# cloudflare/zkp-ecdsa

Measured on NVIDIA H100. Metric: ZKAttest proofs/sec, higher is better.
Workload: dtype u256/u258 (32-bit limbs, Montgomery)

## Files before the change

### __graft_entry__.py

```python
from __future__ import annotations

import hashlib
import os
import subprocess
import sys

ROOT = os.path.dirname(os.path.abspath(__file__))
CSRC = os.path.join(ROOT, 'zkp_ecdsa_b200', 'csrc')
LIB = os.path.join(ROOT, 'zkp_ecdsa_b200', 'libzkattest.so')
LIB_WAR = os.path.join(ROOT, 'zkp_ecdsa_b200', 'libzkattest_war256.so')
HOSTSIM = os.path.join(ROOT, 'tests', 'hostsim', 'libzkattest_hostsim.so')
HOSTSIM_WAR = os.path.join(ROOT, 'tests', 'hostsim', 'libzkattest_hostsim_war256.so')
PROBE_SRC = os.path.join(ROOT, 'tests', 'probe', 'zk_probe.cu')
PROBE = os.path.join(ROOT, 'tests', 'probe', 'libzkprobe.so')
PROBE_HOST = os.path.join(ROOT, 'tests', 'probe', 'libzkprobe_host.so')
PROBE_JAC_SRC = os.path.join(ROOT, 'tests', 'probe', 'zk_probe_jac.cu')
PROBE_JAC = os.path.join(ROOT, 'tests', 'probe', 'libzkprobe_jac.so')
PROBE_JAC_HOST = os.path.join(ROOT, 'tests', 'probe', 'libzkprobe_jac_host.so')
PROBE_SEED_SRC = os.path.join(ROOT, 'tests', 'probe', 'zk_probe_seed.cu')
PROBE_SEED = os.path.join(ROOT, 'tests', 'probe', 'libzkprobe_seed.so')
PROBE_SEED_HOST = os.path.join(ROOT, 'tests', 'probe', 'libzkprobe_seed_host.so')
ORACLE_CPU = os.path.join(ROOT, 'oracle', '_ref', 'libzkattest_cpu.so')
ARCH = ['-gencode', 'arch=compute_90a,code=sm_90a']
NVCC_FLAGS = ARCH + ['-O3', '-std=c++17', '-lineinfo',
              '--compiler-options', '-fPIC', '-shared']


def _sources():
    return sorted(os.path.join(CSRC, f) for f in os.listdir(CSRC) if f.endswith(('.cu', '.cuh', '.h', '.inc')))


def _stamp(extra='', files=()):
    h = hashlib.sha256(extra.encode())
    for p in _sources() + [os.path.join(ROOT, 'include', 'zkattest.h')] + list(files):
        h.update(p.encode())
        h.update(open(p, 'rb').read())
    return h.hexdigest()


def _build_if_stale(out, cmd, tag, files=()):
    stamp_file = out + '.stamp'
    stamp = _stamp(' '.join(cmd), files)
    if os.path.exists(out) and os.path.exists(stamp_file) and open(stamp_file).read() == stamp:
        return False
    print(f'[build] {tag}: {" ".join(cmd)}', flush=True)
    tmp = out + '.tmp'
    subprocess.check_call([tmp if c == out else c for c in cmd], cwd=ROOT)
    os.replace(tmp, out)
    open(stamp_file, 'w').write(stamp)
    return True


def build_lib():
    nvcc = os.environ.get('NVCC', '/usr/local/cuda/bin/nvcc')
    cmd = [nvcc] + NVCC_FLAGS + ['-I' + os.path.join(ROOT, 'include'), '-I' + CSRC, '-o', LIB,
                                 os.path.join(CSRC, 'zkattest.cu')]
    return _build_if_stale(LIB, cmd, 'libzkattest.so (sm_90a)')


def build_lib_war():
    nvcc = os.environ.get('NVCC', '/usr/local/cuda/bin/nvcc')
    cmd = [nvcc] + NVCC_FLAGS + ['-DZKA_PG_WAR256', '-I' + os.path.join(ROOT, 'include'), '-I' + CSRC, '-o', LIB_WAR,
                                 os.path.join(CSRC, 'zkattest.cu')]
    return _build_if_stale(LIB_WAR, cmd, 'libzkattest_war256.so (sm_90a)')


def build_hostsim(war=False):
    out = HOSTSIM_WAR if war else HOSTSIM
    os.makedirs(os.path.dirname(out), exist_ok=True)
    cmd = ['g++', '-std=c++17', '-O2', '-DZKA_HOSTSIM'] + (['-DZKA_PG_WAR256'] if war else []) + [
        '-x', 'c++', '-I' + os.path.join(ROOT, 'include'), '-I' + CSRC, '-fPIC', '-shared', '-o', out,
        os.path.join(CSRC, 'zkattest.cu')]
    return _build_if_stale(out, cmd, 'hostsim war256 (tests only)' if war else 'hostsim (tests only)')


def build_probe(host=False, jac=False):
    out = (PROBE_JAC_HOST if host else PROBE_JAC) if jac else (PROBE_HOST if host else PROBE)
    src = PROBE_JAC_SRC if jac else PROBE_SRC
    if host:
        cmd = ['g++', '-std=c++17', '-O2', '-DZKA_HOSTSIM', '-x', 'c++', '-fPIC', '-shared']
    else:
        cmd = [os.environ.get('NVCC', '/usr/local/cuda/bin/nvcc')] + NVCC_FLAGS
    cmd += ['-I' + os.path.join(ROOT, 'include'), '-I' + CSRC, '-o', out, src]
    tag = ('probe_jac' if jac else 'probe') + (' host (tests only)' if host else ' (sm_90a, tests only)')
    return _build_if_stale(out, cmd, tag, [PROBE_SRC, PROBE_JAC_SRC] if jac else [PROBE_SRC])


def build_probe_seed(host=False):
    out = PROBE_SEED_HOST if host else PROBE_SEED
    if host:
        cmd = ['g++', '-std=c++17', '-O2', '-DZKA_HOSTSIM', '-x', 'c++', '-fPIC', '-shared']
    else:
        cmd = [os.environ.get('NVCC', '/usr/local/cuda/bin/nvcc')] + NVCC_FLAGS
    cmd += ['-I' + os.path.join(ROOT, 'include'), '-I' + CSRC, '-o', out, PROBE_SEED_SRC]
    return _build_if_stale(out, cmd, 'probe_seed' + (' host (tests only)' if host else ' (sm_90a, tests only)'), [PROBE_SEED_SRC])


def build_oracle_cpu():
    src = os.path.join(ROOT, 'oracle', 'cpu', 'zkattest_cpu.cpp')
    hdr = os.path.join(ROOT, 'include', 'zkattest.h')
    if os.path.exists(ORACLE_CPU) and os.path.getmtime(ORACLE_CPU) >= max(os.path.getmtime(src), os.path.getmtime(hdr)):
        return False
    print('[build] oracle/cpu -> oracle/_ref/libzkattest_cpu.so', flush=True)
    subprocess.check_call(['make', '-C', os.path.join(ROOT, 'oracle', 'cpu')])
    return True


def build_tools():
    nvcc = os.environ.get('NVCC', '/usr/local/cuda/bin/nvcc')
    tdir = os.path.join(ROOT, 'tools')
    for name in ('imad_peak', 'mul_peak'):
        src, out = os.path.join(tdir, name + '.cu'), os.path.join(tdir, name)
        if not os.path.exists(src):
            continue
        if os.path.exists(out) and os.path.getmtime(out) >= max(os.path.getmtime(p) for p in _sources() + [src]):
            continue
        cmd = [nvcc] + ARCH + ['-O3', '-std=c++17', '-I' + CSRC,
               '-I' + os.path.join(ROOT, 'include'), '-o', out, src]
        print(f'[build] tools/{name}: {" ".join(cmd)}', flush=True)
        subprocess.check_call(cmd, cwd=ROOT)


def build() -> None:
    from concurrent.futures import ThreadPoolExecutor
    jobs = [build_lib, build_lib_war, build_hostsim, lambda: build_hostsim(war=True), build_oracle_cpu, build_tools,
            build_probe, lambda: build_probe(host=True), lambda: build_probe(jac=True),
            lambda: build_probe(host=True, jac=True), build_probe_seed, lambda: build_probe_seed(host=True)]
    with ThreadPoolExecutor(max_workers=min(len(jobs), max(1, (os.cpu_count() or 2)))) as ex:
        for f in [ex.submit(j) for j in jobs]:
            f.result()
    sys.path.insert(0, ROOT)
    import zkp_ecdsa_b200
    import oracle


def smoke() -> None:
    sys.path.insert(0, ROOT)
    import numpy as np
    from zkp_ecdsa_b200 import api, synth
    from oracle import flat
    from oracle import zkattest as OZ
    from oracle.big import Tape

    eng = api.Engine(device=0)
    rnd = synth.params_rnd(1)
    params = eng.generate_params_list(rnd=rnd)
    wl = synth.Workload(B=2, N=8, seed=1)
    tape = synth.random_tape(2, eng.lib.prove_tape_len(8), seed=2)
    res = eng.prove_batch(params, wl.msg_hash, wl.sig, wl.pk, wl.which, wl.ring, tape)
    assert (res.status == 0).all(), res.status
    oparams = OZ.generate_params_list(Tape(rnd))
    for b in range(2):
        pr = OZ.prove_signature_list(oparams, wl.msg_hash[b].tobytes(), wl.sig[b].tobytes(), wl.pk[b].tobytes(),
                                     int(wl.which[b]), wl.ring_ints(), Tape(tape[b].tobytes()))
        assert flat.ser_proof(pr) == res.proof_bytes(b), f'proof {b} differs from the oracle'
    from oracle import seed_tape as ST
    seed = bytes(range(32))
    rs = eng.prove_batch_seeded(params, wl.msg_hash[:1], wl.sig[:1], wl.pk[:1], wl.which[:1], wl.ring,
                                np.frombuffer(seed, np.uint8).reshape(1, 32).copy())
    assert rs.status[0] == 0, rs.status
    pr = OZ.prove_signature_list(oparams, wl.msg_hash[0].tobytes(), wl.sig[0].tobytes(), wl.pk[0].tobytes(),
                                 int(wl.which[0]), wl.ring_ints(), Tape(ST.prove_tape(seed, 80, 3)))
    assert flat.ser_proof(pr) == rs.proof_bytes(0), 'seeded proof differs from the oracle on the expanded tape'
    from zkp_ecdsa_b200 import verify_tape as VT
    vts = eng.lib.verify_tape_len(8, 80)
    ok = np.zeros(2, np.uint8)
    st = np.zeros(2, np.int32)
    eng.lib.verify_batch(params.handle, 2, wl.msg_hash, wl.ring, 8, res.proofs, res.proofs.shape[1], res.proof_len,
                         VT.random_verify_tape(2, vts, 8, 80, seed=3), vts, ok, st)
    assert list(ok) == [1, 1] and not st.any(), (ok, st)
    rw = synth.RingsWorkload(2, [17, 5], [1, 0], seed=5)
    rings = eng.load_rings(rw.rings)
    rt = synth.random_tape(2, eng.lib.prove_tape_len(17), seed=6)
    rr = eng.prove_batch_rings(params, rings, rw.ring_of, rw.msg_hash, rw.sig, rw.pk, rw.which, rt)
    assert (rr.status == 0).all(), rr.status
    for b in range(2):
        pr = OZ.prove_signature_list(oparams, rw.msg_hash[b].tobytes(), rw.sig[b].tobytes(), rw.pk[b].tobytes(),
                                     int(rw.which[b]), rw.ring_ints(int(rw.ring_of[b])), Tape(rt[b].tobytes()))
        assert flat.ser_proof(pr) == rr.proof_bytes(b), f'ring-set proof {b} differs from the oracle'
    rings.close()
    launched = eng.lib.launch_count()
    war = ''
    if os.path.exists(LIB_WAR):
        from oracle.curves import tomEdwards256, war256
        ew = api.Engine(device=0, proof_group='war256')
        pw = ew.generate_params_list(16, rnd=rnd)
        tw = synth.random_tape(1, ew.lib.prove_tape_len(8, 16), seed=4)
        rw = ew.prove_batch(pw, wl.msg_hash[:1], wl.sig[:1], wl.pk[:1], wl.which[:1], wl.ring, tw)
        assert (rw.status == 0).all(), rw.status
        flat.set_proof_group(war256)
        try:
            ow = OZ.generate_params_list(Tape(rnd), 16, war256)
            pr = OZ.prove_signature_list(ow, wl.msg_hash[0].tobytes(), wl.sig[0].tobytes(), wl.pk[0].tobytes(),
                                         int(wl.which[0]), wl.ring_ints(), Tape(tw[0].tobytes()))
            assert flat.ser_proof(pr) == rw.proof_bytes(0), 'war256 proof differs from the oracle'
        finally:
            flat.set_proof_group(tomEdwards256)
        launched += ew.lib.launch_count()
        war = '; war256 build: 1 proof bit-exact'
    print(f'smoke ok: 2 proofs bit-exact vs oracle and accepted by the verifier, 1 seeded proof bit-exact, '
          f'2 ring-set proofs over rings of depths 3 and 5 bit-exact{war}; '
          'kernels launched:', launched)


if __name__ == '__main__':
    build()
    if len(sys.argv) > 1 and sys.argv[1] == 'smoke':
        smoke()
```

### zkp_ecdsa_b200/capi.py

```python
from __future__ import annotations

import ctypes as C
import os
from typing import Optional

import numpy as np

_HERE = os.path.dirname(os.path.abspath(__file__))
DEFAULT_LIB = os.path.join(_HERE, 'libzkattest.so')

SYMBOLS = [
    'zka_init', 'zka_shutdown', 'zka_last_error', 'zka_version', 'zka_launch_count',
    'zka_params_generate', 'zka_params_create', 'zka_params_destroy', 'zka_key_to_int',
    'zka_proof_max_len', 'zka_prove_tape_len', 'zka_verify_tape_len',
    'zka_prove_batch', 'zka_verify_batch',
    'zka_tom_commit_batch', 'zka_p256_mul_batch', 'zka_field_op_batch', 'zka_hash80_batch',
    'zka_get_stream', 'zka_set_profiling', 'zka_profile_reset', 'zka_profile_json', 'zka_config',
    'zka_lanes', 'zka_set_option', 'zka_proofs_pack', 'zka_proofs_unpack', 'zka_verify_batch_ex', 'zka_verify_tape_len_ex',
    'zka_verify_exp_batch', 'zka_verify_membership_batch', 'zka_verify_equality_batch', 'zka_verify_mult_batch',
    'zka_verify_pointadd_batch', 'zka_prove_exp_batch', 'zka_prove_membership_batch',
    'zka_prove_equality_batch', 'zka_prove_mult_batch', 'zka_prove_pointadd_batch', 'zka_stat', 'zka_proof_group', 'zka_set_progress', 'zka_chunk_schedule',
    'zka_prove_batch_seeded', 'zka_verify_batch_seeded', 'zka_seed_tape',
    'zka_rings_create', 'zka_rings_destroy', 'zka_prove_batch_rings', 'zka_prove_batch_rings_seeded', 'zka_verify_batch_rings',
    'zka_verify_batch_rings_seeded',
# ... 96 lines not shown
                                              C.c_size_t, C.c_void_p, C.c_void_p, C.c_size_t, C.c_void_p, C.c_void_p, C.c_uint32]
            L.zka_set_option.argtypes = [C.c_void_p, C.c_char_p, C.c_long]
            L.zka_stat.restype = C.c_longlong
            L.zka_stat.argtypes = [C.c_void_p, C.c_char_p]
            L.zka_verify_exp_batch.argtypes = [C.c_void_p, C.c_void_p, C.c_uint32] + [C.c_void_p] * 6 + [C.c_size_t, C.c_void_p, C.c_void_p,
                                               C.c_size_t, C.c_uint32, C.c_void_p, C.c_void_p]
            L.zka_verify_membership_batch.argtypes = [C.c_void_p, C.c_void_p, C.c_uint32, C.c_void_p, C.c_void_p, C.c_uint32, C.c_void_p,
                                                      C.c_size_t, C.c_void_p, C.c_void_p, C.c_size_t, C.c_void_p, C.c_void_p]
            for f in ('zka_verify_equality_batch', 'zka_verify_mult_batch', 'zka_verify_pointadd_batch'):
                getattr(L, f).argtypes = [C.c_void_p, C.c_void_p, C.c_uint32, C.c_void_p, C.c_void_p, C.c_void_p, C.c_size_t,
                                          C.c_void_p, C.c_void_p]
            L.zka_prove_exp_batch.argtypes = [C.c_void_p, C.c_void_p, C.c_uint32] + [C.c_void_p] * 5 + [C.c_size_t, C.c_void_p, C.c_size_t,
                                              C.c_void_p, C.c_void_p]
            L.zka_prove_membership_batch.argtypes = [C.c_void_p, C.c_void_p, C.c_uint32, C.c_void_p, C.c_void_p, C.c_void_p, C.c_uint32,
                                                     C.c_void_p, C.c_size_t, C.c_void_p, C.c_size_t, C.c_void_p, C.c_void_p]
            for f in ('zka_prove_equality_batch', 'zka_prove_mult_batch'):
                getattr(L, f).argtypes = [C.c_void_p, C.c_void_p, C.c_uint32, C.c_void_p, C.c_void_p, C.c_size_t, C.c_void_p, C.c_void_p,
                                          C.c_void_p]
            L.zka_prove_pointadd_batch.argtypes = [C.c_void_p, C.c_void_p, C.c_uint32, C.c_void_p, C.c_void_p, C.c_void_p, C.c_size_t,
                                                   C.c_void_p, C.c_void_p, C.c_void_p]
            L.zka_proofs_pack.argtypes = [C.c_void_p, C.c_uint32, C.c_void_p, C.c_size_t, C.c_void_p, C.c_void_p, C.c_size_t,
                                          C.c_void_p, C.c_void_p]
            L.zka_proofs_unpack.argtypes = [C.c_void_p, C.c_uint32, C.c_void_p, C.c_size_t, C.c_void_p, C.c_void_p, C.c_size_t,
                                            C.c_void_p, C.c_void_p]
        if hasattr(L, 'zka_seed_tape'):
            L.zka_prove_batch_seeded.argtypes = [C.c_void_p, C.c_void_p, C.c_uint32] + [C.c_void_p] * 5 + [C.c_uint32, C.c_void_p,
                                                 C.c_void_p, C.c_size_t, C.c_void_p, C.c_void_p]
            L.zka_verify_batch_seeded.argtypes = [C.c_void_p, C.c_void_p, C.c_uint32, C.c_void_p, C.c_void_p, C.c_uint32, C.c_void_p,
                                                  C.c_size_t, C.c_void_p, C.c_void_p, C.c_uint32, C.c_void_p, C.c_void_p]
            L.zka_seed_tape.argtypes = [C.c_void_p, C.c_int, C.c_uint32, C.c_void_p, C.c_uint32, C.c_uint32, C.c_uint32, C.c_void_p,
                                        C.c_size_t]
        if hasattr(L, 'zka_rings_create'):
            L.zka_rings_create.argtypes = [C.c_void_p, C.c_uint32, C.c_void_p, C.c_void_p, C.POINTER(C.c_void_p)]
            L.zka_rings_destroy.argtypes = [C.c_void_p]
            L.zka_prove_batch_rings.argtypes = [C.c_void_p, C.c_void_p, C.c_void_p, C.c_void_p, C.c_uint32] + [C.c_void_p] * 5 + [
                C.c_size_t, C.c_void_p, C.c_size_t, C.c_void_p, C.c_void_p]
            L.zka_prove_batch_rings_seeded.argtypes = [C.c_void_p, C.c_void_p, C.c_void_p, C.c_void_p, C.c_uint32] + [C.c_void_p] * 6 + [
                C.c_size_t, C.c_void_p, C.c_void_p]
            L.zka_verify_batch_rings.argtypes = [C.c_void_p, C.c_void_p, C.c_void_p, C.c_void_p, C.c_uint32, C.c_void_p, C.c_void_p,
                                                 C.c_size_t, C.c_void_p, C.c_void_p, C.c_size_t, C.c_uint32, C.c_void_p, C.c_void_p]
            L.zka_verify_batch_rings_seeded.argtypes = [C.c_void_p, C.c_void_p, C.c_void_p, C.c_void_p, C.c_uint32, C.c_void_p,
                                                        C.c_void_p, C.c_size_t, C.c_void_p, C.c_void_p, C.c_uint32, C.c_void_p,
                                                        C.c_void_p]
        ctx = C.c_void_p()
        rc = L.zka_init(device, C.byref(ctx))
        if rc != 0 or not ctx:
            raise ZkaError(f'zka_init(device={device}) failed with {rc}: no usable CUDA device '
                           '(libzkattest has no CPU fallback)')
        self.ctx = ctx
        self.device = device

    def close(self):
        if getattr(self, 'ctx', None):
            self.lib.zka_shutdown(self.ctx)
            self.ctx = None

    def _check(self, rc, what):
        if rc != 0:
            raise ZkaError(f'{what} failed ({rc}): {self.lib.zka_last_error(self.ctx).decode()}')

    def launch_count(self) -> int:
        return int(self.lib.zka_launch_count(self.ctx))

    def stream_ptr(self) -> int:
        return int(self.lib.zka_get_stream(self.ctx) or 0)

    def set_profiling(self, on: bool):
        self._check(self.lib.zka_set_profiling(self.ctx, 1 if on else 0), 'zka_set_profiling')

    def profile_reset(self):
        self._check(self.lib.zka_profile_reset(self.ctx), 'zka_profile_reset')

    def profile(self) -> dict:
        import json
        n = self.lib.zka_profile_json(self.ctx, None, 0)
        buf = C.create_string_buffer(int(n) + 16)
        self.lib.zka_profile_json(self.ctx, buf, len(buf))
        return json.loads(buf.value.decode())

    def config(self) -> dict:
        w, nw, ch = C.c_int(), C.c_int(), C.c_int()
        self._check(self.lib.zka_config(self.ctx, C.byref(w), C.byref(nw), C.byref(ch)), 'zka_config')
        lanes = int(self.lib.zka_lanes(self.ctx)) if hasattr(self.lib, 'zka_lanes') else 1
        return {'tom_w': w.value, 'tom_nwin': nw.value, 'chunk': ch.value, 'lanes': lanes}

    def set_option(self, key: str, value: int):
        self._check(self.lib.zka_set_option(self.ctx, key.encode(), int(value)), f'zka_set_option({key})')

    def chunk_schedule(self, B: int, host_buffers: bool = False):
        off = np.zeros(4096, np.uint32)
        self.lib.zka_chunk_schedule.argtypes = [C.c_void_p, C.c_uint32, C.c_int, C.c_void_p, C.c_uint32]
        n = self.lib.zka_chunk_schedule(self.ctx, B, 1 if host_buffers else 0, _ptr(off), off.size)
        if n < 0:
            raise ZkaError('zka_chunk_schedule')
        return [int(v) for v in off[:n + 1]]

    def set_progress(self, flags: Optional[np.ndarray]):
        self.lib.zka_set_progress.argtypes = [C.c_void_p, C.c_void_p, C.c_uint32]
        if flags is None:
            self._check(self.lib.zka_set_progress(self.ctx, None, 0), 'zka_set_progress')
        else:
            assert flags.dtype == np.uint32 and flags.flags['C_CONTIGUOUS']
            self._check(self.lib.zka_set_progress(self.ctx, _ptr(flags), flags.size), 'zka_set_progress')

    def stat(self, key: str) -> int:
        return int(self.lib.zka_stat(self.ctx, key.encode()))

    def proof_max_len(self, ring_size, sec_level=80): return int(self.lib.zka_proof_max_len(ring_size, sec_level))
    def prove_tape_len(self, ring_size, sec_level=80): return int(self.lib.zka_prove_tape_len(ring_size, sec_level))
    def verify_tape_len(self, ring_size, sec_level=80): return int(self.lib.zka_verify_tape_len(ring_size, sec_level))

    def params_generate(self, rnd: bytes):
        assert len(rnd) == 64
        hn = np.zeros(65, np.uint8)
        hp = np.zeros(self.wp, np.uint8)
        self._check(self.lib.zka_params_generate(self.ctx, _ptr(rnd), _ptr(hn), _ptr(hp)), 'zka_params_generate')
        return hn.tobytes(), hp.tobytes()

    def params_create(self, h_nist: bytes, h_proof: bytes, sec_level: int = 80):
        h = C.c_void_p()
        self._check(self.lib.zka_params_create(self.ctx, _ptr(h_nist), _ptr(h_proof), sec_level, C.byref(h)),
                    'zka_params_create')
        return h

    def params_destroy(self, h):
        self.lib.zka_params_destroy(h)

    def key_to_int(self, pk: np.ndarray):
        count = pk.shape[0]
        out = np.zeros((count, 32), np.uint8)
        st = np.zeros(count, np.int32)
        self._check(self.lib.zka_key_to_int(self.ctx, count, _ptr(pk), _ptr(out), _ptr(st)), 'zka_key_to_int')
        return out, st

    def prove_batch(self, params, B, msg_hash, sig, pk, which, ring, N, tape, tape_stride,
                    proofs, proof_stride, proof_len, status):
        self._check(self.lib.zka_prove_batch(self.ctx, params, B, _ptr(msg_hash), _ptr(sig), _ptr(pk), _ptr(which),
                                             _ptr(ring), N, _ptr(tape), tape_stride, _ptr(proofs), proof_stride,
                                             _ptr(proof_len), _ptr(status)), 'zka_prove_batch')

    def verify_batch(self, params, B, msg_hash, ring, N, proofs, proof_stride, proof_len, tape, tape_stride,
                     ok, status):
        self._check(self.lib.zka_verify_batch(self.ctx, params, B, _ptr(msg_hash), _ptr(ring), N, _ptr(proofs),
                                              proof_stride, _ptr(proof_len), _ptr(tape), tape_stride, _ptr(ok),
                                              _ptr(status)), 'zka_verify_batch')

    def verify_tape_len_ex(self, ring_size, sec_level, samples):
        return int(self.lib.zka_verify_tape_len_ex(ring_size, sec_level, samples))

    def verify_batch_ex(self, params, B, msg_hash, ring, N, proofs, proof_stride, proof_len, tape, tape_stride, ok, status, samples):
        self._check(self.lib.zka_verify_batch_ex(self.ctx, params, B, _ptr(msg_hash), _ptr(ring), N, _ptr(proofs), proof_stride,
                                                 _ptr(proof_len), _ptr(tape), tape_stride, _ptr(ok), _ptr(status), samples),
                    'zka_verify_batch_ex')

    def prove_batch_seeded(self, params, B, msg_hash, sig, pk, which, ring, N, seeds, proofs, proof_stride, proof_len, status):
        self._check(self.lib.zka_prove_batch_seeded(self.ctx, params, B, _ptr(msg_hash), _ptr(sig), _ptr(pk), _ptr(which), _ptr(ring),
                                                    N, _ptr(seeds), _ptr(proofs), proof_stride, _ptr(proof_len), _ptr(status)),
                    'zka_prove_batch_seeded')

    def verify_batch_seeded(self, params, B, msg_hash, ring, N, proofs, proof_stride, proof_len, seeds, samples, ok, status):
        self._check(self.lib.zka_verify_batch_seeded(self.ctx, params, B, _ptr(msg_hash), _ptr(ring), N, _ptr(proofs), proof_stride,
                                                     _ptr(proof_len), _ptr(seeds), samples, _ptr(ok), _ptr(status)),
                    'zka_verify_batch_seeded')

    def seed_tape(self, kind, seeds, ring_size, sec_level=80, samples=20) -> np.ndarray:
        B = seeds.shape[0]
        ln = self.prove_tape_len(ring_size, sec_level) if kind == 0 else self.verify_tape_len_ex(ring_size, sec_level, samples)
# ... 136 lines not shown
```

### zkp_ecdsa_b200/csrc/zk_launch.cuh

```cuda
#pragma once
#include <stdint.h>
#include <stdlib.h>
#include <string.h>

#include <map>
#include <stdexcept>
#include <string>
#include <typeinfo>
#include <vector>

#include <cxxabi.h>

#if !defined(ZKA_HOSTSIM)
#include <cuda_runtime.h>
#endif

namespace zk {

#if !defined(ZKA_HOSTSIM)

#define ZK_CUDA_CHECK(expr)                                                                   \
  do {                                                                                        \
    cudaError_t _e = (expr);                                                                  \
    if (_e != cudaSuccess)                                                                    \
// ... 86 lines not shown
inline void copy_d2h_2d(Stream& st, void* h, size_t hpitch, const void* d, size_t dpitch, size_t width, size_t height) {
  if (width && height) ZK_CUDA_CHECK(cudaMemcpy2DAsync(h, hpitch, d, dpitch, width, height, cudaMemcpyDefault, st.s));
}
inline void dev_memset(Stream& st, void* d, int v, size_t n) {
  if (n) ZK_CUDA_CHECK(cudaMemsetAsync(d, v, n, st.s));
}
inline void sync(Stream& st) {
  ZK_CUDA_CHECK(cudaStreamSynchronize(st.s));
  if (!st.pending.empty()) prof_collect(st);
}
struct Event { cudaEvent_t e = nullptr; };
inline void stream_create(Stream& st) {
  if (!st.s) ZK_CUDA_CHECK(cudaStreamCreateWithFlags(&st.s, cudaStreamNonBlocking));
}
inline void stream_destroy(Stream& st) {
  if (st.s) cudaStreamDestroy(st.s);
  st.s = nullptr;
}
inline void ev_record(Event& ev, Stream& st) {
  if (!ev.e) ZK_CUDA_CHECK(cudaEventCreateWithFlags(&ev.e, cudaEventDisableTiming));
  ZK_CUDA_CHECK(cudaEventRecord(ev.e, st.s));
}
inline void ev_wait(Stream& st, Event& ev) {
  if (ev.e) ZK_CUDA_CHECK(cudaStreamWaitEvent(st.s, ev.e, 0));
}
inline void ev_destroy(Event& ev) {
  if (ev.e) cudaEventDestroy(ev.e);
  ev.e = nullptr;
}
inline bool is_device_ptr(const void* p) {
  cudaPointerAttributes a;
  cudaError_t e = cudaPointerGetAttributes(&a, p);
  if (e != cudaSuccess) {
    cudaGetLastError();
    return false;
  }
  return a.type == cudaMemoryTypeDevice || a.type == cudaMemoryTypeManaged;
}

#else

struct ProfEntry {
  uint64_t launches = 0;
  double ms = 0.0;
  uint64_t items = 0;
};
struct Stream {
  uint64_t launches = 0;
  bool profiling = false;
  std::map<std::string, ProfEntry> prof;
};
template <class Task>
inline void launch(Stream& st, long long n, const Task& task) {
  for (long long t = 0; t < n; t++) task((int)t);
  st.launches++;
}
inline void* dev_alloc(size_t bytes) { return calloc(bytes ? bytes : 1, 1); }
inline void dev_free(void* p) { free(p); }
inline void copy_h2d(Stream&, void* d, const void* h, size_t n) { if (n) memcpy(d, h, n); }
inline void copy_d2h(Stream&, void* h, const void* d, size_t n) { if (n) memcpy(h, d, n); }
inline void copy_d2d(Stream&, void* d, const void* s, size_t n) { if (n) memcpy(d, s, n); }
inline void copy_d2h_2d(Stream&, void* h, size_t hpitch, const void* d, size_t dpitch, size_t width, size_t height) {
  for (size_t r = 0; r < height; r++) memcpy((char*)h + r * hpitch, (const char*)d + r * dpitch, width);
}
inline void dev_memset(Stream&, void* d, int v, size_t n) { if (n) memset(d, v, n); }
inline void sync(Stream&) {}
struct Event {};
inline void stream_create(Stream&) {}
inline void stream_destroy(Stream&) {}
inline void ev_record(Event&, Stream&) {}
inline void ev_wait(Stream&, Event&) {}
inline void ev_destroy(Event&) {}
inline bool is_device_ptr(const void*) { return false; }

#endif

struct DevBuf {
  void* p = nullptr;
  size_t cap = 0;
  DevBuf() = default;
  DevBuf(const DevBuf&) = delete;
  DevBuf& operator=(const DevBuf&) = delete;
  ~DevBuf() { dev_free(p); }
  template <class T>
  T* get(size_t count) {
    size_t bytes = count * sizeof(T);
    if (bytes > cap) {
      dev_free(p);
      size_t want = bytes + bytes / 8 + 256;
      p = dev_alloc(want);
      cap = want;
    }
    return reinterpret_cast<T*>(p);
  }
};

struct Cursor {
  DevBuf *next_, *end_;
  template <size_t N>
  explicit Cursor(DevBuf (&pool)[N]) : next_(pool), end_(pool + N) {}
  DevBuf& next() {
    if (next_ == end_) throw std::runtime_error("workspace pool exhausted");
    return *next_++;
  }
  template <class T>
  T* take(size_t count) { return next().get<T>(count); }
  template <class T>
  T* take_if(bool need, size_t count) {
    T* p = take<T>(need ? count : 0);
    return need ? p : nullptr;
  }
};

}
```

### zkp_ecdsa_b200/csrc/zk_ops.cuh

```cuda
#pragma once
#include "zk_curves.cuh"
#include "zk_layout.h"
#include "zk_sha256.cuh"

namespace zk {

#if defined(__CUDA_ARCH__)
#define ZK_SET_STATUS(ptr, code) atomicCAS((int*)(ptr), 0, (int)(code))
#define ZK_SET_STATUS_OVER(ptr, code, over) \
  do {                                      \
    atomicCAS((int*)(ptr), 0, (int)(code)); \
    atomicCAS((int*)(ptr), (int)(over), (int)(code)); \
  } while (0)
#else
#define ZK_SET_STATUS_OVER(ptr, code, over)              \
  do {                                                   \
    if (*(ptr) == 0 || *(ptr) == (over)) *(ptr) = (code); \
  } while (0)
#define ZK_SET_STATUS(ptr, code) \
  do {                           \
    if (*(ptr) == 0) *(ptr) = (code); \
  } while (0)
#endif

// ... 97 lines not shown
#pragma unroll
  for (int i = 0; i < 9; i++) {
    const uint32_t a = q.x[i], b = q.y[i];
    q.x[i] = neg ? b : a;
    q.y[i] = neg ? a : b;
    q.k[i] = neg ? nk[i] : q.k[i];
  }
}
ZK_HD void tom_ld_pre(TomPre& q, const uint32_t* m) {
#if defined(__CUDA_ARCH__)
  const uint4* v = reinterpret_cast<const uint4*>(m);
  uint32_t w[32];
#pragma unroll
  for (int i = 0; i < 7; i++) {
    uint4 u = __ldg(v + i);
    w[4 * i] = u.x; w[4 * i + 1] = u.y; w[4 * i + 2] = u.z; w[4 * i + 3] = u.w;
  }
#pragma unroll
  for (int i = 0; i < 9; i++) { q.x[i] = w[i]; q.y[i] = w[9 + i]; q.k[i] = w[18 + i]; }
#else
  ld<9>(q.x, m); ld<9>(q.y, m + 9); ld<9>(q.k, m + 18);
#endif
}

#endif

ZK_HD void ld4(uint32_t* w, const void* p) {
#if defined(__CUDA_ARCH__)
  const uint4 u = *reinterpret_cast<const uint4*>(p);
  w[0] = u.x; w[1] = u.y; w[2] = u.z; w[3] = u.w;
#else
  const uint32_t* q = reinterpret_cast<const uint32_t*>(p);
  for (int i = 0; i < 4; i++) w[i] = q[i];
#endif
}
ZK_HD void st4(void* p, const uint32_t* w) {
#if defined(__CUDA_ARCH__)
  *reinterpret_cast<uint4*>(p) = make_uint4(w[0], w[1], w[2], w[3]);
#else
  uint32_t* q = reinterpret_cast<uint32_t*>(p);
  for (int i = 0; i < 4; i++) q[i] = w[i];
#endif
}
ZK_HD void ld8v(uint32_t* r, const uint32_t* p) { ld4(r, p); ld4(r + 4, p + 4); }
ZK_HD void st8v(uint32_t* p, const uint32_t* r) { st4(p, r); st4(p + 4, r + 4); }
ZK_HD bool aligned16(const void* p) { return ((size_t)p & 15) == 0; }

template <int N, int CB>
ZK_HD uint32_t enc_byte(int i, uint32_t tag, const uint32_t* x, const uint32_t* y) {
  if (i == 0) return tag;
  if (i >= 1 + 2 * CB) return 0u;
  const uint32_t* c = i <= CB ? x : y;
  const int pos = CB - 1 - (i <= CB ? i - 1 : i - 1 - CB);
  return (pos >> 2) < N ? ((c[pos >> 2] >> (8 * (pos & 3))) & 0xffu) : 0u;
}
template <int N, int CB>
ZK_HD void store_point_words(uint8_t* o, uint32_t tag, const uint32_t* x, const uint32_t* y) {
  uint32_t w[BSTRIDE / 4];
#pragma unroll
  for (int j = 0; j < BSTRIDE / 4; j++)
    w[j] = enc_byte<N, CB>(4 * j, tag, x, y) | (enc_byte<N, CB>(4 * j + 1, tag, x, y) << 8) |
           (enc_byte<N, CB>(4 * j + 2, tag, x, y) << 16) | (enc_byte<N, CB>(4 * j + 3, tag, x, y) << 24);
  if (aligned16(o)) {
#pragma unroll
    for (int j = 0; j < BSTRIDE / 16; j++) st4(o + 16 * j, w + 4 * j);
  } else {
    uint32_t* ow = reinterpret_cast<uint32_t*>(o);
#pragma unroll
    for (int j = 0; j < BSTRIDE / 4; j++) ow[j] = w[j];
  }
}

ZK_HD uint32_t digit4(const uint32_t* k, int j) { return (k[j >> 3] >> (4 * (j & 7))) & 15u; }
ZK_HD uint32_t digit8(const uint32_t* k, int j) { return (k[j >> 2] >> (8 * (j & 3))) & 255u; }
ZK_HD uint32_t digit_w(const uint32_t* k, int pos, int w) {
  int wi = pos >> 5, sh = pos & 31;
  uint64_t v = k[wi];
  if (wi + 1 < 8) v |= (uint64_t)k[wi + 1] << 32;
  return (uint32_t)(v >> sh) & ((1u << w) - 1u);
}

ZK_HD int fb_entries(int w) { return (1 << (w - 1)) + 1; }
ZK_HD int fb_windows(int w) { return (256 + w) / w; }
ZK_HD uint32_t signed_digit(const uint32_t* k, int j, int w, uint32_t& carry, bool& neg) {
  const int pos = j * w;
  uint32_t d = carry;
  if (pos < 256) d += digit_w(k, pos, (256 - pos) < w ? (256 - pos) : w);
  const uint32_t half = 1u << (w - 1);
  neg = d > half;
  carry = neg ? 1u : 0u;
  return neg ? (1u << w) - d : d;
}

ZK_HD uint32_t bswap32(uint32_t x) {
#if defined(__CUDA_ARCH__)
  return __byte_perm(x, 0u, 0x0123);
#else
  return (x >> 24) | ((x >> 8) & 0xff00u) | ((x << 8) & 0xff0000u) | (x << 24);
#endif
}
ZK_HD void tape_draw(uint32_t* r, const uint8_t* tape, int draw) {
  const uint8_t* p = tape + 32 * (size_t)draw;
#if defined(__CUDA_ARCH__)
  if (aligned16(p)) {
    const uint4 a = __ldg(reinterpret_cast<const uint4*>(p)), b = __ldg(reinterpret_cast<const uint4*>(p) + 1);
    r[7] = bswap32(a.x); r[6] = bswap32(a.y); r[5] = bswap32(a.z); r[4] = bswap32(a.w);
    r[3] = bswap32(b.x); r[2] = bswap32(b.y); r[1] = bswap32(b.z); r[0] = bswap32(b.w);
    return;
  }
#endif
#pragma unroll
  for (int i = 0; i < 8; i++) {
    const uint8_t* q = p + 28 - 4 * i;
    r[i] = ((uint32_t)q[0] << 24) | ((uint32_t)q[1] << 16) | ((uint32_t)q[2] << 8) | (uint32_t)q[3];
  }
}

#define WEI_PT P256Pt
#define WEI_AFF P256Aff
#define WEI_JAC P256Jac
#define WEI_F P256p
#define WEI_FN(n) p256_##n
#define WEI_T(n) P256##n
#include "zk_weier_ops.inc"
#undef WEI_PT
#undef WEI_AFF
#undef WEI_JAC
#undef WEI_F
#undef WEI_FN
#undef WEI_T

enum : int { KEY_W_MIN = 5, KEY_W_MAX = 8, KEY_CAP = 52 * 17 };
ZK_HD int key_window_bits(uint32_t count, uint32_t B, uint32_t uses) {
  int best = KEY_W_MIN;
  uint64_t best_cost = ~0ull;
  for (int w = KEY_W_MIN; w <= KEY_W_MAX; w++) {
    const uint64_t nwin = (uint64_t)fb_windows(w), ne = (uint64_t)fb_entries(w);
    if (w > KEY_W_MIN && (uint64_t)count * nwin * ne > (uint64_t)B * KEY_CAP) break;
    const uint64_t cost = nwin * ((uint64_t)count * (ne - 1) * 2 + (uint64_t)B * uses);
    if (cost < best_cost) { best_cost = cost; best = w; }
  }
  return best;
}
ZK_HD size_t key_table_words(int w) { return (size_t)fb_windows(w) * fb_entries(w) * P256_AFF_WORDS; }

enum : int { RT_W = 5, RT_NWIN = 52, RT_ROW = 16, RT_ENTRIES = RT_NWIN * RT_ROW };
struct P256RowsSignedTask {
  const uint32_t* pows;
  uint32_t* rows;
  const uint32_t* count_dev = nullptr;
  ZK_HD void operator()(int t) const {
    if (count_dev && (uint32_t)(t / RT_NWIN) >= *count_dev) return;
    P256Pt p, acc;
    p256_ld_proj(p, pows + (size_t)t * P256_PROJ_WORDS);
    acc = p;
    uint32_t* out = rows + (size_t)t * RT_ROW * P256_PROJ_WORDS;
    for (int d = 1; d <= RT_ROW; d++) {
      p256_st_proj(out + (size_t)(d - 1) * P256_PROJ_WORDS, acc);
      if (d < RT_ROW) p256_add(acc, acc, p);
    }
  }
};
ZK_HD void p256_accum_rtab(P256Pt& acc, const uint32_t* tab, const uint32_t* k) {
  uint32_t carry = 0;
  for (int j = 0; j < RT_NWIN; j++) {
    const int pos = j * RT_W;
    uint32_t d = (pos < 256 ? digit_w(k, pos, (256 - pos) < RT_W ? (256 - pos) : RT_W) : 0u) + carry;
    carry = d > 16 ? 1u : 0u;
    const bool neg = d > 16;
    if (neg) d = 32 - d;
    if (d) {
      P256Aff q;
      p256_ld_aff(q, tab + ((size_t)j * RT_ROW + (d - 1)) * P256_AFF_WORDS);
      if (neg) P256p::neg(q.y, q.y);
      p256_madd(acc, acc, q);
    }
  }
}
#if defined(ZKA_PG_WAR256)
enum : int { GJOBS_PER_ITEM = 28, TOM_EXT_WORDS = 24 };
#else
enum : int { GJOBS_PER_ITEM = 28, TOM_EXT_WORDS = 36 };
#endif
ZK_HD int item_gpart_of_job(int j) {
  if (j < 6) return j;
  if (j < 30) {
    const int m = (j - 6) / 6, u = (j - 6) % 6;
    return 6 + 5 * m + (u < 4 ? u : u - 1);
  }
  return 26 + ((j - 30) >> 1);
}
ZK_HD int item_job_of_gpart(int g) {
  if (g < 6) return g;
  if (g < 26) {
    const int m = (g - 6) / 5, u = (g - 6) % 5;
    return 6 + 6 * m + (u < 4 ? u : 5);
  }
  return 30 + 2 * (g - 26);
}
#if defined(ZKA_PG_WAR256)
#include "zk_ops_war.cuh"
#else
struct TomPowsTask {
  const uint32_t* base_aff;
  uint32_t* pows;
  int nbase, nwin, w;
  ZK_HD void operator()(int t) const {
    uint32_t x[9], y[9];
    ld<9>(x, base_aff + (size_t)t * TOM_AFF_WORDS);
    ld<9>(y, base_aff + (size_t)t * TOM_AFF_WORDS + 9);
    TomPt p;
    tom_from_affine(p, x, y);
    for (int j = 0; j < nwin; j++) {
      uint32_t* o = pows + ((size_t)t * nwin + j) * 36;
      st<9>(o, p.x); st<9>(o + 9, p.y); st<9>(o + 18, p.t); st<9>(o + 27, p.z);
      for (int k = 0; k < w; k++) tom_dbl(p, p);
    }
  }
};
struct TomRowsTask {
  const uint32_t* pows;
  uint32_t* rows;
  int w;
  ZK_HD void operator()(int t) const {
    TomPt p, acc;
    const uint32_t* s = pows + (size_t)t * 36;
    ld<9>(p.x, s); ld<9>(p.y, s + 9); ld<9>(p.t, s + 18); ld<9>(p.z, s + 27);
    tom_set_identity(acc);
    const int ne = fb_entries(w);
    uint32_t* out = rows + (size_t)t * ne * TOM_PROJ_WORDS;
    for (int d = 0; d < ne; d++) {
      uint32_t* o = out + (size_t)d * TOM_PROJ_WORDS;
      tom_st_xyz(o, acc.x, acc.y, acc.z);
      tom_add(acc, acc, p);
    }
  }
};
struct TomRowsHiTask {
  const uint32_t* pows;
  uint32_t* hi;
  uint32_t* rows;
  int w;
  ZK_HD void operator()(int t) const {
    TomPt p, acc;
    const uint32_t* s = pows + (size_t)t * 36;
    ld<9>(p.x, s); ld<9>(p.y, s + 9); ld<9>(p.t, s + 18); ld<9>(p.z, s + 27);
    for (int k = 0; k < 8; k++) tom_dbl(p, p);
    tom_set_identity(acc);
    const int nh = 1 << (w - 9);
    for (int m = 0; m < nh; m++) {
      uint32_t* o = hi + ((size_t)t * nh + m) * 36;
      st<9>(o, acc.x); st<9>(o + 9, acc.y); st<9>(o + 18, acc.t); st<9>(o + 27, acc.z);
      tom_add(acc, acc, p);
    }
    tom_st_xyz(rows + ((size_t)t * fb_entries(w) + ((size_t)1 << (w - 1))) * TOM_PROJ_WORDS, acc.x, acc.y, acc.z);
  }
};
struct TomRowsLoTask {
  const uint32_t* pows;
  const uint32_t* hi;
  uint32_t* rows;
  int w;
  ZK_HD void operator()(int t) const {
    const int nh = 1 << (w - 9);
    const int j = t / nh, m = t % nh;
    TomPt p, acc;
    const uint32_t* s = pows + (size_t)j * 36;
    ld<9>(p.x, s); ld<9>(p.y, s + 9); ld<9>(p.t, s + 18); ld<9>(p.z, s + 27);
    const uint32_t* h = hi + (size_t)t * 36;
    ld<9>(acc.x, h); ld<9>(acc.y, h + 9); ld<9>(acc.t, h + 18); ld<9>(acc.z, h + 27);
    uint32_t* out = rows + ((size_t)j * fb_entries(w) + ((size_t)m << 8)) * TOM_PROJ_WORDS;
    for (int d = 0; d < 256; d++) {
      uint32_t* o = out + (size_t)d * TOM_PROJ_WORDS;
      tom_st_xyz(o, acc.x, acc.y, acc.z);
      tom_add(acc, acc, p);
    }
  }
};
struct TomTabE2Task {
  const uint32_t* proj;
  uint32_t* pre;
  int count;
  ZK_HD void operator()(int t) const {
    using F = Tomp;
    constexpr int CH = 16;
    const int lo = t * CH;
    int n = count - lo;
    if (n > CH) n = CH;
    if (n <= 0) return;
    uint32_t pf[CH][9];
    uint32_t acc[9], y[9], z[9], den[9];
    F::set_one(acc);
    for (int k = 0; k < n; k++) {
      const uint32_t* src = proj + (size_t)(lo + k) * TOM_PROJ_WORDS;
      uint32_t xx[9];
      tom_ld_xyz(xx, y, z, src);
      F::mul(den, y, z);
      F::mul(acc, acc, den);
      copy_n<9>(pf[k], acc);
    }
    uint32_t inv[9], s2[9], dd2[9];
    F::inv(inv, acc);
    tom_const(s2, TOM_SQRTND1);
    tom_const(dd2, TOM_2D2);
    for (int k = n - 1; k >= 0; k--) {
      const uint32_t* src = proj + (size_t)(lo + k) * TOM_PROJ_WORDS;
      uint32_t x[9], di[9], w[9], v[9], kk[9], ym[9], yp[9];
      tom_ld_xyz(x, y, z, src);
      F::mul(den, y, z);
      if (k > 0) F::mul(di, inv, pf[k - 1]); else copy_n<9>(di, inv);
      F::mul(inv, inv, den);
      F::mul(w, x, y);
      F::mul(w, w, di);
      F::mul(w, w, s2);
      F::sqr(v, z);
      F::mul(v, v, di);
      F::mul(kk, w, v);
      F::mul(kk, kk, dd2);
      F::sub(ym, v, w);
      F::add(yp, v, w);
      F::reduce(ym); F::reduce(yp); F::reduce(kk);
      uint32_t* o = pre + (size_t)(lo + k) * TOM_PRE_WORDS;
      st<9>(o, ym); st<9>(o + 9, yp); st<9>(o + 18, kk);
      for (int i = 27; i < 32; i++) o[i] = 0;
    }
  }
};

struct TomNormTask {
  const uint32_t* proj;
  uint32_t* aff;
  uint8_t* bytes;
  int count;
  int chunk;
  int e2;
  int aff_mod, aff_lim;
  int stride;
  ZK_HD static void canon2p(uint32_t* r) {
    uint32_t t[9], p2[9];
#pragma unroll
    for (int i = 0; i < 9; i++) p2[i] = (FpTom::p(i) << 1) | (i > 0 ? (FpTom::p(i - 1) >> 31) : 0u);
    uint32_t br = sub_n<9>(t, r, p2);
    csel_n<9>(r, br == 0, t, r);
    br = sub_p<FpTom>(t, r);
    csel_n<9>(r, br == 0, t, r);
  }
  ZK_HD void operator()(int t) const {
    using F = Tomp;
    const int lo = t * chunk;
    int n = count - lo;
    if (n > chunk) n = chunk;
    if (n <= 0) return;
    uint32_t pre[NORM_CHUNK_MAX][9];
    uint32_t acc[9], z[9], h[9], den[9];
    F::set_one(acc);
    for (int k = 0; k < n; k++) {
      const uint32_t* src = proj + (size_t)(lo + k) * stride;
      uint32_t xx[9], yy[9];
      if (e2) {
        tom_ld_efgh(xx, yy, z, h, src);
        F::mul(den, z, h);
      } else {
        tom_ld_xyz(xx, yy, den, src);
      }
      F::mul(acc, acc, den);
      copy_n<9>(pre[k], acc);
    }
    uint32_t inv[9], cxk[9], is2[9], one_plain[9];
    F::inv(inv, acc);
    tom_const(cxk, e2 ? TOM_INVSQRTND : TOM_INVSQRTA);
    tom_const(is2, TOM_INVSQRTND1);
    zero_n<9>(one_plain);
    one_plain[0] = 1;
    for (int k = n - 1; k >= 0; k--) {
      const uint32_t* src = proj + (size_t)(lo + k) * stride;
      uint32_t X[9], Y[9], di[9];
      if (e2) {
        tom_ld_efgh(X, Y, z, h, src);
        F::mul(den, z, h);
        F::mul(X, X, h);
        F::mul(Y, Y, z);
      } else {
        tom_ld_xyz(X, Y, den, src);
      }
      if (k > 0) F::mul(di, inv, pre[k - 1]); else copy_n<9>(di, inv);
      F::mul(inv, inv, den);
      if (bytes) {
        uint32_t Dp[9], cx[9], cy[9];
        F::mul(Dp, di, one_plain);
        F::mul(cx, X, cxk);
        F::mul(cx, cx, Dp);
        F::mul(cy, Y, Dp);
        canon2p(cx);
        canon2p(cy);
        store_point_words<9, 33>(bytes + (size_t)(lo + k) * BSTRIDE, 0x04u, cx, cy);
      }
      if (aff && ((lo + k) % aff_mod) < aff_lim) {
        uint32_t x[9], y[9];
        F::mul(x, X, di);
        if (e2) F::mul(x, x, is2);
        F::mul(y, Y, di);
        uint32_t* a = aff + (size_t)(lo + k) * TOM_AFF_WORDS;
        st<9>(a, x);
        st<9>(a + 9, y);
      }
    }
  }
};

ZK_HD void tom2_ld_entry(TomPre& q, const uint32_t* tab, int j, size_t ne, uint32_t d, bool neg) {
  tom_ld_pre(q, tab + ((size_t)j * ne + d) * TOM_PRE_WORDS);
  tom2_pre_neg(q, neg);
}

struct TomCommitTask {
  const uint32_t* jv;
  const uint32_t* jr;
  const uint32_t* gtab;
  const uint32_t* htab;
  uint32_t* proj;
  int w, nwin;
  int xyz = 0;
  ZK_HD void operator()(int t) const {
    uint32_t v[8], r[8];
    ld<8>(v, jv + (size_t)t * 8);
    ld<8>(r, jr + (size_t)t * 8);
    const size_t ne = (size_t)fb_entries(w);
    uint32_t cv = 0, cr = 0;
    bool nv, nr;
    TomPre q;
    uint32_t dv = signed_digit(v, 0, w, cv, nv);
    tom2_ld_entry(q, gtab, 0, ne, dv, nv);
    TomPt acc;
    tom2_from_pre(acc, q);
    for (int j = 0;; j++) {
      const uint32_t dr = signed_digit(r, j, w, cr, nr);
      tom2_ld_entry(q, htab, j, ne, dr, nr);
      if (j == nwin - 1) break;
      tom2_madd<true>(acc, acc, q);
      dv = signed_digit(v, j + 1, w, cv, nv);
      tom2_ld_entry(q, gtab, j + 1, ne, dv, nv);
      tom2_madd<true>(acc, acc, q);
    }
    if (xyz) {
      tom2_madd<false>(acc, acc, q);
      tom_st_xyz(proj + (size_t)t * TOM_PROJ_WORDS, acc.x, acc.y, acc.z);
    } else {
      TomEfgh e;
      tom2_madd_end(e, acc, q);
      tom_st_efgh(proj + (size_t)t * TOM_E2_WORDS, e);
    }
  }
};

struct TomCommitGTask {
  const uint32_t* jv;
  const uint32_t* gtab;
  uint32_t* ext;
  int w, nwin;
  ZK_HD void operator()(int t) const {
    const int item = t / GJOBS_PER_ITEM, g = t % GJOBS_PER_ITEM;
    uint32_t v[8];
    ld<8>(v, jv + ((size_t)item * JOBS_PER_ITEM + item_job_of_gpart(g)) * 8);
    const size_t ne = (size_t)fb_entries(w);
    uint32_t carry = 0;
    bool neg;
    TomPre q;
    const uint32_t d0 = signed_digit(v, 0, w, carry, neg);
    tom2_ld_entry(q, gtab, 0, ne, d0, neg);
    TomPt acc;
    tom2_from_pre<TompCommit>(acc, q);
#pragma unroll 1
    for (int j = 1; j < nwin; j++) {
      const uint32_t d = signed_digit(v, j, w, carry, neg);
      tom2_ld_entry(q, gtab, j, ne, d, neg);
      tom2_madd<true, TompCommit>(acc, acc, q);
    }
    uint32_t* o = ext + (size_t)t * TOM_EXT_WORDS;
    st<9>(o, acc.x); st<9>(o + 9, acc.y); st<9>(o + 18, acc.t); st<9>(o + 27, acc.z);
  }
};
struct TomCommitHTask {
  const uint32_t* jr;
  const uint32_t* htab;
  const uint32_t* ext;
  uint32_t* proj;
  int w, nwin;
  ZK_HD void operator()(int t) const {
    const int item = t / JOBS_PER_ITEM, jb = t % JOBS_PER_ITEM;
    uint32_t r[8];
    ld<8>(r, jr + (size_t)t * 8);
    TomPt acc;
    const uint32_t* s = ext + ((size_t)item * GJOBS_PER_ITEM + item_gpart_of_job(jb)) * TOM_EXT_WORDS;
    ld<9>(acc.x, s); ld<9>(acc.y, s + 9); ld<9>(acc.t, s + 18); ld<9>(acc.z, s + 27);
    const size_t ne = (size_t)fb_entries(w);
    uint32_t carry = 0;
    bool neg;
    TomPre q;
#pragma unroll 1
    for (int j = 0; j < nwin - 1; j++) {
      const uint32_t d = signed_digit(r, j, w, carry, neg);
      tom2_ld_entry(q, htab, j, ne, d, neg);
      tom2_madd<true, TompCommit>(acc, acc, q);
    }
    const uint32_t d = signed_digit(r, nwin - 1, w, carry, neg);
    tom2_ld_entry(q, htab, nwin - 1, ne, d, neg);
    TomEfgh e;
    tom2_madd_end<TompCommit>(e, acc, q);
    tom_st_efgh(proj + (size_t)t * TOM_E2_WORDS, e);
  }
};

#if !defined(ZKA_HOSTSIM) && defined(ZKA_COMMIT_MINBLOCKS)
template <> struct TaskMinBlocks<TomCommitHTask> { static constexpr int value = ZKA_COMMIT_MINBLOCKS; };
template <> struct TaskMinBlocks<TomCommitGTask> { static constexpr int value = ZKA_COMMIT_MINBLOCKS; };
template <> struct TaskMinBlocks<TomCommitTask> { static constexpr int value = ZKA_COMMIT_MINBLOCKS; };
#endif

#endif

enum : int { GK_BLOCK_BITS = 10 };
ZK_HD int gk_block_bits(int n) { return n < GK_BLOCK_BITS ? n : GK_BLOCK_BITS; }
ZK_HD void gk_block_sum(uint32_t* acc, const uint32_t* ring_m, const uint32_t (*fz)[8], const uint32_t (*fo)[8], int n,
                        int k, uint32_t blk, const uint32_t* vw) {
  using F = Tomq;
  uint32_t P[21][8];
  F::set_one(P[n]);
  for (int j = n - 1; j >= k; j--) F::mul(P[j], P[j + 1], ((blk >> (j - k)) & 1u) ? fo[j] : fz[j]);
  for (int j = k - 1; j >= 0; j--) F::mul(P[j], P[j + 1], fz[j]);
  zero_n<8>(acc);
  const size_t base = (size_t)blk << k;
  const uint32_t cnt = 1u << k;
  for (uint32_t l = 0;;) {
    uint32_t vi[8], term[8];
    ld<8>(vi, ring_m + (base + l) * 8);
    if (vw) F::sub(vi, vw, vi);
    F::mul(term, vi, P[0]);
    F::add(acc, acc, term);
    l++;
    if (l == cnt) break;
    int tz = 0;
    while (!((l >> tz) & 1u)) tz++;
    F::mul(P[tz], P[tz + 1], fo[tz]);
    for (int j = tz - 1; j >= 0; j--) F::mul(P[j], P[j + 1], fz[j]);
  }
}

ZK_HD bool hash_pt_fetch(uint32_t* t, const uint8_t* p, int len) {
  if (((size_t)p & 3) || len < 64 || len > 68) return false;
  if (aligned16(p)) {
#pragma unroll
    for (int j = 0; j < 4; j++) ld4(t + 4 * j, p + 16 * j);
    t[16] = len > 64 ? *reinterpret_cast<const uint32_t*>(p + 64) : 0u;
    return true;
  }
  const uint32_t* q = reinterpret_cast<const uint32_t*>(p);
#pragma unroll
  for (int j = 0; j < 17; j++) t[j] = (4 * j < len) ? q[j] : 0u;
  return true;
}
template <class Src>
ZK_HD void hash_points80(uint32_t* c3, const Src& src, int npts) {
  Sha256 h;
  h.init();
  uint32_t nx[17], cu[17];
  int nlen = 0;
  const uint8_t* np = npts > 0 ? src(0, nlen) : nullptr;
  bool nfast = npts > 0 && hash_pt_fetch(nx, np, nlen);
  for (int i = 0; i < npts; i++) {
    const uint8_t* p = np;
    const int len = nlen;
    const bool fast = nfast;
#pragma unroll
    for (int j = 0; j < 17; j++) cu[j] = nx[j];
    if (i + 1 < npts) {
      np = src(i + 1, nlen);
      nfast = hash_pt_fetch(nx, np, nlen);
    }
    if (fast) h.feed17(cu, len);
    else h.update(p, len);
  }
  h.final80(c3);
}

ZK_HD void challenge_to_limbs(uint32_t* r, const uint32_t* c3) {
  zero_n<8>(r);
  r[0] = c3[0]; r[1] = c3[1]; r[2] = c3[2];
}

// ... 125 lines not shown
```

### zkp_ecdsa_b200/csrc/zk_ops_war.cuh

```cuda
#pragma once

#define WEI_PT WarPt
#define WEI_AFF WarAff
#define WEI_JAC WarJac
#define WEI_F Warp
#define WEI_FN(n) war_##n
#define WEI_T(n) War##n
#include "zk_weier_ops.inc"
#undef WEI_PT
#undef WEI_AFF
#undef WEI_JAC
#undef WEI_F
#undef WEI_FN
#undef WEI_T

struct TomNormTask {
  const uint32_t* proj;
  uint32_t* aff;
  uint8_t* bytes;
  int count;
  int chunk;
  int e2;
  int aff_mod, aff_lim;
  int stride;
  ZK_HD void operator()(int t) const {
    using F = Warp;
    const int lo = t * chunk;
    int n = count - lo;
    if (n > chunk) n = chunk;
    if (n <= 0) return;
    uint32_t pre[NORM_CHUNK_MAX][8];
    uint32_t acc[8], z[8], one[8];
    F::set_one(one);
    copy_n<8>(acc, one);
    for (int k = 0; k < n; k++) {
      ld<8>(z, proj + (size_t)(lo + k) * stride + 16);
      if (is_zero_n<8>(z)) copy_n<8>(z, one);
      F::mul(acc, acc, z);
      copy_n<8>(pre[k], acc);
    }
    uint32_t inv[8];
    F::inv(inv, acc);
    for (int k = n - 1; k >= 0; k--) {
      const uint32_t* src = proj + (size_t)(lo + k) * stride;
      ld<8>(z, src + 16);
      const bool isinf = is_zero_n<8>(z);
      if (isinf) copy_n<8>(z, one);
      uint32_t zi[8];
      if (k > 0) F::mul(zi, inv, pre[k - 1]); else copy_n<8>(zi, inv);
      F::mul(inv, inv, z);
      uint32_t X[8], Y[8], x[8], y[8];
      ld<8>(X, src);
      ld<8>(Y, src + 8);
      F::mul(x, X, zi);
      F::mul(y, Y, zi);
      if (aff && ((lo + k) % aff_mod) < aff_lim) {
        uint32_t* a = aff + (size_t)(lo + k) * TOM_AFF_WORDS;
        st<8>(a, x);
        st<8>(a + 8, y);
      }
      if (bytes) {
        uint32_t cx[8], cy[8];
        F::from_mont(cx, x);
        F::from_mont(cy, y);
        if (isinf) { zero_n<8>(cx); zero_n<8>(cy); }
        store_point_words<8, 32>(bytes + (size_t)(lo + k) * BSTRIDE, isinf ? 0x00u : 0x04u, cx, cy);
      }
    }
  }
};

struct TomCommitTask {
  const uint32_t* jv;
  const uint32_t* jr;
  const uint32_t* gtab;
  const uint32_t* htab;
  uint32_t* proj;
  int w, nwin;
  int xyz = 0;
  ZK_HD void operator()(int t) const {
    uint32_t v[8], r[8];
    ld<8>(v, jv + (size_t)t * 8);
    ld<8>(r, jr + (size_t)t * 8);
    WarJac aj;
    war_set_identity_jac(aj);
    war_accum_fixed_jac(aj, gtab, v, w);
    war_accum_fixed_jac(aj, htab, r, w);
    WarPt acc;
    war_jac_to_hom(acc, aj);
    war_st_proj(proj + (size_t)t * TOM_PROJ_WORDS, acc);
  }
};
struct TomCommitGTask {
  const uint32_t* jv;
  const uint32_t* gtab;
  uint32_t* ext;
  int w, nwin;
  ZK_HD void operator()(int t) const {
    const int item = t / GJOBS_PER_ITEM, g = t % GJOBS_PER_ITEM;
    uint32_t v[8];
    ld<8>(v, jv + ((size_t)item * JOBS_PER_ITEM + item_job_of_gpart(g)) * 8);
    WarJac aj;
    war_set_identity_jac(aj);
    war_accum_fixed_jac(aj, gtab, v, w);
    WarPt acc;
    war_jac_to_hom(acc, aj);
    war_st_proj(ext + (size_t)t * TOM_EXT_WORDS, acc);
  }
};
struct TomCommitHTask {
  const uint32_t* jr;
  const uint32_t* htab;
  const uint32_t* ext;
  uint32_t* proj;
  int w, nwin;
  ZK_HD void operator()(int t) const {
    const int item = t / JOBS_PER_ITEM, jb = t % JOBS_PER_ITEM;
    uint32_t r[8];
    ld<8>(r, jr + (size_t)t * 8);
    WarPt acc;
    war_ld_proj(acc, ext + ((size_t)item * GJOBS_PER_ITEM + item_gpart_of_job(jb)) * TOM_EXT_WORDS);
    war_accum_fixed(acc, htab, r, w);
    war_st_proj(proj + (size_t)t * TOM_PROJ_WORDS, acc);
  }
};
```

### zkp_ecdsa_b200/csrc/zk_prove.cuh

```cuda
#pragma once
#include "zk_sigma.cuh"

namespace zk {

struct ProveCtx {
  int B;
  int S;
  int N;
  int n;
  int M;
  int tom_w, tom_nwin;
  int mode;
  int head_len;
  const uint8_t* base;
  const uint8_t* s_in;
  const uint8_t* q_in;
  uint32_t* base_aff;
  const uint8_t* msg_hash;
  const uint8_t* sig;
  const uint8_t* pk;
  const uint32_t* which;
  uint32_t* which_s;
  const uint8_t* tape;
  size_t tape_stride;
  uint32_t tape_draws;
  const uint32_t* ring_m;
  const uint32_t* ring_of;
  const uint32_t* ring_base;
  const uint32_t* ring_size;
  const uint32_t* ring_depth;
  const uint32_t* g_tab8;
  const uint32_t* h_tab8;
  int h_w;
  const uint32_t* g_tabw;
  int g_w;
  const uint32_t* tg_tab;
  const uint32_t* th_tab;
  const uint8_t* tg_bytes;
  uint32_t* s1;
  uint32_t* pk_aff;
  uint32_t* q_aff;
  uint8_t* q_inf;
  uint32_t* r_aff;
  uint8_t* r_bytes;
  uint32_t* u12;
  uint32_t* tab_of;
  uint32_t* tab_rep;
  uint32_t* tab_count;
  uint32_t* rpows;
  uint32_t* rrows;
  uint32_t* rtab;
  uint32_t* pa_T;
  uint32_t* pa_A;
  uint32_t* pa_T_aff;
  uint8_t* pa_T_inf;
  uint32_t* pa_A_aff;
  uint8_t* pa_A_bytes;
  uint8_t* pa_A_inf;
  uint32_t *s1_jv, *s1_jr, *s1_proj, *s1_aff;
  uint8_t* s1_bytes;
  uint32_t* chal;
  uint32_t* zcount;
  uint32_t* item_base;
  uint32_t* item_total;
  uint32_t* rep_off;
  uint32_t* gk_off;
  uint32_t* item_b;
  uint32_t* item_i;
  uint32_t* item_k;
  uint32_t* pb_T1;
  uint32_t* pb_T1_aff;
  uint8_t* pb_T1_inf;
  uint32_t *s2_jv, *s2_jr, *s2_proj, *s2_aff;
  uint8_t* s2_bytes;
  uint32_t* item_inv;
  uint32_t* secrets;
  uint32_t* item_chal;
  uint32_t* gk_dv;
  uint32_t* gk_part;
  uint32_t* gk_lag;
  uint32_t* gk_x;
  uint8_t* proofs;
  size_t proof_stride;
  uint32_t* proof_len;
  int32_t* status;

  ZK_HD size_t s2_job(size_t item, int j) const { return item * JOBS_PER_ITEM + j; }
  ZK_HD size_t s2_der(size_t item, int j) const { return (size_t)M * JOBS_PER_ITEM + item * DERS_PER_ITEM + j; }
  ZK_HD size_t s2_gk(size_t b, int j) const { return (size_t)M * (JOBS_PER_ITEM + DERS_PER_ITEM) + b * 4 * n + j; }
  ZK_HD size_t s2_count() const { return (size_t)M * (JOBS_PER_ITEM + DERS_PER_ITEM) + (size_t)B * 4 * n; }
  ZK_HD size_t s1_pt(size_t b, int j) const { return b * (2 + 2 * S) + j; }
  ZK_HD const uint8_t* tape_of(int b) const { return tape + (size_t)b * tape_stride; }
  ZK_HD const uint32_t* ring_of_row(int b) const { return ring_of ? ring_m + (size_t)8 * ring_base[ring_of[b]] : ring_m; }
  ZK_HD uint32_t ring_size_row(int b) const { return ring_of ? ring_size[ring_of[b]] : (uint32_t)N; }
// ... 1114 lines not shown
```

### zkp_ecdsa_b200/csrc/zk_verify.cuh

```cuda
#pragma once
#include "zk_prove.cuh"

namespace zk {

enum : int {
  V_SAMPLES = 20,
  V_ENT_PER_SAMPLE = 2 + PA_ENTRIES,
  V_SEG = 20,
  V_ENT_SEG = V_SEG * V_ENT_PER_SAMPLE + 2,
  V_IDX_PAD = 96,
  V_PART_WORDS = 7 * 8,
  MSM_C = 6,
  MSM_NWIN = 43,
  MSM_C_N = 4,
  MSM_NWIN_N = 65,
  AGG_SKIP = 0,
  AGG_TOM_PASS = 1,
  AGG_NIST_PASS = 2,
  AGG_CTL_WORDS = 4,
};

ZK_LAYOUT_FN size_t verify_tape_len(int n, int , int K = V_SAMPLES) {
  return (size_t)32 * (2 * n + 1) + V_IDX_PAD + (size_t)32 * 25 * K;
}

struct VerifyCtx {
  int B, S, N, n;
  int K;
  int mode;
  const uint8_t* q_ext;
  int tom_w, tom_nwin;
  const uint8_t* msg_hash;
  const uint8_t* proofs;
  size_t proof_stride;
  const uint32_t* proof_len;
  const uint8_t* tape;
  size_t tape_stride;
  const uint32_t* ring_m;
  const uint32_t* ring_of;
  const uint32_t* ring_base;
  const uint32_t* ring_depth;
  const uint32_t* g_tab8;
  const uint32_t* h_tab8;
  int h_w;
  const uint32_t* tg_tab;
  const uint32_t* th_tab;
  const uint8_t* tg_bytes;
  uint32_t* rep_off;
  uint32_t* gk_off;
  uint32_t* tagbits;
  uint32_t* chal;
  uint8_t* gk_ok_len;
  uint8_t* gk_tape_bad;
  uint32_t* r_aff;
  uint32_t* q_aff;
  uint8_t* q_inf;
  uint32_t* rpows;
  uint32_t* rrows;
  uint32_t* rtab;
  uint32_t* samp_idx;
  uint32_t* samp_draw;
  uint32_t* sp_T;
  uint32_t* sp_T_aff;
  uint8_t* sp_T_inf;
  uint32_t *ta_jv, *ta_jr, *ta_proj, *ta_aff;
  uint32_t *td_proj, *td_aff;
  uint8_t* td_bytes;
  uint32_t* item_chal;
  uint32_t* ent_scalar;
  uint32_t* ent_off;
  uint32_t* ent_pre;
  uint32_t* ent_cnt;
  uint32_t* part;
  uint32_t* nent_scalar;
  uint32_t* nent_aff;
  uint8_t* nent_skip;
  uint32_t* gk_scalar;
  uint32_t* gk_part;
  uint32_t* gk_pre;
  uint32_t *fx_jv, *fx_jr, *fx_proj;
  uint32_t* nfix;
  uint32_t* win_w;
  uint32_t* win_g;
  uint32_t* win_n;
  uint8_t* id_flags;
  const uint32_t* agg_ctl;
  uint8_t* ok;
  int32_t* status;

  ZK_HD int ent_tom() const { return K * V_ENT_PER_SAMPLE + 2; }
  ZK_HD int ent_nist() const { return K + 1; }
  ZK_HD int segs() const { return (K + V_SEG - 1) / V_SEG; }
  ZK_HD const uint8_t* proof_of(int b) const { return proofs + (size_t)b * proof_stride; }
  ZK_HD const uint8_t* tape_of(int b) const { return tape + (size_t)b * tape_stride; }
  ZK_HD const uint32_t* ring_of_row(int b) const { return ring_of ? ring_m + (size_t)8 * ring_base[ring_of[b]] : ring_m; }
  ZK_HD int n_row(int b) const { return ring_of ? (int)ring_depth[ring_of[b]] : n; }
  ZK_HD size_t gk_tape_bytes(int b) const { return mode == 1 ? 0 : (size_t)32 * (2 * n_row(b) + 1); }
  ZK_HD const uint8_t* exp_tape(int b) const { return tape_of(b) + gk_tape_bytes(b) + V_IDX_PAD; }
  ZK_HD size_t ta_pt(size_t sample, int j) const { return sample * 2 + j; }
  ZK_HD size_t td_pt(size_t sample, int j) const { return sample * DERS_PER_ITEM + j; }
};

struct VLayoutTask {
  VerifyCtx c;
  ZK_HD void operator()(int b) const {
    using Fn = P256n;
    using Fp = P256p;
    c.status[b] = ZKA_OK;
    c.ok[b] = 0;
    const uint8_t* pr = c.proof_of(b);
    const uint32_t len = c.proof_len[b];
    bool bad = len < HEAD_LEN || len > c.proof_stride;
    uint32_t off = HEAD_LEN, tg[3] = {0, 0, 0};
    for (int i = 0; i < c.S && !bad; i++) {
// ... 989 lines not shown
```

### zkp_ecdsa_b200/csrc/zkattest.cu

```cuda
#include "zkattest.h"

#include <math.h>
#include <stdio.h>

#include <algorithm>
#include <atomic>
#include <cmath>
#include <mutex>
#include <chrono>
#include <memory>
#include <thread>
#include <string>
#include <vector>

#include "zk_launch.cuh"
#include "zk_prove.cuh"
#include "zk_seed.cuh"
#include "zk_verify_agg.cuh"

namespace zk {
struct ParsePointsTask {
  const uint8_t* nist;
  const uint8_t* tom;
  uint32_t* nist_aff;
// ... 184 lines not shown
  uint8_t* rows;
  size_t stride;
  const uint32_t* len;
  const uint64_t* off;
  uint8_t* packed;
  size_t cap;
  int pieces;
  int dir;
  ZK_HD void operator()(int t) const {
    const int b = t / pieces, j = t % pieces;
    const size_t o = (size_t)16 * j;
    if (o >= len[b]) return;
    const size_t po = (size_t)off[b] + o;
    if (po + 16 > cap) return;
    uint8_t* r = rows + (size_t)b * stride + o;
    uint8_t* q = packed + po;
    if (dir == 0) { for (int i = 0; i < 16; i++) q[i] = o + i < stride ? r[i] : 0; }
    else { for (int i = 0; i < 16; i++) if (o + i < stride) r[i] = q[i]; }
  }
};
struct PackCopy16Task {
  uint8_t* rows;
  size_t stride;
  const uint32_t* len;
  const uint64_t* off;
  uint8_t* packed;
  size_t cap;
  int pieces;
  int dir;
  ZK_HD void operator()(int t) const {
    const int b = t / pieces, j = t % pieces;
    const size_t o = (size_t)16 * j;
    if (o >= len[b]) return;
    const size_t po = (size_t)off[b] + o;
    if (po + 16 > cap) return;
    U4* r = reinterpret_cast<U4*>(rows + (size_t)b * stride + o);
    U4* q = reinterpret_cast<U4*>(packed + po);
    if (dir == 0) *q = *r; else *r = *q;
  }
};

}

using namespace zk;

namespace {

struct FixedTable {
  DevBuf buf;
  uint32_t* tab = nullptr;
};

}

struct Lane {
  Stream st;
  Stream cs_in, cs_out;
  Event ev_small[2], ev_tape[2], ev_done[2], ev_out[2];
  Stream aux[2];
  Event ev_fork, ev_join[2];
  DevBuf w[51];
  DevBuf in[2][10], out[2][3];
  DevBuf agg[8], agg_tom[5 + 2 * AGG_MAX_LEVELS], agg_nist[5 + 2 * AGG_MAX_LEVELS];
  std::string err;
  ~Lane() {
    for (int i = 0; i < 2; i++) {
      ev_destroy(ev_small[i]); ev_destroy(ev_tape[i]); ev_destroy(ev_done[i]); ev_destroy(ev_out[i]);
    }
    ev_destroy(ev_fork); ev_destroy(ev_join[0]); ev_destroy(ev_join[1]);
    stream_destroy(cs_in);
    stream_destroy(cs_out);
    stream_destroy(aux[0]);
    stream_destroy(aux[1]);
    stream_destroy(st);
  }
};

struct zka_ctx : Lane {
  int device = 0;
  std::vector<std::unique_ptr<Lane>> extra;
  int nlanes = 3;
  DevBuf ring_in, ring_m;
  Lane& lane(int i) { return i == 0 ? *this : *extra[i - 1]; }
  int tom_w = 22, tom_nwin = 12;
  int chunk = 4096;
  int host_chunk = 2048;
  volatile uint32_t* progress = nullptr;
  uint32_t progress_cap = 0;
  int agg = 1;
  int agg_c = 0;
  uint64_t agg_pass = 0, agg_fail = 0;
  std::mutex stat_mu;
  std::mutex copy_mu;
  int agg_c_last = 0;
  bool tape_split = true;
  int p256_hw = 20;
  FixedTable g8;
  FixedTable gw;
  FixedTable tg;
  DevBuf tg_bytes;
  DevBuf lag;
  int lag_n = -1;
};

struct zka_params {
  zka_ctx* ctx = nullptr;
  uint32_t sec_level = 80;
  FixedTable h8;
  int h_w = 20;
  FixedTable th;
  uint8_t h_nist[65];
  uint8_t h_proof[WP];
};

struct zka_rings {
  zka_ctx* ctx = nullptr;
  uint32_t R = 0;
  std::vector<uint32_t> size;
  std::vector<int> depth;
  DevBuf ring_m, ring_base, ring_size, ring_depth;
  DevBuf lag;
};

namespace {

int fail(zka_ctx* ctx, int code, const std::string& msg) {
  if (ctx) ctx->err = msg;
  return code;
}
template <class Fn>
int guarded(zka_ctx* ctx, Fn&& body) {
  try {
    return body();
  } catch (const std::exception& e) {
    return fail(ctx, ZKA_E_CUDA, e.what());
  }
}

template <class Src>
void agg_msm(Stream& st, Cursor A, const Src& src, const AggPlan& pl, const uint32_t* ctl, const uint32_t** rootA,
             const uint32_t** rootB) {
  const AggDigits& D = pl.D;
  const int nwin = D.nwin, nb = D.nb, nseg = (nb + 1 + AGG_SEG - 1) / AGG_SEG;
  const size_t cap = (size_t)src.slots();
  uint32_t* hist = A.take<uint32_t>((size_t)nwin * (nb + 1));
  uint32_t* bstart = A.take<uint32_t>((size_t)nwin * (nb + 2));
  uint32_t* segtot = A.take<uint32_t>((size_t)nwin * nseg);
  uint32_t* sorted = A.take<uint32_t>((size_t)nwin * cap);
  uint32_t* bsum = A.take<uint32_t>((size_t)nwin * nb * Src::PTW);
  dev_memset(st, hist, 0, (size_t)nwin * (nb + 1) * 4);
  launch(st, (long long)cap, AggHistTask<Src>{src, D, ctl, hist});
  launch(st, (long long)nwin * nseg, AggSegSumTask{ctl, hist, segtot, nb, nseg});
  launch(st, nwin, AggSegScanTask{ctl, segtot, nseg});
  launch(st, (long long)nwin * nseg, AggOffsetsTask{ctl, segtot, hist, bstart, nb, nseg});
  launch(st, (long long)cap, AggScatterTask<Src>{src, D, ctl, hist, sorted, cap});
  launch(st, (long long)nwin * nb, AggBucketTask<Src>{src, ctl, bstart, sorted, bsum, cap, nb});
  const uint32_t *inA = bsum, *inB = nullptr;
  int nin = nb, ll = 0;
  for (int lv = 0; lv < pl.levels; lv++) {
    const int nout = nin >> pl.lm[lv];
    uint32_t* oA = A.take<uint32_t>((size_t)nwin * nout * Src::PTW);
    uint32_t* oB = A.take<uint32_t>((size_t)nwin * nout * Src::PTW);
    launch(st, (long long)nwin * nout, AggLevelTask<Src>{ctl, inA, inB, oA, oB, nin, pl.lm[lv], ll, nwin, D.top_shift});
    inA = oA; inB = oB; nin = nout; ll += pl.lm[lv];
  }
  *rootA = inA;
  *rootB = inB;
}

int ceil_log2(uint32_t v) {
  int n = 0;
  while ((1ull << n) < v) n++;
  return n;
}


static int g_norm_slots = 132 * 4;
static bool g_norm_model = true;
inline int norm_chunk_for(long long count, int per_point = 11) {
  if (!g_norm_model) {
    long long c = count / 100000;
    if (c < 8) c = 8;
    if (c > NORM_CHUNK_MAX) c = NORM_CHUNK_MAX;
    return (int)c;
  }
  int best = 8;
  long long best_cost = -1;
  for (int c = 8; c <= NORM_CHUNK_MAX; c++) {
    const long long threads = (count + c - 1) / c, ctas = (threads + 127) / 128;
    const long long waves = (ctas + g_norm_slots - 1) / g_norm_slots;
    const long long cost = waves * ((long long)per_point * c + 70);
    if (best_cost < 0 || cost < best_cost) { best_cost = cost; best = c; }
  }
  return best;
}
inline void launch_p256_norm(Stream& st, const uint32_t* proj, uint32_t* aff, uint8_t* bytes, uint8_t* inf, long long count) {
  if (count <= 0) return;
  const int ch = norm_chunk_for(count, bytes ? 7 : 5);
  launch(st, (count + ch - 1) / ch, P256NormTask{proj, aff, bytes, inf, (int)count, ch});
}
inline void launch_tom_norm(Stream& st, const uint32_t* proj, uint32_t* aff, uint8_t* bytes, long long count, int e2,
                            int aff_mod = 1, int aff_lim = 1, int stride = 0) {
  if (count <= 0) return;
  const int ch = norm_chunk_for(count);
  if (stride == 0) stride = e2 ? TOM_E2_WORDS : TOM_PROJ_WORDS;
  launch(st, (count + ch - 1) / ch, TomNormTask{proj, aff, bytes, (int)count, ch, e2, aff_mod, aff_lim, stride});
}

void build_p256_tab(zka_ctx* ctx, const uint32_t* base_aff_dev, FixedTable& out, int w) {
  Stream& st = ctx->st;
  const int nwin = fb_windows(w);
  const size_t E = (size_t)fb_entries(w), count = (size_t)nwin * E;
  DevBuf pows, rows;
  uint32_t* d_pows = pows.get<uint32_t>((size_t)nwin * P256_PROJ_WORDS);
  uint32_t* d_rows = rows.get<uint32_t>(count * P256_PROJ_WORDS);
  out.tab = out.buf.get<uint32_t>(count * P256_AFF_WORDS);
  launch(st, 1, P256PowsTask{base_aff_dev, nullptr, d_pows, 1, nwin, w});
  if (w > 9) {
    DevBuf hi;
    const int nh = 1 << (w - 9);
    uint32_t* d_hi = hi.get<uint32_t>((size_t)nwin * nh * P256_PROJ_WORDS);
    launch(st, nwin, P256RowsHiTask{d_pows, d_hi, d_rows, w});
    launch(st, (long long)nwin * nh, P256RowsLoTask{d_pows, d_hi, d_rows, w});
    sync(st);
  } else {
    launch(st, nwin, P256RowsTask{d_pows, d_rows, w});
  }
  launch_p256_norm(st, d_rows, out.tab, nullptr, nullptr, (long long)(count));
  sync(st);
}
#if defined(ZKA_PG_WAR256)
void build_tom_tab(zka_ctx* ctx, const uint32_t* base_aff_dev, FixedTable& out) {
  Stream& st = ctx->st;
  const int w = ctx->tom_w, nwin = fb_windows(w);
  const size_t E = (size_t)fb_entries(w), count = (size_t)nwin * E;
  DevBuf pows, rows;
  uint32_t* d_pows = pows.get<uint32_t>((size_t)nwin * P256_PROJ_WORDS);
  uint32_t* d_rows = rows.get<uint32_t>(count * P256_PROJ_WORDS);
  out.tab = out.buf.get<uint32_t>(count * TOM_PRE_WORDS);
  launch(st, 1, WarPowsTask{base_aff_dev, nullptr, d_pows, 1, nwin, w});
  if (w > 9) {
    DevBuf hi;
    const int nh = 1 << (w - 9);
    uint32_t* d_hi = hi.get<uint32_t>((size_t)nwin * nh * P256_PROJ_WORDS);
    launch(st, nwin, WarRowsHiTask{d_pows, d_hi, d_rows, w});
    launch(st, (long long)nwin * nh, WarRowsLoTask{d_pows, d_hi, d_rows, w});
    sync(st);
  } else {
    launch(st, nwin, WarRowsTask{d_pows, d_rows, w});
  }
  {
    const int ch = norm_chunk_for((long long)count, 5);
    launch(st, ((long long)count + ch - 1) / ch, WarNormTask{d_rows, out.tab, nullptr, nullptr, (int)count, ch});
  }
  sync(st);
}
#else
void build_tom_tab(zka_ctx* ctx, const uint32_t* base_aff_dev, FixedTable& out) {
  Stream& st = ctx->st;
  const int w = ctx->tom_w, nwin = ctx->tom_nwin;
  const size_t ne = (size_t)fb_entries(w), count = (size_t)nwin * ne;
  DevBuf pows, rows;
  uint32_t* d_pows = pows.get<uint32_t>((size_t)nwin * 36);
  uint32_t* d_rows = rows.get<uint32_t>(count * TOM_PROJ_WORDS);
  out.tab = out.buf.get<uint32_t>(count * TOM_PRE_WORDS);
  launch(st, 1, TomPowsTask{base_aff_dev, d_pows, 1, nwin, w});
  if (w > 9) {
    DevBuf hi;
    const int nh = 1 << (w - 9);
    uint32_t* d_hi = hi.get<uint32_t>((size_t)nwin * nh * 36);
    launch(st, nwin, TomRowsHiTask{d_pows, d_hi, d_rows, w});
    launch(st, (long long)nwin * nh, TomRowsLoTask{d_pows, d_hi, d_rows, w});
    sync(st);
  } else {
    launch(st, nwin, TomRowsTask{d_pows, d_rows, w});
  }
  launch(st, (long long)(count + 15) / 16, TomTabE2Task{d_rows, out.tab, (int)count});
  sync(st);
}

#endif

template <class T>
const T* stage_in(Stream& st, DevBuf& buf, const T* p, size_t count) {
  if (!p || count == 0) return p;
  if (is_device_ptr(p)) return p;
  T* d = buf.get<T>(count);
  copy_h2d(st, d, p, count * sizeof(T));
  return d;
}

template <class T>
struct Output {
  T* dst;
  size_t width;
  bool dev;
  Output(T* p, size_t width) : dst(p), width(width), dev(is_device_ptr(p)) {}
  T* rows(DevBuf& stage, uint32_t b0, size_t rows) const { return dev ? dst + b0 * width : stage.get<T>(rows * width); }
  void copy_back(Stream& st, uint32_t b0, const T* d, size_t rows) const {
    if (!dev) copy_d2h(st, dst + b0 * width, d, rows * width * sizeof(T));
  }
  void copy_back_2d(Stream& st, uint32_t b0, const T* d, size_t rows, size_t bytes) const {
    if (!dev) copy_d2h_2d(st, dst + b0 * width, width * sizeof(T), d, width * sizeof(T), bytes, rows);
  }
};

std::vector<uint32_t> chunk_schedule(uint32_t B, uint32_t cmax, int lanes, bool taper) {
  std::vector<uint32_t> off{0};
  auto r32 = [](uint32_t v) { return v < 32 ? std::max<uint32_t>(v, 1) : ((v + 31) & ~31u); };
  if (lanes > 1) {
    uint32_t per = r32((B + (uint32_t)lanes - 1) / (uint32_t)lanes);
    cmax = std::min(cmax, std::max<uint32_t>(per, 256));
  }
  uint32_t done = 0;
  auto push = [&](uint32_t n) { n = std::min(n, B - done); if (n) { done += n; off.push_back(done); } };
  if (taper && cmax >= 1024 && B >= 3 * cmax) {
    const uint32_t q = r32(cmax / 4), h = r32(cmax / 2);
    push(q);
    push(h);
    const uint32_t mid = B - done - (h + q);
    const uint32_t nm = (mid + cmax - 1) / cmax;
    const uint32_t each = r32((mid + nm - 1) / nm);
    for (uint32_t i = 0; i + 1 < nm; i++) push(each);
    push(B - done - (h + q));
    push(h);
    push(q);
  } else {
    const uint32_t nk = (B + cmax - 1) / cmax;
    const uint32_t each = r32((B + nk - 1) / nk);
    while (done < B) push(each);
  }
  return off;
}

#if !defined(ZKA_HOSTSIM)
void CUDART_CB progress_cb(void* p) { *reinterpret_cast<volatile uint32_t*>(p) = 1u; }
void notify_progress(Stream& st, volatile uint32_t* flag) { ZK_CUDA_CHECK(cudaLaunchHostFunc(st.s, progress_cb, (void*)flag)); }
#else
void notify_progress(Stream&, volatile uint32_t* flag) { *flag = 1u; }
#endif

template <class Fn>
void run_lanes(zka_ctx* ctx, int used, Fn fn) {
  if (used <= 1) { fn(0); return; }
  std::vector<std::thread> th;
  std::vector<std::exception_ptr> errs((size_t)used);
  for (int li = 1; li < used; li++)
    th.emplace_back([&, li] {
      try {
#if !defined(ZKA_HOSTSIM)
        ZK_CUDA_CHECK(cudaSetDevice(ctx->device));
#endif
        fn(li);
      } catch (...) {
        errs[(size_t)li] = std::current_exception();
      }
    });
  try { fn(0); } catch (...) { errs[0] = std::current_exception(); }
  for (auto& t : th) t.join();
  for (auto& e : errs)
// ... 28 lines not shown
    skip(v.s_in, 32); skip(v.q_in, 65); skip(v.seeds, 32); skip(v.tape, tape_stride);
    skip(v.proofs, proof_stride); skip(v.proof_len, 1); skip(v.status, 1);
    return v;
  }
};
struct VerifyRows {
  const uint8_t *msg_hash{}, *proofs{}, *tape{}, *seeds{}, *q_ext{};
  const uint32_t *proof_len{}, *ring_of{};
  size_t proof_stride{}, tape_stride{};
  uint8_t* ok{}; int32_t* status{};
  VerifyRows() = default;
  VerifyRows(const uint8_t* proofs, size_t stride, const uint32_t* len, uint8_t* ok, int32_t* status)
      : proofs(proofs), proof_len(len), proof_stride(stride), ok(ok), status(status) {}
  VerifyRows at(size_t r0) const {
    VerifyRows v = *this;
    auto skip = [r0](auto*& p, size_t width) { if (p) p += r0 * width; };
    skip(v.msg_hash, 32); skip(v.proofs, proof_stride); skip(v.proof_len, 1); skip(v.tape, tape_stride); skip(v.seeds, 32);
    skip(v.ring_of, 1); skip(v.q_ext, NP); skip(v.ok, 1); skip(v.status, 1);
    return v;
  }
};

struct RingSrc {
  const uint8_t* ring; uint32_t N;
  const zka_rings* set; int n;
  static RingSrc one(const uint8_t* ring, uint32_t N) { return {ring, N, nullptr, ceil_log2(N)}; }
  static RingSrc pass(const zka_rings* set, int n) { return {nullptr, 0, set, n}; }
  static RingSrc none(int n) { return {nullptr, 2, nullptr, n}; }
  const uint32_t* prepare(zka_ctx* ctx, bool lagrange) const {
    if (!set && !ring) return nullptr;
    if (set) return (const uint32_t*)set->ring_m.p;
    const uint32_t* ring_m = prep_ring(ctx, ctx->st, ring, N, n, lagrange);
    sync(ctx->st);
    return ring_m;
  }
  template <class Ctx>
  void fill(Ctx& c, const uint32_t* ring_m, const uint32_t* ring_of) const {
    c.ring_m = ring_m;
    if (!set) return;
    c.ring_of = ring_of;
    c.ring_base = (const uint32_t*)set->ring_base.p;
    c.ring_depth = (const uint32_t*)set->ring_depth.p;
    if constexpr (std::is_same<Ctx, ProveCtx>::value) {
      c.ring_size = (const uint32_t*)set->ring_size.p;
      c.gk_lag = (uint32_t*)set->lag.p;
    }
  }
};

template <class Check, class Pass>
int ring_passes(zka_ctx* ctx, const RingSrc& ring, const uint32_t* ring_of, uint32_t B, Check check, Pass pass) {
  if (ring.set && ring.set->ctx != ctx) return fail(ctx, ZKA_E_ARG, "ring set of another context");
  if (B == 0) return 0;
  return guarded(ctx, [&] {
    if (!ring.set) {
      if (ring.N < 2 || ring.N > (1u << 20)) return fail(ctx, ZKA_E_ARG, "ring size must be in [2, 2^20]");
      const int rc = check(ring.n);
      return rc ? rc : pass(ring);
    }
    std::vector<uint32_t> h(B);
    if (is_device_ptr(ring_of)) {
      copy_d2h(ctx->st, h.data(), ring_of, (size_t)B * 4);
      sync(ctx->st);
    } else {
      memcpy(h.data(), ring_of, (size_t)B * 4);
    }
    const std::vector<int>& depth = ring.set->depth;
    int nmax = 0;
    for (uint32_t b = 0; b < B; b++) {
      if (h[b] >= ring.set->R) return fail(ctx, ZKA_E_ARG, "ring_of[i] >= number of rings in the set");
      nmax = std::max(nmax, depth[h[b]]);
    }
    const int rc = check(nmax);
    return rc ? rc : pass(RingSrc::pass(ring.set, nmax));
  });
}

int gk_blocks(int n) { return 1 << (n - gk_block_bits(n)); }

ProveCtx prove_ctx(const zka_ctx* ctx, const zka_params* P, int B, int S, int N, int n) {
  ProveCtx c;
  memset(&c, 0, sizeof(c));
  c.B = B; c.S = S; c.N = N; c.n = n;
  c.tom_w = ctx->tom_w; c.tom_nwin = ctx->tom_nwin;
  c.g_tab8 = ctx->g8.tab; c.h_tab8 = P->h8.tab; c.h_w = P->h_w;
  c.g_tabw = ctx->gw.tab; c.g_w = ctx->p256_hw;
  c.tg_tab = ctx->tg.tab; c.th_tab = P->th.tab;
  c.tg_bytes = (const uint8_t*)ctx->tg_bytes.p;
  c.gk_lag = (uint32_t*)ctx->lag.p;
  return c;
}
VerifyCtx verify_ctx(const zka_ctx* ctx, const zka_params* P, int B, int S, int N, int n, int K, int mode) {
  VerifyCtx c;
  memset(&c, 0, sizeof(c));
  c.B = B; c.S = S; c.N = N; c.n = n; c.K = K; c.mode = mode;
  c.tom_w = ctx->tom_w; c.tom_nwin = ctx->tom_nwin;
  c.g_tab8 = ctx->g8.tab; c.h_tab8 = P->h8.tab; c.h_w = P->h_w;
  c.tg_tab = ctx->tg.tab; c.th_tab = P->th.tab;
  c.tg_bytes = (const uint8_t*)ctx->tg_bytes.p;
  return c;
}

void prove_store1(Stream& st, const ProveCtx& c) {
  const long long n1 = (long long)c.B * (2 + 2 * c.S);
  launch(st, n1, JobsATask{c});
  launch(st, n1, TomCommitTask{c.s1_jv, c.s1_jr, c.tg_tab, c.th_tab, c.s1_proj, c.tom_w, c.tom_nwin});
  launch_tom_norm(st, c.s1_proj, c.s1_aff, c.s1_bytes, n1, 1);
}
void prove_items_gk(Stream& st, const ProveCtx& c, uint32_t* gext, bool items, bool gk) {
  const long long M = c.M, nj = M * JOBS_PER_ITEM, nd = M * DERS_PER_ITEM;
  const long long Bn = (long long)c.B * c.n, ng = 4 * Bn;
  const int nblk = gk_blocks(c.n);
  const size_t g0 = c.s2_gk(0, 0);
  if (items) {
    launch(st, (M + ITEM_INV_CHUNK - 1) / ITEM_INV_CHUNK, ItemInvTask{c});
    launch(st, M, ItemScalarsTask{c});
  }
  if (gk) {
    launch(st, Bn, GkJobsTask{c});
    launch(st, Bn * nblk, GkPolyTask{c});
    if (nblk > 1) launch(st, Bn, GkPolyReduceTask{c});
    launch(st, Bn, GkCdJobsTask{c});
  }
  if (items) {
    launch(st, M * GJOBS_PER_ITEM, TomCommitGTask{c.s2_jv, c.tg_tab, gext, c.tom_w, c.tom_nwin});
    launch(st, nj, TomCommitHTask{c.s2_jr, c.th_tab, gext, c.s2_proj, c.tom_w, c.tom_nwin});
  }
  if (gk)
    launch(st, ng, TomCommitTask{c.s2_jv + g0 * 8, c.s2_jr + g0 * 8, c.tg_tab, c.th_tab, c.s2_proj + g0 * TOM_E2_WORDS, c.tom_w,
                                 c.tom_nwin});
  if (items) {
    launch_tom_norm(st, c.s2_proj, c.s2_aff, c.s2_bytes, nj, 1, JOBS_PER_ITEM, 2);
    launch(st, M, DerivedTask{c});
    launch_tom_norm(st, c.s2_proj + nj * TOM_E2_WORDS, nullptr, c.s2_bytes + nj * BSTRIDE, nd, 0, 1, 1, TOM_E2_WORDS);
  }
  if (gk) launch_tom_norm(st, c.s2_proj + g0 * TOM_E2_WORDS, nullptr, c.s2_bytes + g0 * BSTRIDE, ng, 1);
  if (items) {
    launch(st, M * HASHES_PER_ITEM, ItemHashTask{c});
    launch(st, M * 7, ItemEmitTask{c});
  }
}
void verify_gk(Stream& st, const VerifyCtx& c, uint32_t* gk_offs) {
  const int nblk = gk_blocks(c.n), ngk = 4 * c.n + 1;
  if (nblk > 1) launch(st, (long long)c.B * nblk, VGkSumTask{c});
  launch(st, c.B, VGkTask{c});
  launch(st, (long long)c.B * ngk, VGkOffsetsTask{c, gk_offs});
}

}

extern "C" {

int zka_version(void) { return 1; }

const char* zka_last_error(const zka_ctx* ctx) { return ctx ? ctx->err.c_str() : "null context"; }

uint64_t zka_launch_count(const zka_ctx* ctx) {
  if (!ctx) return 0;
  uint64_t n = ctx->st.launches + ctx->aux[0].launches + ctx->aux[1].launches;
  for (const auto& l : ctx->extra) n += l->st.launches + l->aux[0].launches + l->aux[1].launches;
  return n;
}

void* zka_get_stream(zka_ctx* ctx) {
#if !defined(ZKA_HOSTSIM)
  return ctx ? (void*)ctx->st.s : nullptr;
#else
  return nullptr;
#endif
}
int zka_set_profiling(zka_ctx* ctx, int enable) {
  if (!ctx) return ZKA_E_ARG;
  try {
    for (int i = 0; i < 1 + (int)ctx->extra.size(); i++) { sync(ctx->lane(i).st); ctx->lane(i).st.profiling = enable != 0; }
  } catch (...) { return ZKA_E_CUDA; }
  return 0;
}
int zka_profile_reset(zka_ctx* ctx) {
  if (!ctx) return ZKA_E_ARG;
  try {
    for (int i = 0; i < 1 + (int)ctx->extra.size(); i++) { sync(ctx->lane(i).st); ctx->lane(i).st.prof.clear(); }
  } catch (...) { return ZKA_E_CUDA; }
  return 0;
}
int zka_set_option(zka_ctx* ctx, const char* key, long value) {
  if (!ctx || !key || value < 1) return ZKA_E_ARG;
  const std::string k(key);
  return guarded(ctx, [&]() -> int {
    if (k == "lanes") {
      if (value > 8) return ZKA_E_ARG;
      while ((int)ctx->extra.size() + 1 < value) {
        auto l = std::make_unique<Lane>();
        stream_create(l->st);
        stream_create(l->cs_in);
        stream_create(l->cs_out);
        stream_create(l->aux[0]);
        stream_create(l->aux[1]);
        l->st.profiling = ctx->st.profiling;
        ctx->extra.push_back(std::move(l));
      }
      ctx->nlanes = (int)value;
    } else if (k == "chunk") {
      ctx->chunk = (int)value;
    } else if (k == "host_chunk") {
      ctx->host_chunk = (int)value;
    } else if (k == "agg") {
      ctx->agg = (int)value - 1;
    } else if (k == "agg_c") {
      if (value < 4 || value > 16) return ZKA_E_ARG;
      ctx->agg_c = (int)value;
    } else {
      return ZKA_E_ARG;
    }
    return 0;
  });
}
long long zka_stat(zka_ctx* ctx, const char* key) {
  if (!ctx || !key) return -1;
  const std::string k(key);
  std::lock_guard<std::mutex> g(ctx->stat_mu);
  if (k == "agg_pass") return (long long)ctx->agg_pass;
  if (k == "agg_fail") return (long long)ctx->agg_fail;
  if (k == "agg_c") return (long long)ctx->agg_c_last;
  return -1;
}
size_t zka_profile_json(zka_ctx* ctx, char* buf, size_t cap) {
  if (!ctx) return 0;
  std::map<std::string, ProfEntry> all;
  try {
    for (int i = 0; i < 1 + (int)ctx->extra.size(); i++) {
      sync(ctx->lane(i).st);
      for (auto& kv : ctx->lane(i).st.prof) {
        ProfEntry& e = all[kv.first];
        e.launches += kv.second.launches; e.ms += kv.second.ms; e.items += kv.second.items;
      }
    }
  } catch (...) { return 0; }
  std::string j = "{";
  bool first = true;
  for (auto& kv : all) {
    char tmp[512];
    snprintf(tmp, sizeof tmp, "%s\"%s\": {\"launches\": %llu, \"ms\": %.6f, \"items\": %llu}", first ? "" : ", ",
             kv.first.c_str(), (unsigned long long)kv.second.launches, kv.second.ms,
             (unsigned long long)kv.second.items);
    j += tmp;
    first = false;
  }
  j += "}";
  if (buf && cap) {
    size_t n = std::min(cap - 1, j.size());
    memcpy(buf, j.data(), n);
    buf[n] = 0;
  }
  return j.size() + 1;
}
int zka_proof_group(char* name, size_t cap, int* point_bytes, int* scalar_bytes) {
#if defined(ZKA_PG_WAR256)
  const char* n = "war256";
#else
  const char* n = "tomEdwards256";
#endif
  if (name && cap) {
    strncpy(name, n, cap - 1);
    name[cap - 1] = 0;
  }
  if (point_bytes) *point_bytes = WP;
  if (scalar_bytes) *scalar_bytes = WS;
  return 0;
}
int zka_set_progress(zka_ctx* ctx, volatile uint32_t* flags, uint32_t cap) {
  if (!ctx) return ZKA_E_ARG;
  ctx->progress = flags;
  ctx->progress_cap = flags ? cap : 0;
  return 0;
}
int zka_chunk_schedule(zka_ctx* ctx, uint32_t B, int host_buffers, uint32_t* off, uint32_t cap) {
  if (!ctx || !off || cap == 0) return ZKA_E_ARG;
  const std::vector<uint32_t> v = chunk_schedule(B, (uint32_t)(host_buffers ? std::min(ctx->chunk, ctx->host_chunk) : ctx->chunk), ctx->nlanes,
                                                 host_buffers != 0);
  if (v.size() > cap) return ZKA_E_ARG;
  for (size_t i = 0; i < v.size(); i++) off[i] = v[i];
  return (int)v.size() - 1;
}
int zka_lanes(const zka_ctx* ctx) { return ctx ? ctx->nlanes : 0; }
int zka_config(const zka_ctx* ctx, int* tom_w, int* tom_nwin, int* chunk) {
  if (!ctx) return ZKA_E_ARG;
  if (tom_w) *tom_w = ctx->tom_w;
  if (tom_nwin) *tom_nwin = ctx->tom_nwin;
  if (chunk) *chunk = ctx->chunk;
  return 0;
}

int zka_init(int device, zka_ctx** out) {
  if (!out) return ZKA_E_ARG;
  *out = nullptr;
#if !defined(ZKA_HOSTSIM)
  int ndev = 0;
  cudaError_t e = cudaGetDeviceCount(&ndev);
  if (e != cudaSuccess || ndev == 0 || device >= ndev) {
    cudaGetLastError();
    return ZKA_E_CUDA;
  }
#endif
  std::unique_ptr<zka_ctx> ctx(new zka_ctx());
  const int rc = guarded(ctx.get(), [&] {
#if !defined(ZKA_HOSTSIM)
    ZK_CUDA_CHECK(cudaSetDevice(device));
    ZK_CUDA_CHECK(cudaStreamCreateWithFlags(&ctx->st.s, cudaStreamNonBlocking));
#endif
    ctx->device = device;
    if (const char* e = getenv("ZKA_TOM_W")) {
      int w = atoi(e);
      if (w >= 2 && w <= 24) ctx->tom_w = w;
    }
    ctx->tom_nwin = fb_windows(ctx->tom_w);
    if (const char* e = getenv("ZKA_CHUNK")) {
      int c = atoi(e);
      if (c >= 1) ctx->chunk = c;
    }
    if (const char* e = getenv("ZKA_NORM_MODEL")) g_norm_model = atoi(e) != 0;
#if !defined(ZKA_HOSTSIM)
    {
      int sms = 0;
      if (cudaDeviceGetAttribute(&sms, cudaDevAttrMultiProcessorCount, device) == cudaSuccess && sms > 0) g_norm_slots = sms * 4;
    }
#endif
    if (const char* e = getenv("ZKA_HOST_CHUNK")) {
      int c = atoi(e);
      if (c >= 1) ctx->host_chunk = c;
    }
    stream_create(ctx->cs_in);
    stream_create(ctx->cs_out);
    stream_create(ctx->aux[0]);
    stream_create(ctx->aux[1]);
    {
      int lanes = 3;
#if defined(ZKA_HOSTSIM)
      lanes = 1;
#endif
      if (const char* e = getenv("ZKA_LANES")) lanes = atoi(e);
      if (lanes < 1) lanes = 1;
      if (lanes > 8) lanes = 8;
      if (zka_set_option(ctx.get(), "lanes", lanes) != 0) throw std::runtime_error("lanes");
    }
    if (const char* e = getenv("ZKA_TAPE_SPLIT")) ctx->tape_split = atoi(e) != 0;
    if (const char* e = getenv("ZKA_AGG")) ctx->agg = atoi(e);
    if (const char* e = getenv("ZKA_AGG_C")) {
      int c = atoi(e);
      if (c >= 4 && c <= 16) ctx->agg_c = c;
    }
    if (const char* e = getenv("ZKA_P256_HW")) {
      int w = atoi(e);
      if (w >= 8 && w <= 24) ctx->p256_hw = w;
    }
    DevBuf gen;
    uint32_t* d_gen = gen.get<uint32_t>(16 + TOM_AFF_WORDS);
    launch(ctx->st, 1, GenAffTask{d_gen, d_gen + 16});
    build_p256_tab(ctx.get(), d_gen, ctx->g8, 8);
    build_p256_tab(ctx.get(), d_gen, ctx->gw, ctx->p256_hw);
    build_tom_tab(ctx.get(), d_gen + 16, ctx->tg);
    DevBuf proj, aff;
    uint32_t* d_proj = proj.get<uint32_t>(TOM_PROJ_WORDS);
    uint32_t* d_aff = aff.get<uint32_t>(TOM_AFF_WORDS);
    uint8_t* d_bytes = ctx->tg_bytes.get<uint8_t>(BSTRIDE);
    launch(ctx->st, 1, GProjTask{d_gen + 16, d_proj});
    launch_tom_norm(ctx->st, d_proj, d_aff, d_bytes, 1, 0);
    sync(ctx->st);
    return 0;
  });
  if (rc) {
    fprintf(stderr, "zka_init: %s\n", ctx->err.c_str());
    return rc;
  }
  *out = ctx.release();
  return 0;
}

void zka_shutdown(zka_ctx* ctx) { delete ctx; }

int zka_params_create(zka_ctx* ctx, const uint8_t h_nist[65], const uint8_t h_proof[67], uint32_t sec_level,
                      zka_params** out) {
  if (!ctx || !h_nist || !h_proof || !out) return ZKA_E_ARG;
  if (sec_level < 1 || sec_level > MAX_REPS) return fail(ctx, ZKA_E_ARG, "sec_level must be in [1,80]");
  return guarded(ctx, [&] {
    std::unique_ptr<zka_params> P(new zka_params());
    P->ctx = ctx;
    P->sec_level = sec_level;
    P->h_w = ctx->p256_hw;
    memcpy(P->h_nist, h_nist, 65);
    memcpy(P->h_proof, h_proof, WP);
    DevBuf bn, bt, an, at, bad, inf;
    uint8_t* d_bn = bn.get<uint8_t>(65);
    uint8_t* d_bt = bt.get<uint8_t>(WP);
    uint32_t* d_an = an.get<uint32_t>(16);
    uint32_t* d_at = at.get<uint32_t>(TOM_AFF_WORDS);
    uint8_t* d_bad = bad.get<uint8_t>(2);
    uint8_t* d_inf = inf.get<uint8_t>(1);
    copy_h2d(ctx->st, d_bn, h_nist, 65);
    copy_h2d(ctx->st, d_bt, h_proof, WP);
    launch(ctx->st, 1, ParsePointsTask{d_bn, nullptr, d_an, nullptr, d_bad, d_inf});
    launch(ctx->st, 1, ParsePointsTask{nullptr, d_bt, nullptr, d_at, d_bad + 1, nullptr});
    uint8_t hb[3];
    copy_d2h(ctx->st, hb, d_bad, 2);
    copy_d2h(ctx->st, hb + 2, d_inf, 1);
    sync(ctx->st);
    if (hb[0] || hb[1] || hb[2]) return fail(ctx, ZKA_E_ARG, "params: h point not on its group");
    build_p256_tab(ctx, d_an, P->h8, P->h_w);
    build_tom_tab(ctx, d_at, P->th);
    *out = P.release();
    return 0;
  });
}

void zka_params_destroy(zka_params* P) { delete P; }

int zka_rings_create(zka_ctx* ctx, uint32_t R, const uint32_t* sizes, const uint8_t* keys, zka_rings** out) {
  if (!ctx || !sizes || !keys || !out) return ZKA_E_ARG;
  *out = nullptr;
  if (R == 0) return fail(ctx, ZKA_E_ARG, "a ring set holds at least one ring");
  if (R > (1u << 23)) return fail(ctx, ZKA_E_ARG, "ring set exceeds 2^24 padded entries");
  std::unique_ptr<zka_rings> set(new zka_rings());
  set->ctx = ctx;
  set->R = R;
  std::vector<uint32_t> key_off(R), base(R);
  uint64_t nkeys = 0, total = 0;
  for (uint32_t r = 0; r < R; r++) {
    const uint32_t N = sizes[r];
    if (N < 2 || N > (1u << 20)) return fail(ctx, ZKA_E_ARG, "ring size must be in [2, 2^20]");
    const int n = ceil_log2(N);
    set->size.push_back(N);
    set->depth.push_back(n);
    key_off[r] = (uint32_t)nkeys;
    base[r] = (uint32_t)total;
    nkeys += N;
    total += 1ull << n;
    if (total > (1ull << 24)) return fail(ctx, ZKA_E_ARG, "ring set exceeds 2^24 padded entries");
  }
  return guarded(ctx, [&] {
    Stream& st = ctx->st;
    DevBuf kbuf, obuf;
    const uint8_t* d_keys = stage_in(st, kbuf, keys, (size_t)nkeys * 32);
    uint32_t* d_off = obuf.get<uint32_t>(R);
    uint32_t* d_base = set->ring_base.get<uint32_t>(R);
    uint32_t* d_size = set->ring_size.get<uint32_t>(R);
    uint32_t* d_depth = set->ring_depth.get<uint32_t>(R);
    const std::vector<uint32_t> depth(set->depth.begin(), set->depth.end());
    const int nmax = *std::max_element(set->depth.begin(), set->depth.end());
    uint32_t* ring_m = set->ring_m.get<uint32_t>((size_t)total * 8);
    copy_h2d(st, d_off, key_off.data(), (size_t)R * 4);
    copy_h2d(st, d_base, base.data(), (size_t)R * 4);
    copy_h2d(st, d_size, set->size.data(), (size_t)R * 4);
    copy_h2d(st, d_depth, depth.data(), (size_t)R * 4);
    launch(st, (long long)total, RingSetPrepTask{d_keys, d_off, d_base, d_size, ring_m, (int)R});
    launch(st, nmax, GkLagrangeSetTask{set->lag.get<uint32_t>(ProveCtx::gk_lag_off(nmax + 1))});
    sync(st);
    *out = set.release();
    return 0;
  });
}

void zka_rings_destroy(zka_rings* set) { delete set; }

size_t zka_proof_max_len(uint32_t ring_size, uint32_t sec_level) {
  return (size_t)proof_len((int)sec_level, ceil_log2(ring_size), (int)sec_level);
}
size_t zka_prove_tape_len(uint32_t ring_size, uint32_t sec_level) {
  return (size_t)32 * prove_draws((int)sec_level, ceil_log2(ring_size), (int)sec_level);
}
size_t zka_verify_tape_len(uint32_t ring_size, uint32_t sec_level) {
  return verify_tape_len(ceil_log2(ring_size), (int)sec_level);
}

int zka_tom_commit_batch(zka_ctx* ctx, const zka_params* P, uint32_t count, const uint8_t* v, const uint8_t* r,
                         uint8_t* out) {
  if (!ctx || !P || !v || !r || !out) return ZKA_E_ARG;
  if (count == 0) return 0;
  return guarded(ctx, [&] {
    Stream& st = ctx->st;
    Cursor in(ctx->in[0]), w(ctx->w), ob(ctx->out[0]);
    const uint8_t* dv = stage_in(st, in.next(), v, (size_t)count * 32);
    const uint8_t* dr = stage_in(st, in.next(), r, (size_t)count * 32);
    uint32_t* jv = w.take<uint32_t>((size_t)count * 8);
    uint32_t* jr = w.take<uint32_t>((size_t)count * 8);
    uint32_t* proj = w.take<uint32_t>((size_t)count * TOM_E2_WORDS);
    uint32_t* aff = w.take<uint32_t>((size_t)count * TOM_AFF_WORDS);
    uint8_t* bytes = w.take<uint8_t>((size_t)count * BSTRIDE);
    const Output<uint8_t> o(out, WP);
    uint8_t* packed = o.rows(ob.next(), 0, count);
    launch(st, count, CommitConvTask{dv, dr, jv, jr});
    launch(st, count, TomCommitTask{jv, jr, ctx->tg.tab, P->th.tab, proj, ctx->tom_w, ctx->tom_nwin});
    launch_tom_norm(st, proj, aff, bytes, (long long)(count), 1);
    launch(st, count, PackTomTask{bytes, packed});
    o.copy_back(st, 0, packed, count);
    sync(st);
    return 0;
  });
}

int zka_p256_mul_batch(zka_ctx* ctx, uint32_t count, const uint8_t* base, const uint8_t* k, uint8_t* out) {
  if (!ctx || !k || !out) return ZKA_E_ARG;
  if (count == 0) return 0;
  return guarded(ctx, [&] {
    Stream& st = ctx->st;
    Cursor in(ctx->in[0]), w(ctx->w), ob(ctx->out[0]);
    const uint8_t* dk = stage_in(st, in.next(), k, (size_t)count * 32);
    const uint8_t* db = stage_in(st, in.next(), base, (size_t)count * 65);
    uint32_t* proj = w.take<uint32_t>((size_t)count * P256_PROJ_WORDS);
    uint32_t* aff = w.take<uint32_t>((size_t)count * P256_AFF_WORDS);
    uint8_t* bytes = w.take<uint8_t>((size_t)count * BSTRIDE);
    uint8_t* inf = w.take<uint8_t>(count);
    const bool per_base = db != nullptr;
    uint32_t* baff = w.take_if<uint32_t>(per_base, (size_t)count * 16);
    uint8_t* bad = w.take_if<uint8_t>(per_base, count);
    uint8_t* binf = w.take_if<uint8_t>(per_base, count);
    uint32_t* pows = w.take_if<uint32_t>(per_base, (size_t)count * RT_NWIN * P256_PROJ_WORDS);
    uint32_t* rows = w.take_if<uint32_t>(per_base, (size_t)count * RT_ENTRIES * P256_PROJ_WORDS);
    uint32_t* rtab = w.take_if<uint32_t>(per_base, (size_t)count * RT_ENTRIES * P256_AFF_WORDS);
    const Output<uint8_t> o(out, NP);
    uint8_t* packed = o.rows(ob.next(), 0, count);
    if (per_base) {
      launch(st, count, ParsePointsTask{db, nullptr, baff, nullptr, bad, binf});
      launch(st, count, P256PowsTask{baff, binf, pows, (int)count, RT_NWIN, RT_W});
      launch(st, (long long)count * RT_NWIN, P256RowsSignedTask{pows, rows});
      const long long np = (long long)count * RT_ENTRIES;
      launch_p256_norm(st, rows, rtab, nullptr, nullptr, (long long)(np));
    }
    launch(st, count, P256MulTask{dk, ctx->g8.tab, rtab, binf, proj});
    launch_p256_norm(st, proj, aff, bytes, inf, (long long)(count));
    launch(st, count, PackP256Task{bytes, packed});
    o.copy_back(st, 0, packed, count);
    sync(st);
    return 0;
  });
}


int zka_field_op_batch(zka_ctx* ctx, int field, int op, uint32_t count, const uint8_t* a, const uint8_t* b,
                       uint8_t* out) {
  if (!ctx || !a || !out || field < 0 || field > 2 || op < 0 || op > 4 || (op < 3 && !b)) return ZKA_E_ARG;
  if (count == 0) return 0;
  return guarded(ctx, [&] {
    Stream& st = ctx->st;
    Cursor in(ctx->in[0]), ob(ctx->out[0]);
    const int nb = field == 2 ? WCB : 32;
    const uint8_t* da = stage_in(st, in.next(), a, (size_t)count * nb);
    const uint8_t* db = stage_in(st, in.next(), b, (size_t)count * nb);
    const Output<uint8_t> o(out, nb);
    uint8_t* dout = o.rows(ob.next(), 0, count);
    if (field == 0) launch(st, count, FieldOpTask<P256p, 32>{da, db, dout, op});
    else if (field == 1) launch(st, count, FieldOpTask<P256n, 32>{da, db, dout, op});
    else launch(st, count, FieldOpTask<PGp, WCB>{da, db, dout, op});
    o.copy_back(st, 0, dout, count);
    sync(st);
    return 0;
  });
}

int zka_hash80_batch(zka_ctx* ctx, uint32_t count, const uint8_t* msgs, size_t msg_stride, const uint32_t* len,
                     uint8_t* out) {
  if (!ctx || !msgs || !len || !out) return ZKA_E_ARG;
  if (count == 0) return 0;
  return guarded(ctx, [&] {
    Stream& st = ctx->st;
    Cursor in(ctx->in[0]), ob(ctx->out[0]);
    const uint8_t* dm = stage_in(st, in.next(), msgs, (size_t)count * msg_stride);
    const uint32_t* dl = stage_in(st, in.next(), len, (size_t)count);
    const Output<uint8_t> o(out, 10);
    uint8_t* dout = o.rows(ob.next(), 0, count);
    launch(st, count, Hash80Task{dm, msg_stride, dl, dout});
    o.copy_back(st, 0, dout, count);
    sync(st);
    return 0;
  });
}

int zka_params_generate(zka_ctx* ctx, const uint8_t rnd[64], uint8_t h_nist[65], uint8_t h_proof[67]) {
  if (!ctx || !rnd || !h_nist || !h_proof) return ZKA_E_ARG;
  return guarded(ctx, [&] {
    int rc = zka_p256_mul_batch(ctx, 1, nullptr, rnd, h_nist);
    if (rc) return rc;
    Stream& st = ctx->st;
    Cursor in(ctx->in[0]), w(ctx->w);
    uint32_t* jv = w.take<uint32_t>(8);
    uint32_t* jr = w.take<uint32_t>(8);
    uint32_t* proj = w.take<uint32_t>(TOM_E2_WORDS);
    uint32_t* aff = w.take<uint32_t>(TOM_AFF_WORDS);
    uint8_t* bytes = w.take<uint8_t>(BSTRIDE);
    uint8_t* d_rnd = in.take<uint8_t>(32);
    copy_h2d(st, d_rnd, rnd + 32, 32);
    launch(st, 1, GenConvTask{d_rnd, jv, jr});
    launch(st, 1, TomCommitTask{jv, jr, ctx->tg.tab, ctx->tg.tab, proj, ctx->tom_w, ctx->tom_nwin});
    launch_tom_norm(st, proj, aff, bytes, (long long)(1), 1);
    copy_d2h(st, h_proof, bytes, WP);
    sync(st);
    return 0;
  });
}

int zka_key_to_int(zka_ctx* ctx, uint32_t count, const uint8_t* pk, uint8_t* x_out, int32_t* status) {
  if (!ctx || !pk || !x_out) return ZKA_E_ARG;
  if (count == 0) return 0;
  return guarded(ctx, [&] {
    Stream& st = ctx->st;
    Cursor in(ctx->in[0]), w(ctx->w), ob(ctx->out[0]);
    const uint8_t* dp = stage_in(st, in.next(), pk, (size_t)count * 65);
    uint32_t* aff = w.take<uint32_t>((size_t)count * 16);
    uint8_t* bad = w.take<uint8_t>(count);
    uint8_t* inf = w.take<uint8_t>(count);
    const Output<uint8_t> xo(x_out, 32);
    const Output<int32_t> so(status, 1);
    uint8_t* dx = xo.rows(ob.next(), 0, count);
    int32_t* ds = so.rows(ob.next(), 0, count);
    launch(st, count, ParsePointsTask{dp, nullptr, aff, nullptr, bad, inf});
    launch(st, count, KeyToIntTask{aff, bad, inf, dx, ds});
    xo.copy_back(st, 0, dx, count);
    if (status) so.copy_back(st, 0, ds, count);
    sync(st);
    return 0;
  });
}

static int prove_impl(zka_ctx* ctx, const zka_params* P, uint32_t B, const ProveRows& rows, const RingSrc& ring, int mode) {
  const int S = (int)P->sec_level, n = ring.n;
  const bool seeded = rows.seeds != nullptr;
  const int seed_draws = prove_draws(S, n, S);
  const uint32_t* ring_m = ring.prepare(ctx, true);
  const Output<uint8_t> po(rows.proofs, rows.proof_stride);
  const Output<uint32_t> lo(rows.proof_len, 1);
  const Output<int32_t> so(rows.status, 1);
  const int lanes = ctx->nlanes;
  const size_t dev_tape_stride = (rows.tape_stride + 15) & ~(size_t)15;
  const bool all_dev = po.dev && is_device_ptr(seeded ? rows.seeds : rows.tape);
  const std::vector<uint32_t> off = chunk_schedule(B, (uint32_t)(all_dev ? ctx->chunk : std::min(ctx->chunk, ctx->host_chunk)), lanes, !all_dev);
  const uint32_t nchunks = (uint32_t)off.size() - 1;
  const int used = (int)std::min<uint32_t>((uint32_t)lanes, nchunks);
  const bool trace = getenv("ZKA_TRACE") != nullptr;
  const auto t_call = std::chrono::steady_clock::now();
  auto ms_now = [&] { return std::chrono::duration<double, std::milli>(std::chrono::steady_clock::now() - t_call).count(); };
  std::atomic<uint32_t> next_chunk((uint32_t)used);
  auto run_lane = [&](int li) {
    Lane& ln = ctx->lane(li);
    Stream& st = ln.st;
    ProveRows cin[2];
    auto issue_inputs = [&](uint32_t k, int slot) {
      const ProveRows r = rows.at(off[k]), e = rows.at(off[k + 1]);
      const size_t Bc = off[k + 1] - off[k];
      Stream& ci = ln.cs_in;
      Cursor in(ln.in[slot]);
      DevBuf& tape_buf = in.next();
      auto stage = [&](auto* p, auto* end) { return stage_in(ci, in.next(), p, (size_t)(end - p)); };
      ev_wait(ci, ln.ev_done[slot]);
      ProveRows& d = cin[slot];
      d.msg_hash = stage(r.msg_hash, e.msg_hash);
      d.sig = stage(r.sig, e.sig);
      d.pk = stage(r.pk, e.pk);
      d.which = stage(r.which, e.which);
      d.ring_of = stage(r.ring_of, e.ring_of);
      d.base = stage(r.base, e.base);
      d.s_in = stage(r.s_in, e.s_in);
      d.q_in = stage(r.q_in, e.q_in);
      d.seeds = stage(r.seeds, e.seeds);
      ev_record(ln.ev_small[slot], ci);
      if (seeded) {
        d.tape = tape_buf.get<uint8_t>(Bc * (size_t)32 * seed_draws);
      } else if (is_device_ptr(rows.tape)) {
        d.tape = r.tape;
      } else if (!ctx->tape_split && dev_tape_stride == rows.tape_stride) {
        d.tape = stage_in(ci, tape_buf, r.tape, (size_t)(e.tape - r.tape));
      } else {
        uint8_t* dt = tape_buf.get<uint8_t>(Bc * dev_tape_stride);
        const size_t width = ctx->tape_split ? std::min(rows.tape_stride, (size_t)32 * draws_before_items(S)) : rows.tape_stride;
        copy_d2h_2d(ci, dt, dev_tape_stride, r.tape, rows.tape_stride, width, Bc);
        d.tape = dt;
      }
// ... 261 lines not shown

int zka_prove_membership_batch(zka_ctx* ctx, const zka_params* P, uint32_t B, const uint8_t* com_r, const uint32_t* index,
                               const uint8_t* ring, uint32_t N, const uint8_t* tape, size_t tape_stride, uint8_t* proofs,
                               size_t proof_stride, uint32_t* proof_len, int32_t* status) {
  if (!ctx || !P || !com_r || !index || !ring || !tape || !proofs || !proof_len || !status) return ZKA_E_ARG;
  if (B == 0) return 0;
  if (N < 2 || N > (1u << 20)) return fail(ctx, ZKA_E_ARG, "ring size must be in [2, 2^20]");
  const int n = ceil_log2(N);
  if (proof_stride < (size_t)gk_len(n)) return fail(ctx, ZKA_E_ARG, "proof_stride < GK block length");
  if (tape_stride < (size_t)32 * 5 * n) return fail(ctx, ZKA_E_ARG, "tape_stride < 32 * 5n");
  return guarded(ctx, [&] {
    Stream& st = ctx->st;
    const uint32_t* ring_m = prep_ring(ctx, st, ring, N, n, true);
    const Output<uint8_t> po(proofs, proof_stride);
    const Output<uint32_t> lo(proof_len, 1);
    const Output<int32_t> so(status, 1);
    const size_t it_len = 96 + tape_stride, it_stride = (it_len + 15) & ~(size_t)15;
    const uint32_t chunk = 8192;
    for (uint32_t b0 = 0; b0 < B; b0 += chunk) {
      const int Bc = (int)std::min<uint32_t>(chunk, B - b0);
      Cursor in(ctx->in[0]), w(ctx->w), ob(ctx->out[0]);
      const uint8_t* d_cr = stage_in(st, in.next(), com_r + (size_t)b0 * 32, (size_t)Bc * 32);
      const uint32_t* d_idx = stage_in(st, in.next(), index + b0, (size_t)Bc);
      const uint8_t* d_tape = stage_in(st, in.next(), tape + (size_t)b0 * tape_stride, (size_t)Bc * tape_stride);
      ProveCtx c = prove_ctx(ctx, P, Bc, 0, (int)N, n);
      c.which = d_idx;
      c.ring_m = ring_m;
      uint8_t* itape = w.take<uint8_t>((size_t)Bc * it_stride);
      c.tape = itape; c.tape_stride = it_stride; c.tape_draws = (uint32_t)(it_len / 32);
      c.which_s = w.take<uint32_t>(Bc);
      c.zcount = w.take<uint32_t>(Bc);
      c.gk_off = w.take<uint32_t>(Bc);
      c.gk_dv = w.take<uint32_t>((size_t)Bc * n * 8);
      c.gk_x = w.take<uint32_t>((size_t)Bc * 3);
      const size_t ng = (size_t)Bc * 4 * n;
      c.s2_jv = w.take<uint32_t>(ng * 8);
      c.s2_jr = w.take<uint32_t>(ng * 8);
      c.s2_proj = w.take<uint32_t>(ng * TOM_E2_WORDS);
      c.s2_bytes = w.take<uint8_t>(ng * BSTRIDE);
      c.gk_part = w.take_if<uint32_t>(gk_blocks(n) > 1, (size_t)Bc * n * gk_blocks(n) * 8);
      c.proof_stride = proof_stride;
      c.proofs = po.rows(ob.next(), b0, Bc);
      c.proof_len = lo.rows(ob.next(), b0, Bc);
      c.status = so.rows(ob.next(), b0, Bc);
      launch(st, Bc, GkAloneSetupTask{c, d_cr, d_tape, tape_stride, itape});
      prove_items_gk(st, c, nullptr, false, true);
      launch(st, Bc, GkEmitTask{c});
      launch(st, (long long)Bc * FIN_PARTS, FinalizeTask{c});
      po.copy_back_2d(st, b0, c.proofs, Bc, (size_t)gk_len(n));
      lo.copy_back(st, b0, c.proof_len, Bc);
      so.copy_back(st, b0, c.status, Bc);
      sync(st);
    }
    return 0;
  });
}

static int prove_sub(zka_ctx* ctx, const zka_params* P, int kind, uint32_t B, const uint8_t* scalars, const uint8_t* tape,
                     size_t tape_stride, uint8_t* commitments, uint8_t* proofs, int32_t* status) {
  if (!ctx || !P || !scalars || !tape || !commitments || !proofs || !status) return ZKA_E_ARG;
  if (B == 0) return 0;
  const int ns = kind == 0 ? 3 : 6, nd = kind == 0 ? 3 : 7, J = kind == 0 ? SUBP_EQ_JOBS : SUBP_MULT_JOBS;
  const int nc = kind == 0 ? 2 : 3, plen = kind == 0 ? EQ_LEN : MULT_LEN;
  if (tape_stride < (size_t)32 * nd) return fail(ctx, ZKA_E_ARG, "tape_stride too small for this sub-proof");
  return guarded(ctx, [&] {
    Stream& st = ctx->st;
    const Output<uint8_t> co(commitments, (size_t)nc * WP), po(proofs, plen);
    const Output<int32_t> so(status, 1);
    const uint32_t chunk = 16384;
    for (uint32_t b0 = 0; b0 < B; b0 += chunk) {
      const int Bc = (int)std::min<uint32_t>(chunk, B - b0);
      Cursor in(ctx->in[0]), w(ctx->w), ob(ctx->out[0]);
      const uint8_t* d_sc = stage_in(st, in.next(), scalars + (size_t)b0 * ns * 32, (size_t)Bc * ns * 32);
      const uint8_t* d_tape = stage_in(st, in.next(), tape + (size_t)b0 * tape_stride, (size_t)Bc * tape_stride);
      const size_t nj = (size_t)Bc * J;
      uint32_t* jv = w.take<uint32_t>(nj * 8);
      uint32_t* jr = w.take<uint32_t>(nj * 8);
      uint32_t* proj = w.take<uint32_t>(nj * TOM_E2_WORDS);
      uint8_t* bytes = w.take<uint8_t>(nj * BSTRIDE);
      uint8_t* d_com = co.rows(ob.next(), b0, Bc);
      uint8_t* d_prf = po.rows(ob.next(), b0, Bc);
      int32_t* d_st = so.rows(ob.next(), b0, Bc);
      launch(st, Bc, SubProveJobsTask{kind, d_sc, d_tape, tape_stride, jv, jr, d_st});
      launch(st, (long long)nj, TomCommitTask{jv, jr, ctx->tg.tab, P->th.tab, proj, ctx->tom_w, ctx->tom_nwin});
      launch_tom_norm(st, proj, nullptr, bytes, (long long)nj, 1);
      launch(st, Bc, SubProveEmitTask{kind, d_sc, d_tape, tape_stride, jr, bytes, d_com, d_prf, d_st});
      co.copy_back(st, b0, d_com, Bc);
      po.copy_back(st, b0, d_prf, Bc);
      so.copy_back(st, b0, d_st, Bc);
      sync(st);
    }
    return 0;
  });
}
int zka_prove_equality_batch(zka_ctx* ctx, const zka_params* P, uint32_t B, const uint8_t* scalars, const uint8_t* tape,
                             size_t tape_stride, uint8_t* commitments, uint8_t* proofs, int32_t* status) {
  return prove_sub(ctx, P, 0, B, scalars, tape, tape_stride, commitments, proofs, status);
}
int zka_prove_mult_batch(zka_ctx* ctx, const zka_params* P, uint32_t B, const uint8_t* scalars, const uint8_t* tape,
                         size_t tape_stride, uint8_t* commitments, uint8_t* proofs, int32_t* status) {
  return prove_sub(ctx, P, 1, B, scalars, tape, tape_stride, commitments, proofs, status);
}

int zka_prove_pointadd_batch(zka_ctx* ctx, const zka_params* P, uint32_t B, const uint8_t* points, const uint8_t* blinders,
                             const uint8_t* tape, size_t tape_stride, uint8_t* commitments, uint8_t* proofs, int32_t* status) {
  if (!ctx || !P || !points || !blinders || !tape || !commitments || !proofs || !status) return ZKA_E_ARG;
  if (B == 0) return 0;
  if (tape_stride < (size_t)32 * 38) return fail(ctx, ZKA_E_ARG, "tape_stride < 32 * 38");
  return guarded(ctx, [&] {
    Stream& st = ctx->st;
    const size_t it_stride = (size_t)32 * (9 + 38);
    const size_t row_stride = REP0_LEN;
    const Output<uint8_t> co(commitments, 6 * WP), po(proofs, PA_LEN);
    const Output<int32_t> so(status, 1);
    const uint32_t chunk = 8192;
    for (uint32_t b0 = 0; b0 < B; b0 += chunk) {
      const int Bc = (int)std::min<uint32_t>(chunk, B - b0);
      Cursor in(ctx->in[0]), w(ctx->w), ob(ctx->out[0]);
      const uint8_t* d_pts = stage_in(st, in.next(), points + (size_t)b0 * 195, (size_t)Bc * 195);
      const uint8_t* d_bl = stage_in(st, in.next(), blinders + (size_t)b0 * 192, (size_t)Bc * 192);
      const uint8_t* d_tape = stage_in(st, in.next(), tape + (size_t)b0 * tape_stride, (size_t)Bc * tape_stride);
      ProveCtx c = prove_ctx(ctx, P, Bc, 1, 2, 0);
      c.M = Bc; c.mode = 1; c.head_len = 0;
      uint8_t* itape = w.take<uint8_t>((size_t)Bc * it_stride);
      c.tape = itape; c.tape_stride = it_stride; c.tape_draws = (uint32_t)(it_stride / 32);
      const size_t n1 = (size_t)Bc * 4, n2 = (size_t)Bc * (JOBS_PER_ITEM + DERS_PER_ITEM);
      c.s1 = w.take<uint32_t>((size_t)Bc * 8);
      c.pk_aff = w.take<uint32_t>((size_t)Bc * 16);
      c.pa_T_aff = w.take<uint32_t>((size_t)Bc * 2 * 16);
      c.pa_T_inf = w.take<uint8_t>((size_t)Bc * 2);
      c.pa_A_inf = w.take<uint8_t>((size_t)Bc * 2);
      c.pb_T1_aff = w.take<uint32_t>((size_t)Bc * 16);
      c.pb_T1_inf = w.take<uint8_t>(Bc);
      c.chal = w.take<uint32_t>((size_t)Bc * 3);
      c.zcount = w.take<uint32_t>(Bc);
      c.item_base = w.take<uint32_t>(Bc);
      c.item_b = w.take<uint32_t>(Bc);
      c.item_i = w.take<uint32_t>(Bc);
      c.item_k = w.take<uint32_t>(Bc);
      c.rep_off = w.take<uint32_t>(Bc);
      c.s1_jv = w.take<uint32_t>(n1 * 8);
      c.s1_jr = w.take<uint32_t>(n1 * 8);
      c.s1_proj = w.take<uint32_t>(n1 * TOM_E2_WORDS);
      c.s1_aff = w.take<uint32_t>(n1 * TOM_AFF_WORDS);
      c.s1_bytes = w.take<uint8_t>(n1 * BSTRIDE);
      c.s2_jv = w.take<uint32_t>(n2 * 8);
      c.s2_jr = w.take<uint32_t>(n2 * 8);
      c.s2_proj = w.take<uint32_t>(n2 * TOM_E2_WORDS);
      c.s2_aff = w.take<uint32_t>(n2 * TOM_AFF_WORDS);
      c.s2_bytes = w.take<uint8_t>(n2 * BSTRIDE);
      c.secrets = w.take<uint32_t>((size_t)Bc * SECRETS_PER_ITEM * 8);
      c.item_inv = w.take<uint32_t>((size_t)Bc * 8);
      c.item_chal = w.take<uint32_t>((size_t)Bc * HASHES_PER_ITEM * 3);
      uint32_t* gext = w.take<uint32_t>((size_t)Bc * GJOBS_PER_ITEM * TOM_EXT_WORDS);
      c.proof_stride = row_stride;
      c.proofs = w.take<uint8_t>((size_t)Bc * row_stride);
      c.proof_len = w.take<uint32_t>(Bc);
      uint8_t* d_com = co.rows(ob.next(), b0, Bc);
      uint8_t* d_prf = po.rows(ob.next(), b0, Bc);
      c.status = so.rows(ob.next(), b0, Bc);
      launch(st, Bc, PaddSetupTask{c, d_pts, d_bl, d_tape, tape_stride, itape});
      prove_store1(st, c);
      prove_items_gk(st, c, gext, true, false);
      launch(st, Bc, PaddExtractTask{c, d_com, d_prf});
      co.copy_back(st, b0, d_com, Bc);
      po.copy_back(st, b0, d_prf, Bc);
      so.copy_back(st, b0, c.status, Bc);
// ... 79 lines not shown
    c.tape_stride = seeded ? seed_stride : rows.tape_stride;
    ring.fill(c, ring_m, cur.ring_of);
    if (seeded) {
      const SeedVerifyTapeTask vt{cur.seeds, const_cast<uint8_t*>(cur.tape), seed_stride, n, S, K, c.ring_of, c.ring_depth};
      launch(st, (long long)Bc * vt.slots(), vt);
    }
    double t_in = 0.0;
    if (trace) { sync(st); t_in = ms_now(); }
    const size_t ns = (size_t)Bc * K;
    const int ET = c.ent_tom(), EN = c.ent_nist(), SG = c.segs();
    const int ngk = 4 * n + 1;
    Cursor w(ln.w);
    c.rep_off = w.take<uint32_t>((size_t)Bc * S);
    c.gk_off = w.take<uint32_t>(Bc);
    c.tagbits = w.take<uint32_t>((size_t)Bc * 3);
    c.chal = w.take<uint32_t>((size_t)Bc * 3);
    c.gk_ok_len = w.take<uint8_t>(Bc);
    c.r_aff = w.take<uint32_t>((size_t)Bc * 16);
    c.q_aff = w.take<uint32_t>((size_t)Bc * 16);
    c.q_inf = w.take<uint8_t>(Bc);
    c.rpows = w.take<uint32_t>((size_t)Bc * RT_NWIN * P256_PROJ_WORDS);
    c.rrows = w.take<uint32_t>((size_t)Bc * RT_ENTRIES * P256_PROJ_WORDS);
    c.rtab = w.take<uint32_t>((size_t)Bc * RT_ENTRIES * P256_AFF_WORDS);
    c.samp_idx = w.take<uint32_t>(ns);
    c.samp_draw = w.take<uint32_t>(ns);
    c.sp_T = w.take<uint32_t>(ns * P256_PROJ_WORDS);
    c.sp_T_aff = w.take<uint32_t>(ns * 16);
    c.sp_T_inf = w.take<uint8_t>(ns);
    c.ta_jv = w.take<uint32_t>(ns * 2 * 8);
    c.ta_jr = w.take<uint32_t>(ns * 2 * 8);
    c.ta_proj = w.take<uint32_t>(ns * 2 * TOM_E2_WORDS);
    c.ta_aff = w.take<uint32_t>(ns * 2 * TOM_AFF_WORDS);
    c.td_proj = w.take<uint32_t>(ns * DERS_PER_ITEM * TOM_PROJ_WORDS);
    c.td_aff = w.take<uint32_t>(ns * DERS_PER_ITEM * TOM_AFF_WORDS);
    c.td_bytes = w.take<uint8_t>(ns * DERS_PER_ITEM * BSTRIDE);
    c.item_chal = w.take<uint32_t>(ns * HASHES_PER_ITEM * 3);
    c.ent_scalar = w.take<uint32_t>((size_t)Bc * ET * 8);
    c.ent_off = w.take<uint32_t>((size_t)Bc * ET);
    c.ent_pre = w.take<uint32_t>((size_t)Bc * ET * TOM_PRE_WORDS);
    c.ent_cnt = w.take<uint32_t>(ns);
    c.part = w.take<uint32_t>(ns * V_PART_WORDS);
    c.fx_jv = w.take<uint32_t>((size_t)Bc * 2 * 8);
    c.fx_jr = w.take<uint32_t>((size_t)Bc * 2 * 8);
    c.fx_proj = w.take<uint32_t>((size_t)Bc * 2 * TOM_PROJ_WORDS);
    c.nfix = w.take<uint32_t>((size_t)Bc * P256_PROJ_WORDS);
    c.id_flags = w.take<uint8_t>((size_t)Bc * 3);
    c.gk_tape_bad = w.take_if<uint8_t>(mode == 0, Bc);
    c.nent_scalar = w.take<uint32_t>((size_t)Bc * EN * 8);
    c.nent_aff = w.take<uint32_t>((size_t)Bc * EN * 16);
    c.nent_skip = w.take<uint8_t>((size_t)Bc * EN);
    c.gk_scalar = w.take<uint32_t>((size_t)Bc * ngk * 8);
    c.gk_pre = w.take<uint32_t>((size_t)Bc * ngk * TOM_PRE_WORDS);
    uint32_t* gk_offs = w.take<uint32_t>((size_t)Bc * ngk);
    c.win_w = w.take<uint32_t>((size_t)Bc * SG * MSM_NWIN * 36);
    c.win_g = w.take<uint32_t>((size_t)Bc * MSM_NWIN * 36);
    c.win_n = w.take<uint32_t>((size_t)Bc * MSM_NWIN_N * P256_PROJ_WORDS);
    c.gk_part = w.take_if<uint32_t>(gk_blocks(n) > 1, (size_t)Bc * gk_blocks(n) * 8);
    Cursor ob(ln.out[0]);
    c.ok = oo.rows(ob.next(), b0, Bc);
    c.status = so.rows(ob.next(), b0, Bc);

    launch(st, Bc, VLayoutTask{c});
    launch(st, (long long)Bc * (S + 1), VValidateTask{c});
    {
      const bool fork = !st.profiling;
      Stream& sr = fork ? ln.aux[0] : st;
      if (fork) { ev_record(ln.ev_fork, st); ev_wait(sr, ln.ev_fork); }
      launch(sr, Bc, P256PowsTask{c.r_aff, nullptr, c.rpows, Bc, RT_NWIN, RT_W});
      launch(sr, (long long)Bc * RT_NWIN, P256RowsSignedTask{c.rpows, c.rrows});
      launch_p256_norm(sr, c.rrows, c.rtab, nullptr, nullptr, (long long)Bc * RT_ENTRIES);
      launch(st, Bc, VChallengeTask{c});
      if (fork) { ev_record(ln.ev_join[0], sr); ev_wait(st, ln.ev_join[0]); }
    }
    const bool gk_fork = mode == 0 && !st.profiling;
    if (gk_fork) {
      ev_record(ln.ev_fork, st);
      ev_wait(ln.aux[1], ln.ev_fork);
      verify_gk(ln.aux[1], c, gk_offs);
      ev_record(ln.ev_join[1], ln.aux[1]);
    }
    launch(st, (long long)ns, VSampleP256Task{c});
    launch_p256_norm(st, c.sp_T, c.sp_T_aff, nullptr, c.sp_T_inf, (long long)(ns));
    launch(st, (long long)ns, VSampleJobsTask{c});
    launch(st, (long long)ns * 2, TomCommitTask{c.ta_jv, c.ta_jr, c.tg_tab, c.th_tab, c.ta_proj, c.tom_w, c.tom_nwin});
    launch_tom_norm(st, c.ta_proj, c.ta_aff, nullptr, (long long)(ns * 2), 1);
    launch(st, (long long)ns, VDerivedTask{c});
    launch_tom_norm(st, c.td_proj, nullptr, c.td_bytes, (long long)(ns * DERS_PER_ITEM), 0);
    launch(st, (long long)ns * HASHES_PER_ITEM, VItemHashTask{c});
    dev_memset(st, c.ent_off, 0, (size_t)Bc * ET * 4);
    launch(st, (long long)ns, VRelationsTask{c});
    if (mode == 0) {
      if (gk_fork) ev_wait(st, ln.ev_join[1]);
      else verify_gk(st, c, gk_offs);
    }
    launch(st, Bc, VReduceTask{c});
    launch(st, (long long)Bc * ET, VParseEntriesTask{c.proofs, c.proof_stride, c.ent_off, c.ent_pre, ET});
    if (mode == 0) launch(st, (long long)Bc * ngk, VParseEntriesTask{c.proofs, c.proof_stride, gk_offs, c.gk_pre, ngk});
    launch(st, (long long)Bc * 2, TomCommitTask{c.fx_jv, c.fx_jr, c.tg_tab, c.th_tab, c.fx_proj, c.tom_w, c.tom_nwin, 1});
    uint32_t* ctl = nullptr;
    if (ctx->agg && mode == 0) {
      Cursor A(ln.agg);
      const int fgroups = (Bc * 2 + 63) / 64, ngroups = (Bc + 31) / 32, ngroups2 = (ngroups + 31) / 32;
      ctl = A.take<uint32_t>(AGG_CTL_WORDS);
#if !defined(ZKA_PG_WAR256)
      uint32_t* tpart = A.take<uint32_t>((size_t)Bc * (K + 1) * 2 * PG_EXT_WORDS);
#endif
      uint32_t* fpart = A.take<uint32_t>((size_t)fgroups * 16);
      uint32_t* fjv = A.take<uint32_t>(8);
      uint32_t* fjr = A.take<uint32_t>(8);
      uint32_t* fproj = A.take<uint32_t>(TOM_PROJ_WORDS);
      uint32_t* npart = A.take<uint32_t>((size_t)ngroups * P256_PROJ_WORDS);
      uint32_t* npart2 = A.take_if<uint32_t>(ngroups > 32, (size_t)ngroups2 * P256_PROJ_WORDS);
      dev_memset(st, ctl, 0, AGG_CTL_WORDS * 4);
      launch(st, Bc, AggGateTask{c, ctl});
      const AggTomSrc tsrc{c.ent_scalar, c.ent_pre, c.ent_cnt, c.gk_scalar, c.gk_pre, Bc, ET, K, ngk};
      const AggNistSrc nsrc{c.nent_scalar, c.nent_aff, c.nent_skip, Bc, EN};
      const bool fork = !st.profiling;
      Stream& sa = fork ? ln.aux[0] : st;
      Stream& sb = fork ? ln.aux[1] : st;
      if (fork) {
        ev_record(ln.ev_fork, st);
        ev_wait(sa, ln.ev_fork);
        ev_wait(sb, ln.ev_fork);
      }
#if !defined(ZKA_PG_WAR256)
      launch(sa, (long long)Bc * (K + 1) * 2, AggTorsionPartTask{tsrc, ctl, tpart});
      launch(sa, Bc, AggTorsionTask{tpart, ctl, K});
#endif
      const AggPlan tp = agg_plan((double)Bc * (0.5 * K * V_ENT_PER_SAMPLE + 2 + ngk), ctx->agg_c);
      const AggPlan np = agg_plan((double)Bc * EN, 0);
      ctx->agg_c_last = tp.D.c;
      const uint32_t *tA, *tB, *nA, *nB;
      agg_msm(st, Cursor(ln.agg_tom), tsrc, tp, ctl, &tA, &tB);
      agg_msm(sb, Cursor(ln.agg_nist), nsrc, np, ctl, &nA, &nB);
      launch(st, fgroups, AggFixPartTask{ctl, c.fx_jv, c.fx_jr, fpart, Bc});
      launch(st, 1, AggFixSumTask{ctl, fpart, fjv, fjr, fgroups});
      launch(st, 1, TomCommitTask{fjv, fjr, c.tg_tab, c.th_tab, fproj, c.tom_w, c.tom_nwin, 1});
      launch(sb, ngroups, AggNistFixPartTask{ctl, c.nfix, npart, Bc});
      int nleft = ngroups;
      const uint32_t* nsum = npart;
      if (nleft > 32) {
        launch(sb, ngroups2, AggNistFixPartTask{ctl, npart, npart2, nleft});
        nsum = npart2;
        nleft = ngroups2;
      }
      if (fork) {
        ev_record(ln.ev_join[0], sa);
        ev_record(ln.ev_join[1], sb);
        ev_wait(st, ln.ev_join[0]);
        ev_wait(st, ln.ev_join[1]);
      }
      launch(st, 33, AggFinalTask{ctl, tA, tB, fproj, tp.D.nwin, tp.D.c, nA, nB, nsum, np.D.nwin, np.D.c, nleft});
      c.agg_ctl = ctl;
    }
    {
      const int nW = Bc * SG * MSM_NWIN, nWp = (nW + 31) & ~31, nG = Bc * MSM_NWIN;
      launch(st, (long long)nWp + nG,
             MsmTomWindowBothTask{MsmTomWindowTask{c.ent_scalar, c.ent_pre, c.ent_cnt, ET, K, V_ENT_PER_SAMPLE, 2, V_SEG, SG, c.win_w},
                                  MsmTomWindowTask{c.gk_scalar, c.gk_pre, nullptr, ngk, 0, 0, mode == 0 ? ngk : 0, V_SEG, 1, c.win_g}, nW, nWp, nG, ctl});
    }
    launch(st, (long long)Bc * MSM_NWIN_N, MsmP256WindowTask{c.nent_scalar, c.nent_aff, c.nent_skip, c.win_n, EN, ctl});
    {
      const int Bp = (Bc + 31) & ~31;
      launch(st, 3ll * Bp, MsmCombineAllTask{MsmTomCombineTask{c.win_g, c.fx_proj, c.id_flags, 2, 0, 0},
                                             MsmTomCombineTask{c.win_w, c.fx_proj, c.id_flags, 2, 1, 1, SG},
                                             MsmP256CombineTask{c.win_n, c.nfix, c.id_flags}, Bc, Bp, ctl});
    }
    launch(st, Bc, VFinalTask{c});
    oo.copy_back(st, b0, c.ok, Bc);
    so.copy_back(st, b0, c.status, Bc);
    uint32_t hctl[AGG_CTL_WORDS] = {0, 0, 0, 0};
    if (ctl) copy_d2h(st, hctl, ctl, sizeof(hctl));
    const double t_enq = trace ? ms_now() : 0.0;
    sync(st);
    if (trace)
      fprintf(stderr, "VTRACE lane %d chunk %u rows %d begin %.2f inputs_on_device %.2f enqueued %.2f done %.2f\n", li, k, Bc, t_begin, t_in,
              t_enq, ms_now());
    if (ctl) {
      std::lock_guard<std::mutex> g(ctx->stat_mu);
      if (hctl[AGG_TOM_PASS] && hctl[AGG_NIST_PASS]) ctx->agg_pass++;
      else ctx->agg_fail++;
    }
    if (kn >= nchunks) break;
    k = kn;
    cur = nxt;
    slot ^= 1;
  }
  };
  run_lanes(ctx, used, run_lane);
  sync(ctx->cs_in);
  return 0;
}

static int verify_batch(zka_ctx* ctx, const zka_params* P, uint32_t B, const VerifyRows& rows, const RingSrc& ring,
                        uint32_t samples, int mode) {
  if (!ctx || !P || !rows.proofs || !rows.proof_len || (!rows.tape && !rows.seeds) || !rows.ok || !rows.status) return ZKA_E_ARG;
  if (mode == 0 && (!rows.msg_hash || !(ring.set ? (const void*)rows.ring_of : ring.ring))) return ZKA_E_ARG;
  const int S = (int)P->sec_level, K = (int)samples;
  auto check = [&](int n) {
    if (K < 1) return fail(ctx, ZKA_E_ARG, "samples must be >= 1");
    if (S < K) return fail(ctx, ZKA_E_ARG, "security level not achieved");
    if (rows.tape && rows.tape_stride < (mode == 1 ? (size_t)V_IDX_PAD + (size_t)32 * 25 * K : verify_tape_len(n, S, K)))
      return fail(ctx, ZKA_E_ARG, "tape_stride < zka_verify_tape_len");
    return 0;
  };
  return ring_passes(ctx, ring, rows.ring_of, B, check, [&](const RingSrc& pass) { return verify_impl(ctx, P, B, rows, pass, samples, mode); });
}

int zka_verify_batch(zka_ctx* ctx, const zka_params* P, uint32_t B, const uint8_t* msg_hash, const uint8_t* ring,
                     uint32_t N, const uint8_t* proofs, size_t proof_stride, const uint32_t* proof_len,
                     const uint8_t* tape, size_t tape_stride, uint8_t* ok, int32_t* status) {
  return zka_verify_batch_ex(ctx, P, B, msg_hash, ring, N, proofs, proof_stride, proof_len, tape, tape_stride, ok, status, V_SAMPLES);
}

int zka_verify_batch_ex(zka_ctx* ctx, const zka_params* P, uint32_t B, const uint8_t* msg_hash, const uint8_t* ring,
                        uint32_t N, const uint8_t* proofs, size_t proof_stride, const uint32_t* proof_len,
                        const uint8_t* tape, size_t tape_stride, uint8_t* ok, int32_t* status, uint32_t samples) {
  VerifyRows r(proofs, proof_stride, proof_len, ok, status);
  r.msg_hash = msg_hash; r.tape = tape; r.tape_stride = tape_stride;
  return verify_batch(ctx, P, B, r, RingSrc::one(ring, N), samples, 0);
// ... 23 lines not shown
  return verify_batch(ctx, P, B, r, RingSrc::pass(rings, 0), samples, 0);
}

int zka_verify_exp_batch(zka_ctx* ctx, const zka_params* P, uint32_t B, const uint8_t* base, const uint8_t* com,
                         const uint8_t* px, const uint8_t* py, const uint8_t* q, const uint8_t* proofs, size_t proof_stride,
                         const uint32_t* proof_len, const uint8_t* tape, size_t tape_stride, uint32_t samples, uint8_t* ok,
                         int32_t* status) {
  if (!ctx || !P || !base || !com || !px || !py || !proofs || !proof_len || !tape || !ok || !status || proof_stride == 0) return ZKA_E_ARG;
  if (B == 0) return 0;
  return guarded(ctx, [&] {
    Stream& st = ctx->st;
    DevBuf bufs[10];
    Cursor in(bufs);
    const uint8_t* d_base = stage_in(st, in.next(), base, (size_t)B * NP);
    const uint8_t* d_com = stage_in(st, in.next(), com, (size_t)B * NP);
    const uint8_t* d_px = stage_in(st, in.next(), px, (size_t)B * WP);
    const uint8_t* d_py = stage_in(st, in.next(), py, (size_t)B * WP);
    const uint8_t* d_q = stage_in(st, in.next(), q, (size_t)B * NP);
    const uint8_t* d_body = stage_in(st, in.next(), proofs, (size_t)B * proof_stride);
    const uint32_t* d_len = stage_in(st, in.next(), proof_len, (size_t)B);
    const uint8_t* d_tape = stage_in(st, in.next(), tape, (size_t)B * tape_stride);
    const size_t row_stride = (HEAD_LEN + proof_stride + 15) & ~(size_t)15;
    uint8_t* d_rows = in.take<uint8_t>((size_t)B * row_stride);
    uint32_t* d_rlen = in.take<uint32_t>(B);
    const int pieces = (int)((row_stride + 63) / 64);
    launch(st, (long long)B * pieces, VAssembleTask{d_base, d_com, d_px, d_py, d_body, proof_stride, d_len, d_rows, row_stride, d_rlen, pieces});
    sync(st);
    VerifyRows r(d_rows, row_stride, d_rlen, ok, status);
    r.tape = d_tape; r.tape_stride = tape_stride; r.q_ext = d_q;
    return verify_batch(ctx, P, B, r, RingSrc::none(1), samples, 1);
  });
}

int zka_verify_membership_batch(zka_ctx* ctx, const zka_params* P, uint32_t B, const uint8_t* com, const uint8_t* ring, uint32_t N,
                                const uint8_t* proofs, size_t proof_stride, const uint32_t* proof_len, const uint8_t* tape,
                                size_t tape_stride, uint8_t* ok, int32_t* status) {
  if (!ctx || !P || !com || !ring || !proofs || !proof_len || !tape || !ok || !status || proof_stride == 0) return ZKA_E_ARG;
  if (B == 0) return 0;
  if (N < 2 || N > (1u << 20)) return fail(ctx, ZKA_E_ARG, "ring size must be in [2, 2^20]");
  const int n = ceil_log2(N);
  if (tape_stride < (size_t)32 * (2 * n + 1)) return fail(ctx, ZKA_E_ARG, "tape_stride < 32 * (2n + 1)");
  return guarded(ctx, [&] {
    Stream& st = ctx->st;
    DevBuf bufs[4];
    const uint32_t* ring_m = prep_ring(ctx, st, ring, N, n, false);
    const Output<uint8_t> oo(ok, 1);
    const Output<int32_t> so(status, 1);
    const size_t row_stride = (HEAD_LEN + proof_stride + 15) & ~(size_t)15;
    const int pieces = (int)((row_stride + 63) / 64);
    const int ngk = 4 * n + 1;
    const uint32_t chunk = 4096;
    for (uint32_t b0 = 0; b0 < B; b0 += chunk) {
      const int Bc = (int)std::min<uint32_t>(chunk, B - b0);
      Cursor in(bufs), w(ctx->w), ob(ctx->out[0]);
      const uint8_t* d_com = stage_in(st, in.next(), com + (size_t)b0 * WP, (size_t)Bc * WP);
      const uint8_t* d_body = stage_in(st, in.next(), proofs + (size_t)b0 * proof_stride, (size_t)Bc * proof_stride);
      const uint32_t* d_len = stage_in(st, in.next(), proof_len + b0, (size_t)Bc);
      VerifyCtx c = verify_ctx(ctx, P, Bc, (int)P->sec_level, (int)N, n, 1, 2);
      c.tape = stage_in(st, in.next(), tape + (size_t)b0 * tape_stride, (size_t)Bc * tape_stride);
      c.tape_stride = tape_stride;
      c.ring_m = ring_m;
      uint8_t* d_rows = w.take<uint8_t>((size_t)Bc * row_stride);
      uint32_t* d_rlen = w.take<uint32_t>(Bc);
      c.proofs = d_rows; c.proof_stride = row_stride; c.proof_len = d_rlen;
      c.gk_off = w.take<uint32_t>(Bc);
      c.gk_ok_len = w.take<uint8_t>(Bc);
      c.gk_scalar = w.take<uint32_t>((size_t)Bc * ngk * 8);
      c.gk_pre = w.take<uint32_t>((size_t)Bc * ngk * TOM_PRE_WORDS);
      uint32_t* gk_offs = w.take<uint32_t>((size_t)Bc * ngk);
      c.fx_jv = w.take<uint32_t>((size_t)Bc * 2 * 8);
      c.fx_jr = w.take<uint32_t>((size_t)Bc * 2 * 8);
      c.fx_proj = w.take<uint32_t>((size_t)Bc * 2 * TOM_PROJ_WORDS);
      c.win_g = w.take<uint32_t>((size_t)Bc * MSM_NWIN * 36);
      c.id_flags = w.take<uint8_t>((size_t)Bc * 3);
      c.gk_part = w.take_if<uint32_t>(gk_blocks(n) > 1, (size_t)Bc * gk_blocks(n) * 8);
      c.ok = oo.rows(ob.next(), b0, Bc);
      c.status = so.rows(ob.next(), b0, Bc);
      launch(st, (long long)Bc * pieces, VAssembleTask{nullptr, nullptr, d_com, nullptr, d_body, proof_stride, d_len, d_rows, row_stride, d_rlen, pieces});
      launch(st, Bc, VGkOnlyLayoutTask{c});
      dev_memset(st, c.fx_jv, 0, (size_t)Bc * 2 * 8 * 4);
      dev_memset(st, c.fx_jr, 0, (size_t)Bc * 2 * 8 * 4);
      verify_gk(st, c, gk_offs);
      launch(st, (long long)Bc * ngk, VParseEntriesTask{c.proofs, row_stride, gk_offs, c.gk_pre, ngk});
      launch(st, (long long)Bc * 2, TomCommitTask{c.fx_jv, c.fx_jr, c.tg_tab, c.th_tab, c.fx_proj, c.tom_w, c.tom_nwin, 1});
      launch(st, (long long)Bc * MSM_NWIN, MsmTomWindowTask{c.gk_scalar, c.gk_pre, nullptr, ngk, 0, 0, ngk, V_SEG, 1, c.win_g});
      launch(st, Bc, MsmTomCombineTask{c.win_g, c.fx_proj, c.id_flags, 2, 0, 0});
      launch(st, Bc, VGkOnlyFinalTask{c});
      oo.copy_back(st, b0, c.ok, Bc);
      so.copy_back(st, b0, c.status, Bc);
      sync(st);
    }
    return 0;
  });
}

static int verify_sub(zka_ctx* ctx, const zka_params* P, int kind, uint32_t B, const uint8_t* points, const uint8_t* proofs,
                      const uint8_t* tape, size_t tape_stride, uint8_t* ok, int32_t* status) {
  if (!ctx || !P || !points || !proofs || !tape || !ok || !status) return ZKA_E_ARG;
  if (B == 0) return 0;
  if (tape_stride < (size_t)32 * sub_draws(kind)) return fail(ctx, ZKA_E_ARG, "tape_stride too small for this sub-proof");
  return guarded(ctx, [&] {
    Stream& st = ctx->st;
    const int la = sub_points(kind) * WP, lc = sub_proof_len(kind), ne = sub_entries(kind);
    const size_t stride = (size_t)(la + lc + 15) & ~(size_t)15;
    const Output<uint8_t> oo(ok, 1);
    const Output<int32_t> so(status, 1);
    const uint32_t chunk = 8192;
    for (uint32_t b0 = 0; b0 < B; b0 += chunk) {
      const int Bc = (int)std::min<uint32_t>(chunk, B - b0);
      Cursor in(ctx->in[0]), w(ctx->w), ob(ctx->out[0]);
      const uint8_t* d_pts = stage_in(st, in.next(), points + (size_t)b0 * la, (size_t)Bc * la);
      const uint8_t* d_prf = stage_in(st, in.next(), proofs + (size_t)b0 * lc, (size_t)Bc * lc);
      const uint8_t* d_tape = stage_in(st, in.next(), tape + (size_t)b0 * tape_stride, (size_t)Bc * tape_stride);
      uint8_t* rows = w.take<uint8_t>((size_t)Bc * stride);
      uint32_t* ent_scalar = w.take<uint32_t>((size_t)Bc * SUB_ENT_MAX * 8);
      uint32_t* ent_off = w.take<uint32_t>((size_t)Bc * SUB_ENT_MAX);
      uint32_t* ent_pre = w.take<uint32_t>((size_t)Bc * SUB_ENT_MAX * TOM_PRE_WORDS);
      uint32_t* fx_jv = w.take<uint32_t>((size_t)Bc * 2 * 8);
      uint32_t* fx_jr = w.take<uint32_t>((size_t)Bc * 2 * 8);
      uint32_t* fx_proj = w.take<uint32_t>((size_t)Bc * 2 * TOM_PROJ_WORDS);
      uint32_t* win = w.take<uint32_t>((size_t)Bc * MSM_NWIN * 36);
      uint8_t* flags = w.take<uint8_t>((size_t)Bc * 3);
      uint8_t* d_ok = oo.rows(ob.next(), b0, Bc);
      int32_t* d_st = so.rows(ob.next(), b0, Bc);
      launch(st, (long long)Bc * (la + lc), VConcatTask{d_pts, d_prf, la, lc, rows, stride});
      launch(st, Bc, VSubProofTask{kind, rows, stride, d_tape, tape_stride, (const uint8_t*)ctx->tg_bytes.p, ent_scalar, ent_off,
                                   fx_jv, fx_jr, d_st, d_ok});
      launch(st, (long long)Bc * SUB_ENT_MAX, VParseEntriesTask{rows, stride, ent_off, ent_pre, SUB_ENT_MAX});
      launch(st, (long long)Bc * 2, TomCommitTask{fx_jv, fx_jr, ctx->tg.tab, P->th.tab, fx_proj, ctx->tom_w, ctx->tom_nwin, 1});
      launch(st, (long long)Bc * MSM_NWIN, MsmTomWindowTask{ent_scalar, ent_pre, nullptr, SUB_ENT_MAX, 0, 0, ne, V_SEG, 1, win});
      launch(st, Bc, MsmTomCombineTask{win, fx_proj, flags, 2, 1, 1});
      launch(st, Bc, VSubFinalTask{d_st, flags, d_ok});
      oo.copy_back(st, b0, d_ok, Bc);
      so.copy_back(st, b0, d_st, Bc);
      sync(st);
    }
    return 0;
  });
}
int zka_verify_equality_batch(zka_ctx* ctx, const zka_params* P, uint32_t B, const uint8_t* points, const uint8_t* proofs,
                              const uint8_t* tape, size_t tape_stride, uint8_t* ok, int32_t* status) {
  return verify_sub(ctx, P, SUB_EQ, B, points, proofs, tape, tape_stride, ok, status);
}
int zka_verify_mult_batch(zka_ctx* ctx, const zka_params* P, uint32_t B, const uint8_t* points, const uint8_t* proofs,
                          const uint8_t* tape, size_t tape_stride, uint8_t* ok, int32_t* status) {
  return verify_sub(ctx, P, SUB_MULT, B, points, proofs, tape, tape_stride, ok, status);
}
int zka_verify_pointadd_batch(zka_ctx* ctx, const zka_params* P, uint32_t B, const uint8_t* points, const uint8_t* proofs,
                              const uint8_t* tape, size_t tape_stride, uint8_t* ok, int32_t* status) {
  return verify_sub(ctx, P, SUB_PADD, B, points, proofs, tape, tape_stride, ok, status);
}

namespace {
int pack_common(zka_ctx* ctx, uint32_t B, uint8_t* rows, size_t stride, const uint32_t* len, uint8_t* packed, size_t cap,
                uint64_t* offsets, void* stream, int dir) {
  if (!ctx || !rows || !len || !packed || !offsets || stride == 0) return ZKA_E_ARG;
  if (B == 0) return 0;
#if !defined(ZKA_HOSTSIM)
  if (!is_device_ptr(rows) || !is_device_ptr(len) || !is_device_ptr(packed) || !is_device_ptr(offsets))
    return fail(ctx, ZKA_E_ARG, "zka_proofs_pack/unpack take device pointers");
#endif
  return guarded(ctx, [&] {
    Stream tmp;
    Stream* st = &ctx->st;
#if !defined(ZKA_HOSTSIM)
    if (stream) { tmp.s = (cudaStream_t)stream; st = &tmp; }
#endif
    const int pieces = (int)((stride + 15) / 16);
    launch(*st, 1, PackScanTask{len, offsets, (int)B});
    const bool al = (stride % 16 == 0) && (((size_t)rows | (size_t)packed) % 16 == 0);
    if (al) launch(*st, (long long)B * pieces, PackCopy16Task{rows, stride, len, offsets, packed, cap, pieces, dir});
    else launch(*st, (long long)B * pieces, PackCopyTask{rows, stride, len, offsets, packed, cap, pieces, dir});
    if (st == &tmp) ctx->st.launches += tmp.launches; else sync(*st);
    return 0;
  });
}
}

int zka_proofs_pack(zka_ctx* ctx, uint32_t B, const uint8_t* proofs, size_t proof_stride, const uint32_t* proof_len,
                    uint8_t* packed, size_t cap, uint64_t* offsets, void* stream) {
  return pack_common(ctx, B, const_cast<uint8_t*>(proofs), proof_stride, proof_len, packed, cap, offsets, stream, 0);
}
int zka_proofs_unpack(zka_ctx* ctx, uint32_t B, const uint8_t* packed, size_t cap, const uint32_t* proof_len, uint8_t* proofs,
                      size_t proof_stride, uint64_t* offsets, void* stream) {
  return pack_common(ctx, B, proofs, proof_stride, proof_len, const_cast<uint8_t*>(packed), cap, offsets, stream, 1);
}

}
```

Measured before the change: 112,400.

## Use mixed-width fixed-base windows to cut Pedersen commit lookups to eleven

Replaces the uniform 22-bit window fixed-base tables (12 windows) with a mixed-width shape, FbShape, where the top windows are one bit wider. This reaches 257 bits in 11 windows, so each Tom commit does fewer table lookups and point additions. Table construction, offsets and signed digit extraction are generalized to variable widths. If allocating the larger table fails, initialization falls back to 12 windows. In exchange the table needs more device memory and more startup build time, and random table gathers may suffer more cache misses.

```diff
diff --git a/__graft_entry__.py b/__graft_entry__.py
--- a/__graft_entry__.py
+++ b/__graft_entry__.py
@@ -20,6 +20,9 @@
 PROBE_SEED_SRC = os.path.join(ROOT, 'tests', 'probe', 'zk_probe_seed.cu')
 PROBE_SEED = os.path.join(ROOT, 'tests', 'probe', 'libzkprobe_seed.so')
 PROBE_SEED_HOST = os.path.join(ROOT, 'tests', 'probe', 'libzkprobe_seed_host.so')
+PROBE_SHAPE_SRC = os.path.join(ROOT, 'tests', 'probe', 'zk_probe_shape.cu')
+PROBE_SHAPE = os.path.join(ROOT, 'tests', 'probe', 'libzkprobe_shape.so')
+PROBE_SHAPE_HOST = os.path.join(ROOT, 'tests', 'probe', 'libzkprobe_shape_host.so')
 ORACLE_CPU = os.path.join(ROOT, 'oracle', '_ref', 'libzkattest_cpu.so')
 ARCH = ['-gencode', 'arch=compute_90a,code=sm_90a']
 NVCC_FLAGS = ARCH + ['-O3', '-std=c++17', '-lineinfo',
@@ -94,6 +97,16 @@
         cmd = [os.environ.get('NVCC', '/usr/local/cuda/bin/nvcc')] + NVCC_FLAGS
     cmd += ['-I' + os.path.join(ROOT, 'include'), '-I' + CSRC, '-o', out, PROBE_SEED_SRC]
     return _build_if_stale(out, cmd, 'probe_seed' + (' host (tests only)' if host else ' (sm_90a, tests only)'), [PROBE_SEED_SRC])
+
+
+def build_probe_shape(host=False):
+    out = PROBE_SHAPE_HOST if host else PROBE_SHAPE
+    if host:
+        cmd = ['g++', '-std=c++17', '-O2', '-DZKA_HOSTSIM', '-x', 'c++', '-fPIC', '-shared']
+    else:
+        cmd = [os.environ.get('NVCC', '/usr/local/cuda/bin/nvcc')] + NVCC_FLAGS
+    cmd += ['-I' + os.path.join(ROOT, 'include'), '-I' + CSRC, '-o', out, PROBE_SHAPE_SRC]
+    return _build_if_stale(out, cmd, 'probe_shape' + (' host (tests only)' if host else ' (sm_90a, tests only)'), [PROBE_SHAPE_SRC])
 
 
 def build_oracle_cpu():
@@ -125,7 +138,8 @@
     from concurrent.futures import ThreadPoolExecutor
     jobs = [build_lib, build_lib_war, build_hostsim, lambda: build_hostsim(war=True), build_oracle_cpu, build_tools,
             build_probe, lambda: build_probe(host=True), lambda: build_probe(jac=True),
-            lambda: build_probe(host=True, jac=True), build_probe_seed, lambda: build_probe_seed(host=True)]
+            lambda: build_probe(host=True, jac=True), build_probe_seed, lambda: build_probe_seed(host=True),
+            build_probe_shape, lambda: build_probe_shape(host=True)]
     with ThreadPoolExecutor(max_workers=min(len(jobs), max(1, (os.cpu_count() or 2)))) as ex:
         for f in [ex.submit(j) for j in jobs]:
             f.result()
diff --git a/zkp_ecdsa_b200/capi.py b/zkp_ecdsa_b200/capi.py
--- a/zkp_ecdsa_b200/capi.py
+++ b/zkp_ecdsa_b200/capi.py
@@ -202,7 +202,10 @@
         w, nw, ch = C.c_int(), C.c_int(), C.c_int()
         self._check(self.lib.zka_config(self.ctx, C.byref(w), C.byref(nw), C.byref(ch)), 'zka_config')
         lanes = int(self.lib.zka_lanes(self.ctx)) if hasattr(self.lib, 'zka_lanes') else 1
-        return {'tom_w': w.value, 'tom_nwin': nw.value, 'chunk': ch.value, 'lanes': lanes}
+        cfg = {'tom_w': w.value, 'tom_nwin': nw.value, 'chunk': ch.value, 'lanes': lanes}
+        if hasattr(self.lib, 'zka_stat') and self.stat('tom_n_lo') >= 0:
+            cfg.update(tom_n_lo=self.stat('tom_n_lo'), tom_fallback=bool(self.stat('tom_fallback')))
+        return cfg
 
     def set_option(self, key: str, value: int):
         self._check(self.lib.zka_set_option(self.ctx, key.encode(), int(value)), f'zka_set_option({key})')
diff --git a/zkp_ecdsa_b200/csrc/zk_launch.cuh b/zkp_ecdsa_b200/csrc/zk_launch.cuh
--- a/zkp_ecdsa_b200/csrc/zk_launch.cuh
+++ b/zkp_ecdsa_b200/csrc/zk_launch.cuh
@@ -192,15 +192,27 @@
   DevBuf(const DevBuf&) = delete;
   DevBuf& operator=(const DevBuf&) = delete;
   ~DevBuf() { dev_free(p); }
+  void release() {
+    dev_free(p);
+    p = nullptr;
+    cap = 0;
+  }
   template <class T>
   T* get(size_t count) {
     size_t bytes = count * sizeof(T);
     if (bytes > cap) {
-      dev_free(p);
+      release();
       size_t want = bytes + bytes / 8 + 256;
       p = dev_alloc(want);
       cap = want;
     }
+    return reinterpret_cast<T*>(p);
+  }
+  template <class T>
+  T* get_exact(size_t count) {
+    release();
+    p = dev_alloc(count * sizeof(T));
+    cap = count * sizeof(T);
     return reinterpret_cast<T*>(p);
   }
 };
diff --git a/zkp_ecdsa_b200/csrc/zk_ops.cuh b/zkp_ecdsa_b200/csrc/zk_ops.cuh
--- a/zkp_ecdsa_b200/csrc/zk_ops.cuh
+++ b/zkp_ecdsa_b200/csrc/zk_ops.cuh
@@ -203,14 +203,35 @@
 
 ZK_HD int fb_entries(int w) { return (1 << (w - 1)) + 1; }
 ZK_HD int fb_windows(int w) { return (256 + w) / w; }
-ZK_HD uint32_t signed_digit(const uint32_t* k, int j, int w, uint32_t& carry, bool& neg) {
-  const int pos = j * w;
+ZK_HD uint32_t signed_digit_at(const uint32_t* k, int pos, int w, uint32_t& carry, bool& neg) {
   uint32_t d = carry;
   if (pos < 256) d += digit_w(k, pos, (256 - pos) < w ? (256 - pos) : w);
   const uint32_t half = 1u << (w - 1);
   neg = d > half;
   carry = neg ? 1u : 0u;
   return neg ? (1u << w) - d : d;
+}
+ZK_HD uint32_t signed_digit(const uint32_t* k, int j, int w, uint32_t& carry, bool& neg) {
+  return signed_digit_at(k, j * w, w, carry, neg);
+}
+
+struct FbShape {
+  int w, nwin, n_lo;
+  ZK_HD int wide(int j) const { return j > n_lo ? j - n_lo : 0; }
+  ZK_HD int width(int j) const { return w + (j >= n_lo ? 1 : 0); }
+  ZK_HD int bitpos(int j) const { return j * w + wide(j); }
+  ZK_HD int bits() const { return bitpos(nwin); }
+  ZK_HD size_t entries(int j) const { return ((size_t)1 << (width(j) - 1)) + 1; }
+  ZK_HD size_t offset(int j) const { return (size_t)j * (size_t)fb_entries(w) + ((size_t)wide(j) << (w - 1)); }
+  ZK_HD size_t total() const { return offset(nwin); }
+};
+ZK_HD FbShape fb_uniform(int w) { return FbShape{w, fb_windows(w), fb_windows(w)}; }
+ZK_HD FbShape fb_lookups(int nwin) {
+  const int w = 257 / nwin;
+  return FbShape{w, nwin, nwin - (257 - w * nwin)};
+}
+ZK_HD uint32_t signed_digit(const uint32_t* k, int j, const FbShape& s, uint32_t& carry, bool& neg) {
+  return signed_digit_at(k, s.bitpos(j), s.width(j), carry, neg);
 }
 
 ZK_HD uint32_t bswap32(uint32_t x) {
@@ -325,73 +346,69 @@
 struct TomPowsTask {
   const uint32_t* base_aff;
   uint32_t* pows;
-  int nbase, nwin, w;
+  int nbase;
+  FbShape sh;
   ZK_HD void operator()(int t) const {
     uint32_t x[9], y[9];
     ld<9>(x, base_aff + (size_t)t * TOM_AFF_WORDS);
     ld<9>(y, base_aff + (size_t)t * TOM_AFF_WORDS + 9);
     TomPt p;
     tom_from_affine(p, x, y);
-    for (int j = 0; j < nwin; j++) {
-      uint32_t* o = pows + ((size_t)t * nwin + j) * 36;
+    for (int j = 0; j < sh.nwin; j++) {
+      uint32_t* o = pows + ((size_t)t * sh.nwin + j) * 36;
       st<9>(o, p.x); st<9>(o + 9, p.y); st<9>(o + 18, p.t); st<9>(o + 27, p.z);
-      for (int k = 0; k < w; k++) tom_dbl(p, p);
+      for (int k = 0; k < sh.width(j); k++) tom_dbl(p, p);
     }
   }
 };
 struct TomRowsTask {
-  const uint32_t* pows;
+  const uint32_t* pow;
   uint32_t* rows;
   int w;
-  ZK_HD void operator()(int t) const {
+  ZK_HD void operator()(int) const {
     TomPt p, acc;
-    const uint32_t* s = pows + (size_t)t * 36;
-    ld<9>(p.x, s); ld<9>(p.y, s + 9); ld<9>(p.t, s + 18); ld<9>(p.z, s + 27);
+    ld<9>(p.x, pow); ld<9>(p.y, pow + 9); ld<9>(p.t, pow + 18); ld<9>(p.z, pow + 27);
     tom_set_identity(acc);
     const int ne = fb_entries(w);
-    uint32_t* out = rows + (size_t)t * ne * TOM_PROJ_WORDS;
     for (int d = 0; d < ne; d++) {
-      uint32_t* o = out + (size_t)d * TOM_PROJ_WORDS;
+      uint32_t* o = rows + (size_t)d * TOM_PROJ_WORDS;
       tom_st_xyz(o, acc.x, acc.y, acc.z);
       tom_add(acc, acc, p);
     }
   }
 };
+ZK_HD size_t tom_hi_offset(const FbShape& sh, int j) { return ((sh.offset(j) - (size_t)j) >> 8) + (size_t)j; }
 struct TomRowsHiTask {
   const uint32_t* pows;
   uint32_t* hi;
-  uint32_t* rows;
-  int w;
+  FbShape sh;
   ZK_HD void operator()(int t) const {
     TomPt p, acc;
     const uint32_t* s = pows + (size_t)t * 36;
     ld<9>(p.x, s); ld<9>(p.y, s + 9); ld<9>(p.t, s + 18); ld<9>(p.z, s + 27);
     for (int k = 0; k < 8; k++) tom_dbl(p, p);
     tom_set_identity(acc);
-    const int nh = 1 << (w - 9);
-    for (int m = 0; m < nh; m++) {
-      uint32_t* o = hi + ((size_t)t * nh + m) * 36;
+    const int nh = 1 << (sh.width(t) - 9);
+    for (int m = 0; m <= nh; m++) {
+      uint32_t* o = hi + (tom_hi_offset(sh, t) + m) * 36;
       st<9>(o, acc.x); st<9>(o + 9, acc.y); st<9>(o + 18, acc.t); st<9>(o + 27, acc.z);
       tom_add(acc, acc, p);
     }
-    tom_st_xyz(rows + ((size_t)t * fb_entries(w) + ((size_t)1 << (w - 1))) * TOM_PROJ_WORDS, acc.x, acc.y, acc.z);
   }
 };
 struct TomRowsLoTask {
-  const uint32_t* pows;
+  const uint32_t* pow;
   const uint32_t* hi;
   uint32_t* rows;
-  int w;
-  ZK_HD void operator()(int t) const {
-    const int nh = 1 << (w - 9);
-    const int j = t / nh, m = t % nh;
+  int nh;
+  ZK_HD void operator()(int m) const {
     TomPt p, acc;
-    const uint32_t* s = pows + (size_t)j * 36;
-    ld<9>(p.x, s); ld<9>(p.y, s + 9); ld<9>(p.t, s + 18); ld<9>(p.z, s + 27);
-    const uint32_t* h = hi + (size_t)t * 36;
+    ld<9>(p.x, pow); ld<9>(p.y, pow + 9); ld<9>(p.t, pow + 18); ld<9>(p.z, pow + 27);
+    const uint32_t* h = hi + (size_t)m * 36;
     ld<9>(acc.x, h); ld<9>(acc.y, h + 9); ld<9>(acc.t, h + 18); ld<9>(acc.z, h + 27);
-    uint32_t* out = rows + ((size_t)j * fb_entries(w) + ((size_t)m << 8)) * TOM_PROJ_WORDS;
-    for (int d = 0; d < 256; d++) {
+    uint32_t* out = rows + ((size_t)m << 8) * TOM_PROJ_WORDS;
+    const int n = m < nh ? 256 : 1;
+    for (int d = 0; d < n; d++) {
       uint32_t* o = out + (size_t)d * TOM_PROJ_WORDS;
       tom_st_xyz(o, acc.x, acc.y, acc.z);
       tom_add(acc, acc, p);
@@ -529,8 +546,8 @@
   }
 };
 
-ZK_HD void tom2_ld_entry(TomPre& q, const uint32_t* tab, int j, size_t ne, uint32_t d, bool neg) {
-  tom_ld_pre(q, tab + ((size_t)j * ne + d) * TOM_PRE_WORDS);
+ZK_HD void tom2_ld_entry(TomPre& q, const uint32_t* tab, const FbShape& sh, int j, uint32_t d, bool neg) {
+  tom_ld_pre(q, tab + (sh.offset(j) + d) * TOM_PRE_WORDS);
   tom2_pre_neg(q, neg);
 }
 
@@ -540,27 +557,26 @@
   const uint32_t* gtab;
   const uint32_t* htab;
   uint32_t* proj;
-  int w, nwin;
+  FbShape sh;
   int xyz = 0;
   ZK_HD void operator()(int t) const {
     uint32_t v[8], r[8];
     ld<8>(v, jv + (size_t)t * 8);
     ld<8>(r, jr + (size_t)t * 8);
-    const size_t ne = (size_t)fb_entries(w);
     uint32_t cv = 0, cr = 0;
     bool nv, nr;
     TomPre q;
-    uint32_t dv = signed_digit(v, 0, w, cv, nv);
-    tom2_ld_entry(q, gtab, 0, ne, dv, nv);
+    uint32_t dv = signed_digit(v, 0, sh, cv, nv);
+    tom2_ld_entry(q, gtab, sh, 0, dv, nv);
     TomPt acc;
     tom2_from_pre(acc, q);
     for (int j = 0;; j++) {
-      const uint32_t dr = signed_digit(r, j, w, cr, nr);
-      tom2_ld_entry(q, htab, j, ne, dr, nr);
-      if (j == nwin - 1) break;
+      const uint32_t dr = signed_digit(r, j, sh, cr, nr);
+      tom2_ld_entry(q, htab, sh, j, dr, nr);
+      if (j == sh.nwin - 1) break;
       tom2_madd<true>(acc, acc, q);
-      dv = signed_digit(v, j + 1, w, cv, nv);
-      tom2_ld_entry(q, gtab, j + 1, ne, dv, nv);
+      dv = signed_digit(v, j + 1, sh, cv, nv);
+      tom2_ld_entry(q, gtab, sh, j + 1, dv, nv);
       tom2_madd<true>(acc, acc, q);
     }
     if (xyz) {
@@ -578,23 +594,22 @@
   const uint32_t* jv;
   const uint32_t* gtab;
   uint32_t* ext;
-  int w, nwin;
+  FbShape sh;
   ZK_HD void operator()(int t) const {
     const int item = t / GJOBS_PER_ITEM, g = t % GJOBS_PER_ITEM;
     uint32_t v[8];
     ld<8>(v, jv + ((size_t)item * JOBS_PER_ITEM + item_job_of_gpart(g)) * 8);
-    const size_t ne = (size_t)fb_entries(w);
     uint32_t carry = 0;
     bool neg;
     TomPre q;
-    const uint32_t d0 = signed_digit(v, 0, w, carry, neg);
-    tom2_ld_entry(q, gtab, 0, ne, d0, neg);
+    const uint32_t d0 = signed_digit(v, 0, sh, carry, neg);
+    tom2_ld_entry(q, gtab, sh, 0, d0, neg);
     TomPt acc;
     tom2_from_pre<TompCommit>(acc, q);
 #pragma unroll 1
-    for (int j = 1; j < nwin; j++) {
-      const uint32_t d = signed_digit(v, j, w, carry, neg);
-      tom2_ld_entry(q, gtab, j, ne, d, neg);
+    for (int j = 1; j < sh.nwin; j++) {
+      const uint32_t d = signed_digit(v, j, sh, carry, neg);
+      tom2_ld_entry(q, gtab, sh, j, d, neg);
       tom2_madd<true, TompCommit>(acc, acc, q);
     }
     uint32_t* o = ext + (size_t)t * TOM_EXT_WORDS;
@@ -606,7 +621,7 @@
   const uint32_t* htab;
   const uint32_t* ext;
   uint32_t* proj;
-  int w, nwin;
+  FbShape sh;
   ZK_HD void operator()(int t) const {
     const int item = t / JOBS_PER_ITEM, jb = t % JOBS_PER_ITEM;
     uint32_t r[8];
@@ -614,18 +629,17 @@
     TomPt acc;
     const uint32_t* s = ext + ((size_t)item * GJOBS_PER_ITEM + item_gpart_of_job(jb)) * TOM_EXT_WORDS;
     ld<9>(acc.x, s); ld<9>(acc.y, s + 9); ld<9>(acc.t, s + 18); ld<9>(acc.z, s + 27);
-    const size_t ne = (size_t)fb_entries(w);
     uint32_t carry = 0;
     bool neg;
     TomPre q;
 #pragma unroll 1
-    for (int j = 0; j < nwin - 1; j++) {
-      const uint32_t d = signed_digit(r, j, w, carry, neg);
-      tom2_ld_entry(q, htab, j, ne, d, neg);
+    for (int j = 0; j < sh.nwin - 1; j++) {
+      const uint32_t d = signed_digit(r, j, sh, carry, neg);
+      tom2_ld_entry(q, htab, sh, j, d, neg);
       tom2_madd<true, TompCommit>(acc, acc, q);
     }
-    const uint32_t d = signed_digit(r, nwin - 1, w, carry, neg);
-    tom2_ld_entry(q, htab, nwin - 1, ne, d, neg);
+    const uint32_t d = signed_digit(r, sh.nwin - 1, sh, carry, neg);
+    tom2_ld_entry(q, htab, sh, sh.nwin - 1, d, neg);
     TomEfgh e;
     tom2_madd_end<TompCommit>(e, acc, q);
     tom_st_efgh(proj + (size_t)t * TOM_E2_WORDS, e);
diff --git a/zkp_ecdsa_b200/csrc/zk_ops_war.cuh b/zkp_ecdsa_b200/csrc/zk_ops_war.cuh
--- a/zkp_ecdsa_b200/csrc/zk_ops_war.cuh
+++ b/zkp_ecdsa_b200/csrc/zk_ops_war.cuh
@@ -76,7 +76,7 @@
   const uint32_t* gtab;
   const uint32_t* htab;
   uint32_t* proj;
-  int w, nwin;
+  FbShape sh;
   int xyz = 0;
   ZK_HD void operator()(int t) const {
     uint32_t v[8], r[8];
@@ -84,8 +84,8 @@
     ld<8>(r, jr + (size_t)t * 8);
     WarJac aj;
     war_set_identity_jac(aj);
-    war_accum_fixed_jac(aj, gtab, v, w);
-    war_accum_fixed_jac(aj, htab, r, w);
+    war_accum_fixed_jac(aj, gtab, v, sh.w);
+    war_accum_fixed_jac(aj, htab, r, sh.w);
     WarPt acc;
     war_jac_to_hom(acc, aj);
     war_st_proj(proj + (size_t)t * TOM_PROJ_WORDS, acc);
@@ -95,14 +95,14 @@
   const uint32_t* jv;
   const uint32_t* gtab;
   uint32_t* ext;
-  int w, nwin;
+  FbShape sh;
   ZK_HD void operator()(int t) const {
     const int item = t / GJOBS_PER_ITEM, g = t % GJOBS_PER_ITEM;
     uint32_t v[8];
     ld<8>(v, jv + ((size_t)item * JOBS_PER_ITEM + item_job_of_gpart(g)) * 8);
     WarJac aj;
     war_set_identity_jac(aj);
-    war_accum_fixed_jac(aj, gtab, v, w);
+    war_accum_fixed_jac(aj, gtab, v, sh.w);
     WarPt acc;
     war_jac_to_hom(acc, aj);
     war_st_proj(ext + (size_t)t * TOM_EXT_WORDS, acc);
@@ -113,14 +113,14 @@
   const uint32_t* htab;
   const uint32_t* ext;
   uint32_t* proj;
-  int w, nwin;
+  FbShape sh;
   ZK_HD void operator()(int t) const {
     const int item = t / JOBS_PER_ITEM, jb = t % JOBS_PER_ITEM;
     uint32_t r[8];
     ld<8>(r, jr + (size_t)t * 8);
     WarPt acc;
     war_ld_proj(acc, ext + ((size_t)item * GJOBS_PER_ITEM + item_gpart_of_job(jb)) * TOM_EXT_WORDS);
-    war_accum_fixed(acc, htab, r, w);
+    war_accum_fixed(acc, htab, r, sh.w);
     war_st_proj(proj + (size_t)t * TOM_PROJ_WORDS, acc);
   }
 };
diff --git a/zkp_ecdsa_b200/csrc/zk_prove.cuh b/zkp_ecdsa_b200/csrc/zk_prove.cuh
--- a/zkp_ecdsa_b200/csrc/zk_prove.cuh
+++ b/zkp_ecdsa_b200/csrc/zk_prove.cuh
@@ -9,7 +9,7 @@
   int N;
   int n;
   int M;
-  int tom_w, tom_nwin;
+  FbShape tom;
   int mode;
   int head_len;
   const uint8_t* base;
diff --git a/zkp_ecdsa_b200/csrc/zk_verify.cuh b/zkp_ecdsa_b200/csrc/zk_verify.cuh
--- a/zkp_ecdsa_b200/csrc/zk_verify.cuh
+++ b/zkp_ecdsa_b200/csrc/zk_verify.cuh
@@ -29,7 +29,7 @@
   int K;
   int mode;
   const uint8_t* q_ext;
-  int tom_w, tom_nwin;
+  FbShape tom;
   const uint8_t* msg_hash;
   const uint8_t* proofs;
   size_t proof_stride;
diff --git a/zkp_ecdsa_b200/csrc/zkattest.cu b/zkp_ecdsa_b200/csrc/zkattest.cu
--- a/zkp_ecdsa_b200/csrc/zkattest.cu
+++ b/zkp_ecdsa_b200/csrc/zkattest.cu
@@ -290,7 +290,13 @@
   int nlanes = 3;
   DevBuf ring_in, ring_m;
   Lane& lane(int i) { return i == 0 ? *this : *extra[i - 1]; }
-  int tom_w = 22, tom_nwin = 12;
+#if defined(ZKA_PG_WAR256)
+  FbShape tom = fb_uniform(22);
+#else
+  FbShape tom = fb_lookups(11);
+#endif
+  size_t tom_table_max = 0;
+  bool tom_fallback = false;
   int chunk = 4096;
   int host_chunk = 2048;
   volatile uint32_t* progress = nullptr;
@@ -437,15 +443,21 @@
   launch_p256_norm(st, d_rows, out.tab, nullptr, nullptr, (long long)(count));
   sync(st);
 }
+uint32_t* alloc_tom_tab(zka_ctx* ctx, DevBuf& buf) {
+  const size_t words = ctx->tom.total() * TOM_PRE_WORDS;
+  if (ctx->tom_table_max && words * sizeof(uint32_t) > ctx->tom_table_max)
+    throw std::runtime_error("proof-group fixed-base table of " + std::to_string(words * sizeof(uint32_t)) + " bytes exceeds ZKA_TOM_TABLE_MAX");
+  return buf.get_exact<uint32_t>(words);
+}
 #if defined(ZKA_PG_WAR256)
 void build_tom_tab(zka_ctx* ctx, const uint32_t* base_aff_dev, FixedTable& out) {
   Stream& st = ctx->st;
-  const int w = ctx->tom_w, nwin = fb_windows(w);
+  const int w = ctx->tom.w, nwin = ctx->tom.nwin;
   const size_t E = (size_t)fb_entries(w), count = (size_t)nwin * E;
   DevBuf pows, rows;
   uint32_t* d_pows = pows.get<uint32_t>((size_t)nwin * P256_PROJ_WORDS);
   uint32_t* d_rows = rows.get<uint32_t>(count * P256_PROJ_WORDS);
-  out.tab = out.buf.get<uint32_t>(count * TOM_PRE_WORDS);
+  out.tab = alloc_tom_tab(ctx, out.buf);
   launch(st, 1, WarPowsTask{base_aff_dev, nullptr, d_pows, 1, nwin, w});
   if (w > 9) {
     DevBuf hi;
@@ -466,24 +478,29 @@
 #else
 void build_tom_tab(zka_ctx* ctx, const uint32_t* base_aff_dev, FixedTable& out) {
   Stream& st = ctx->st;
-  const int w = ctx->tom_w, nwin = ctx->tom_nwin;
-  const size_t ne = (size_t)fb_entries(w), count = (size_t)nwin * ne;
-  DevBuf pows, rows;
-  uint32_t* d_pows = pows.get<uint32_t>((size_t)nwin * 36);
-  uint32_t* d_rows = rows.get<uint32_t>(count * TOM_PROJ_WORDS);
-  out.tab = out.buf.get<uint32_t>(count * TOM_PRE_WORDS);
-  launch(st, 1, TomPowsTask{base_aff_dev, d_pows, 1, nwin, w});
-  if (w > 9) {
-    DevBuf hi;
-    const int nh = 1 << (w - 9);
-    uint32_t* d_hi = hi.get<uint32_t>((size_t)nwin * nh * 36);
-    launch(st, nwin, TomRowsHiTask{d_pows, d_hi, d_rows, w});
-    launch(st, (long long)nwin * nh, TomRowsLoTask{d_pows, d_hi, d_rows, w});
-    sync(st);
-  } else {
-    launch(st, nwin, TomRowsTask{d_pows, d_rows, w});
-  }
-  launch(st, (long long)(count + 15) / 16, TomTabE2Task{d_rows, out.tab, (int)count});
+  const FbShape sh = ctx->tom;
+  out.tab = alloc_tom_tab(ctx, out.buf);
+  DevBuf pows, rows, hi;
+  uint32_t* d_pows = pows.get<uint32_t>((size_t)sh.nwin * 36);
+  uint32_t* d_rows = rows.get<uint32_t>(sh.entries(sh.nwin - 1) * TOM_PROJ_WORDS);
+  launch(st, 1, TomPowsTask{base_aff_dev, d_pows, 1, sh});
+  const bool two_level = sh.w > 9;
+  uint32_t* d_hi = nullptr;
+  if (two_level) {
+    d_hi = hi.get<uint32_t>(tom_hi_offset(sh, sh.nwin) * 36);
+    launch(st, sh.nwin, TomRowsHiTask{d_pows, d_hi, sh});
+  }
+  for (int j = 0; j < sh.nwin; j++) {
+    const size_t ne = sh.entries(j);
+    const uint32_t* pw = d_pows + (size_t)j * 36;
+    if (two_level) {
+      const int nh = 1 << (sh.width(j) - 9);
+      launch(st, nh + 1, TomRowsLoTask{pw, d_hi + tom_hi_offset(sh, j) * 36, d_rows, nh});
+    } else {
+      launch(st, 1, TomRowsTask{pw, d_rows, sh.width(j)});
+    }
+    launch(st, (long long)(ne + 15) / 16, TomTabE2Task{d_rows, out.tab + sh.offset(j) * TOM_PRE_WORDS, (int)ne});
+  }
   sync(st);
 }
 
@@ -678,7 +695,7 @@
   ProveCtx c;
   memset(&c, 0, sizeof(c));
   c.B = B; c.S = S; c.N = N; c.n = n;
-  c.tom_w = ctx->tom_w; c.tom_nwin = ctx->tom_nwin;
+  c.tom = ctx->tom;
   c.g_tab8 = ctx->g8.tab; c.h_tab8 = P->h8.tab; c.h_w = P->h_w;
   c.g_tabw = ctx->gw.tab; c.g_w = ctx->p256_hw;
   c.tg_tab = ctx->tg.tab; c.th_tab = P->th.tab;
@@ -690,7 +707,7 @@
   VerifyCtx c;
   memset(&c, 0, sizeof(c));
   c.B = B; c.S = S; c.N = N; c.n = n; c.K = K; c.mode = mode;
-  c.tom_w = ctx->tom_w; c.tom_nwin = ctx->tom_nwin;
+  c.tom = ctx->tom;
   c.g_tab8 = ctx->g8.tab; c.h_tab8 = P->h8.tab; c.h_w = P->h_w;
   c.tg_tab = ctx->tg.tab; c.th_tab = P->th.tab;
   c.tg_bytes = (const uint8_t*)ctx->tg_bytes.p;
@@ -700,7 +717,7 @@
 void prove_store1(Stream& st, const ProveCtx& c) {
   const long long n1 = (long long)c.B * (2 + 2 * c.S);
   launch(st, n1, JobsATask{c});
-  launch(st, n1, TomCommitTask{c.s1_jv, c.s1_jr, c.tg_tab, c.th_tab, c.s1_proj, c.tom_w, c.tom_nwin});
+  launch(st, n1, TomCommitTask{c.s1_jv, c.s1_jr, c.tg_tab, c.th_tab, c.s1_proj, c.tom});
   launch_tom_norm(st, c.s1_proj, c.s1_aff, c.s1_bytes, n1, 1);
 }
 void prove_items_gk(Stream& st, const ProveCtx& c, uint32_t* gext, bool items, bool gk) {
@@ -719,12 +736,11 @@
     launch(st, Bn, GkCdJobsTask{c});
   }
   if (items) {
-    launch(st, M * GJOBS_PER_ITEM, TomCommitGTask{c.s2_jv, c.tg_tab, gext, c.tom_w, c.tom_nwin});
-    launch(st, nj, TomCommitHTask{c.s2_jr, c.th_tab, gext, c.s2_proj, c.tom_w, c.tom_nwin});
+    launch(st, M * GJOBS_PER_ITEM, TomCommitGTask{c.s2_jv, c.tg_tab, gext, c.tom});
+    launch(st, nj, TomCommitHTask{c.s2_jr, c.th_tab, gext, c.s2_proj, c.tom});
   }
   if (gk)
-    launch(st, ng, TomCommitTask{c.s2_jv + g0 * 8, c.s2_jr + g0 * 8, c.tg_tab, c.th_tab, c.s2_proj + g0 * TOM_E2_WORDS, c.tom_w,
-                                 c.tom_nwin});
+    launch(st, ng, TomCommitTask{c.s2_jv + g0 * 8, c.s2_jr + g0 * 8, c.tg_tab, c.th_tab, c.s2_proj + g0 * TOM_E2_WORDS, c.tom});
   if (items) {
     launch_tom_norm(st, c.s2_proj, c.s2_aff, c.s2_bytes, nj, 1, JOBS_PER_ITEM, 2);
     launch(st, M, DerivedTask{c});
@@ -818,6 +834,8 @@
   if (k == "agg_pass") return (long long)ctx->agg_pass;
   if (k == "agg_fail") return (long long)ctx->agg_fail;
   if (k == "agg_c") return (long long)ctx->agg_c_last;
+  if (k == "tom_n_lo") return (long long)ctx->tom.n_lo;
+  if (k == "tom_fallback") return ctx->tom_fallback ? 1 : 0;
   return -1;
 }
 size_t zka_profile_json(zka_ctx* ctx, char* buf, size_t cap) {
@@ -881,8 +899,8 @@
 int zka_lanes(const zka_ctx* ctx) { return ctx ? ctx->nlanes : 0; }
 int zka_config(const zka_ctx* ctx, int* tom_w, int* tom_nwin, int* chunk) {
   if (!ctx) return ZKA_E_ARG;
-  if (tom_w) *tom_w = ctx->tom_w;
-  if (tom_nwin) *tom_nwin = ctx->tom_nwin;
+  if (tom_w) *tom_w = ctx->tom.w;
+  if (tom_nwin) *tom_nwin = ctx->tom.nwin;
   if (chunk) *chunk = ctx->chunk;
   return 0;
 }
@@ -905,11 +923,18 @@
     ZK_CUDA_CHECK(cudaStreamCreateWithFlags(&ctx->st.s, cudaStreamNonBlocking));
 #endif
     ctx->device = device;
+    [[maybe_unused]] bool tom_pinned = false;
     if (const char* e = getenv("ZKA_TOM_W")) {
       int w = atoi(e);
-      if (w >= 2 && w <= 24) ctx->tom_w = w;
-    }
-    ctx->tom_nwin = fb_windows(ctx->tom_w);
+      if (w >= 2 && w <= 24) { ctx->tom = fb_uniform(w); tom_pinned = true; }
+    }
+#if !defined(ZKA_PG_WAR256)
+    if (const char* e = tom_pinned ? nullptr : getenv("ZKA_TOM_NWIN")) {
+      int n = atoi(e);
+      if (n >= 11 && n <= 128) ctx->tom = fb_lookups(n);
+    }
+#endif
+    if (const char* e = getenv("ZKA_TOM_TABLE_MAX")) ctx->tom_table_max = (size_t)strtoull(e, nullptr, 10);
     if (const char* e = getenv("ZKA_CHUNK")) {
       int c = atoi(e);
       if (c >= 1) ctx->chunk = c;
@@ -954,7 +979,24 @@
     launch(ctx->st, 1, GenAffTask{d_gen, d_gen + 16});
     build_p256_tab(ctx.get(), d_gen, ctx->g8, 8);
     build_p256_tab(ctx.get(), d_gen, ctx->gw, ctx->p256_hw);
+#if defined(ZKA_PG_WAR256)
     build_tom_tab(ctx.get(), d_gen + 16, ctx->tg);
+#else
+    try {
+      DevBuf room;
+      alloc_tom_tab(ctx.get(), room);
+      build_tom_tab(ctx.get(), d_gen + 16, ctx->tg);
+    } catch (const std::exception&) {
+      if (tom_pinned || ctx->tom.nwin >= 128) throw;
+#if !defined(ZKA_HOSTSIM)
+      cudaGetLastError();
+#endif
+      ctx->tg.buf.release();
+      ctx->tom = fb_lookups(ctx->tom.nwin + 1);
+      ctx->tom_fallback = true;
+      build_tom_tab(ctx.get(), d_gen + 16, ctx->tg);
+    }
+#endif
     DevBuf proj, aff;
     uint32_t* d_proj = proj.get<uint32_t>(TOM_PROJ_WORDS);
     uint32_t* d_aff = aff.get<uint32_t>(TOM_AFF_WORDS);
@@ -1084,7 +1126,7 @@
     const Output<uint8_t> o(out, WP);
     uint8_t* packed = o.rows(ob.next(), 0, count);
     launch(st, count, CommitConvTask{dv, dr, jv, jr});
-    launch(st, count, TomCommitTask{jv, jr, ctx->tg.tab, P->th.tab, proj, ctx->tom_w, ctx->tom_nwin});
+    launch(st, count, TomCommitTask{jv, jr, ctx->tg.tab, P->th.tab, proj, ctx->tom});
     launch_tom_norm(st, proj, aff, bytes, (long long)(count), 1);
     launch(st, count, PackTomTask{bytes, packed});
     o.copy_back(st, 0, packed, count);
@@ -1185,7 +1227,7 @@
     uint8_t* d_rnd = in.take<uint8_t>(32);
     copy_h2d(st, d_rnd, rnd + 32, 32);
     launch(st, 1, GenConvTask{d_rnd, jv, jr});
-    launch(st, 1, TomCommitTask{jv, jr, ctx->tg.tab, ctx->tg.tab, proj, ctx->tom_w, ctx->tom_nwin});
+    launch(st, 1, TomCommitTask{jv, jr, ctx->tg.tab, ctx->tg.tab, proj, ctx->tom});
     launch_tom_norm(st, proj, aff, bytes, (long long)(1), 1);
     copy_d2h(st, h_proof, bytes, WP);
     sync(st);
@@ -1613,7 +1655,7 @@
       uint8_t* d_prf = po.rows(ob.next(), b0, Bc);
       int32_t* d_st = so.rows(ob.next(), b0, Bc);
       launch(st, Bc, SubProveJobsTask{kind, d_sc, d_tape, tape_stride, jv, jr, d_st});
-      launch(st, (long long)nj, TomCommitTask{jv, jr, ctx->tg.tab, P->th.tab, proj, ctx->tom_w, ctx->tom_nwin});
+      launch(st, (long long)nj, TomCommitTask{jv, jr, ctx->tg.tab, P->th.tab, proj, ctx->tom});
       launch_tom_norm(st, proj, nullptr, bytes, (long long)nj, 1);
       launch(st, Bc, SubProveEmitTask{kind, d_sc, d_tape, tape_stride, jr, bytes, d_com, d_prf, d_st});
       co.copy_back(st, b0, d_com, Bc);
@@ -1859,7 +1901,7 @@
     launch(st, (long long)ns, VSampleP256Task{c});
     launch_p256_norm(st, c.sp_T, c.sp_T_aff, nullptr, c.sp_T_inf, (long long)(ns));
     launch(st, (long long)ns, VSampleJobsTask{c});
-    launch(st, (long long)ns * 2, TomCommitTask{c.ta_jv, c.ta_jr, c.tg_tab, c.th_tab, c.ta_proj, c.tom_w, c.tom_nwin});
+    launch(st, (long long)ns * 2, TomCommitTask{c.ta_jv, c.ta_jr, c.tg_tab, c.th_tab, c.ta_proj, c.tom});
     launch_tom_norm(st, c.ta_proj, c.ta_aff, nullptr, (long long)(ns * 2), 1);
     launch(st, (long long)ns, VDerivedTask{c});
     launch_tom_norm(st, c.td_proj, nullptr, c.td_bytes, (long long)(ns * DERS_PER_ITEM), 0);
@@ -1873,7 +1915,7 @@
     launch(st, Bc, VReduceTask{c});
     launch(st, (long long)Bc * ET, VParseEntriesTask{c.proofs, c.proof_stride, c.ent_off, c.ent_pre, ET});
     if (mode == 0) launch(st, (long long)Bc * ngk, VParseEntriesTask{c.proofs, c.proof_stride, gk_offs, c.gk_pre, ngk});
-    launch(st, (long long)Bc * 2, TomCommitTask{c.fx_jv, c.fx_jr, c.tg_tab, c.th_tab, c.fx_proj, c.tom_w, c.tom_nwin, 1});
+    launch(st, (long long)Bc * 2, TomCommitTask{c.fx_jv, c.fx_jr, c.tg_tab, c.th_tab, c.fx_proj, c.tom, 1});
     uint32_t* ctl = nullptr;
     if (ctx->agg && mode == 0) {
       Cursor A(ln.agg);
@@ -1912,7 +1954,7 @@
       agg_msm(sb, Cursor(ln.agg_nist), nsrc, np, ctl, &nA, &nB);
       launch(st, fgroups, AggFixPartTask{ctl, c.fx_jv, c.fx_jr, fpart, Bc});
       launch(st, 1, AggFixSumTask{ctl, fpart, fjv, fjr, fgroups});
-      launch(st, 1, TomCommitTask{fjv, fjr, c.tg_tab, c.th_tab, fproj, c.tom_w, c.tom_nwin, 1});
+      launch(st, 1, TomCommitTask{fjv, fjr, c.tg_tab, c.th_tab, fproj, c.tom, 1});
       launch(sb, ngroups, AggNistFixPartTask{ctl, c.nfix, npart, Bc});
       int nleft = ngroups;
       const uint32_t* nsum = npart;
@@ -2102,7 +2144,7 @@
       dev_memset(st, c.fx_jr, 0, (size_t)Bc * 2 * 8 * 4);
       verify_gk(st, c, gk_offs);
       launch(st, (long long)Bc * ngk, VParseEntriesTask{c.proofs, row_stride, gk_offs, c.gk_pre, ngk});
-      launch(st, (long long)Bc * 2, TomCommitTask{c.fx_jv, c.fx_jr, c.tg_tab, c.th_tab, c.fx_proj, c.tom_w, c.tom_nwin, 1});
+      launch(st, (long long)Bc * 2, TomCommitTask{c.fx_jv, c.fx_jr, c.tg_tab, c.th_tab, c.fx_proj, c.tom, 1});
       launch(st, (long long)Bc * MSM_NWIN, MsmTomWindowTask{c.gk_scalar, c.gk_pre, nullptr, ngk, 0, 0, ngk, V_SEG, 1, c.win_g});
       launch(st, Bc, MsmTomCombineTask{c.win_g, c.fx_proj, c.id_flags, 2, 0, 0});
       launch(st, Bc, VGkOnlyFinalTask{c});
@@ -2147,7 +2189,7 @@
       launch(st, Bc, VSubProofTask{kind, rows, stride, d_tape, tape_stride, (const uint8_t*)ctx->tg_bytes.p, ent_scalar, ent_off,
                                    fx_jv, fx_jr, d_st, d_ok});
       launch(st, (long long)Bc * SUB_ENT_MAX, VParseEntriesTask{rows, stride, ent_off, ent_pre, SUB_ENT_MAX});
-      launch(st, (long long)Bc * 2, TomCommitTask{fx_jv, fx_jr, ctx->tg.tab, P->th.tab, fx_proj, ctx->tom_w, ctx->tom_nwin, 1});
+      launch(st, (long long)Bc * 2, TomCommitTask{fx_jv, fx_jr, ctx->tg.tab, P->th.tab, fx_proj, ctx->tom, 1});
       launch(st, (long long)Bc * MSM_NWIN, MsmTomWindowTask{ent_scalar, ent_pre, nullptr, SUB_ENT_MAX, 0, 0, ne, V_SEG, 1, win});
       launch(st, Bc, MsmTomCombineTask{win, fx_proj, flags, 2, 1, 1});
       launch(st, Bc, VSubFinalTask{d_st, flags, d_ok});
```

Result: faster. 118,100, median of 6 (+5.1%).
